# diku-kmc/kleenexlang

Measured on AMD Instinct MI355X. Metric: input GB/s + % HBM-read roofline, apache_log.kex over 10 GiB synthetic log, higher is better.
Workload: dtype u8

## Files before the change

include/kxhip.h:

```cpp
#ifndef KXHIP_H
#define KXHIP_H
#include <stddef.h>
#include <stdint.h>
#ifdef __cplusplus
extern "C" {
#endif

typedef struct kx_program kx_program;
typedef struct kx_shard kx_shard;

#define KX_OK 0
#define KX_MATCH_ERROR 1
#define KX_E_BLOB (-1)
#define KX_E_HIP (-2)
#define KX_E_CAPACITY (-3)
#define KX_E_ARG (-4)
#define KX_E_IO (-5)

enum { KX_K_SYNC = 0, KX_K_FORWARD = 1, KX_K_HEAD = 2, KX_K_BACKLEN = 3, KX_K_RESOLVE = 4, KX_K_EMIT = 5, KX_NKERNELS = 6 };

typedef struct kx_stats {
  uint64_t fail_pos;
  uint32_t fail_stage;
  uint32_t unsynced_segments;
// ... 44 lines not shown
int kx_load_config(const void* blob, size_t blob_len, const kx_config* cfg, kx_program** prog);
int kx_validate(const void* blob, size_t blob_len);
void kx_free(kx_program* prog);
const char* kx_last_error(void);
int kx_set_config(kx_program* prog, const kx_config* cfg);
uint32_t kx_num_stages(const kx_program* prog);
int kx_stage_has_actions(const kx_program* prog, uint32_t stage);

typedef struct kx_df_info {
  uint32_t available;
  uint32_t delay;
  uint32_t nstates;
  uint32_t nclasses;
  uint32_t image_bytes, off_pool, start_handle, dead_handle, escape_handle;
  uint32_t transitions, escapes;
  uint32_t transitions_start, escapes_start;
  uint32_t merge_window;
  char reason[96];
} kx_df_info;
int kx_df_describe(const void* blob, size_t blob_len, uint32_t stage, kx_df_info* info, void* image, size_t image_cap);
int kx_df_pending(const void* blob, size_t blob_len, uint32_t stage, uint32_t state, uint32_t slot, uint32_t* sst_state,
                  uint32_t* kinds, uint32_t* n_out);
int kx_df_describe_cfg(const void* blob, size_t blob_len, uint32_t stage, const kx_config* cfg, kx_df_info* info, void* image, size_t image_cap);
int kx_df_pending_cfg(const void* blob, size_t blob_len, uint32_t stage, const kx_config* cfg, uint32_t state, uint32_t slot,
                      uint32_t* sst_state, uint32_t* kinds, uint32_t* n_out);
int kx_df_deferred(const void* blob, size_t blob_len, uint32_t stage, const kx_config* cfg, uint32_t state, void* bytes, size_t cap, size_t* n_out);
int kx_df_start_of_state(const void* blob, size_t blob_len, uint32_t stage, const kx_config* cfg, uint32_t sst_state, uint32_t* handle);
int kx_stage_delayed_form(const kx_program* prog, uint32_t stage);
void kx_stage_reset_delayed_form(kx_program* prog, uint32_t stage);

#define KX_STAGE_MAIN 0u
#define KX_STAGE_ALT 1u
#define KX_STAGE_DELAYED 2u
#define KX_STAGE_SLOW 3u
typedef struct kx_stage_info {
  uint32_t size;
  uint32_t which;
  uint64_t image_bytes;
  uint32_t general, big, has_alt, has_df, actions, action_regs, max_const_len, reserved0;
  uint64_t lds_bytes, sync_lds_bytes;
  struct {
    uint64_t packed, pair, wlen, cls, nleaves, fin_leaf, sync16, init_off, init_len;
    uint32_t packed_words, off_fwd, off_ent, off_pool, off_cls, off_adesc, naid, nstates, nclasses, q0h, maxleaves, deadh, nullrow, cshift,
        debug, big, hshift, rshift, rbase, stage_words, pair_words, pair_magic, nsync, sync_multi, sync_words, off_tbl, xlat, tblmode,
        aid_mask, inl, jl, direct, short_consts, reserved0;
  } t;
  struct {
    uint64_t img, start_of_state, sl_fmap, sl_back, sl_nleaves, sl_fin_leaf, sl_cls, sl_pcoff, sl_pcpool, sl_pend, sl_defoff, sl_defpc, sl_q;
    uint32_t words, off_pool, deadh, esch, starth, K, C, orig_c4, hshift, short_consts, debug, nstates, J, wide, sl_Lm, sl_npc, sl_on, reserved0;
  } d;
} kx_stage_info;
int kx_stage_describe_cfg(const void* blob, size_t blob_len, uint32_t stage, const kx_config* cfg, uint32_t which, kx_stage_info* info,
                          void* image, size_t image_cap);

int kx_run_device(kx_program* prog, const void* d_in, size_t n, void* d_out, size_t cap, size_t* out_len,
                  kx_stats* stats, void* stream);

int kx_run_host(kx_program* prog, const void* in, size_t n, void** out, size_t* out_len, kx_stats* stats);
void kx_host_free(void* p);

int kx_run_fd(kx_program* prog, int in_fd, int out_fd, kx_stats* stats);

typedef struct kx_batch_doc {
  uint64_t fail_pos;
  uint32_t status;
  uint32_t fail_stage;
} kx_batch_doc;
typedef struct kx_batch_stats {
  uint64_t docs, docs_rejected;
  uint64_t docs_routed;
  uint64_t in_bytes, out_bytes;
  float forward_ms, back_ms, scan_ms, emit_ms, routed_ms, total_ms;
  uint64_t docs_replayed;
  float actions_ms;
  uint32_t reserved[1];
} kx_batch_stats;
int kx_run_batch(kx_program* prog, const void* d_in, const uint64_t* d_in_off, uint64_t n_docs, void* d_out, size_t cap,
                 uint64_t* d_out_off, kx_batch_doc* d_docs, size_t* out_len, kx_batch_stats* stats, void* stream);

typedef struct kx_batch_frame {
  uint32_t trim;
  uint32_t last_whole;
  uint32_t suffix_len;
  uint8_t suffix[8];
  uint32_t reserved[3];
} kx_batch_frame;
int kx_run_batch_framed(kx_program* prog, const void* d_in, const uint64_t* d_in_off, uint64_t n_docs, const kx_batch_frame* frame,
                        void* d_out, size_t cap, uint64_t* d_out_off, kx_batch_doc* d_docs, size_t* out_len, kx_batch_stats* stats,
                        void* stream);

int kx_split_records(const void* d_in, size_t n, uint8_t sep, uint64_t base, uint64_t* d_off, uint64_t cap,
                     uint64_t* n_records, void* stream);

typedef struct kx_records_stats {
  uint64_t records, records_rejected, records_routed, in_bytes, out_bytes, windows, longest_record;
  float split_ms, batch_ms, total_ms;
  uint32_t reserved[4];
} kx_records_stats;
int kx_run_records_fd(kx_program* p, int in_fd, int out_fd, uint8_t sep, int report_fd, kx_records_stats* stats);

int kx_split_records_quoted(const void* d_in, size_t n, uint8_t sep, uint8_t quote, uint32_t parity_in, uint64_t base,
                            uint64_t* d_off, uint64_t cap, uint64_t* n_records, uint32_t* parity_out, void* stream);
int kx_run_records_fd_quoted(kx_program* p, int in_fd, int out_fd, uint8_t sep, uint8_t quote, int report_fd,
                             kx_records_stats* stats);

int kx_split_records_escaped(const void* d_in, size_t n, uint8_t sep, int quote, uint8_t escape, uint32_t state_in, uint64_t base,
// ... 139 lines not shown
```

kleenexlang_amd/csrc/engine/gen_sweeps.py:

```python
#!/usr/bin/env python3
import sys

SD = "dst_sel:DWORD dst_unused:UNUSED_PAD"


def fwd2():
    L = []
    ap = L.append
    def cls_issue(ch, t, slot):
        wi, by = t >> 2, t & 3
        ap("v_lshlrev_b32_sdwa %%[x%s], 0, %%[w%d] %s src0_sel:DWORD src1_sel:BYTE_%d" % (ch, wi, SD, by))
        ap("ds_read_u8 %%[c%s%d], %%[x%s]" % (ch, slot, ch))
    base = {"A": 0, "B": 32}
    for d in (0, 1):
        for ch in "AB":
            cls_issue(ch, base[ch] + d, d)
    ap("s_waitcnt lgkmcnt(2)")
    for ch in "AB":
        ap("v_add_u32 %%[a%s], %%[h%s], %%[c%s0]" % (ch, ch, ch))
        ap("ds_read_b32 %%[e%s0], %%[a%s]" % (ch, ch))
    for j in range(32):
        cur, nxt = j & 1, (j + 1) & 1
        if j + 2 < 32:
            for ch in "AB":
# ... 314 lines not shown
            sweep2j(),
            ['[%s] "=&v"(%s)' % (t, t) for t in tmpj] + ['[leafA] "+v"(leafA)', '[oA] "+v"(oA)', '[leafB] "+v"(leafB)', '[oB] "+v"(oB)',
                                                        '[pA] "+v"(pA)', '[pB] "+v"(pB)'],
            ['[bo%d] "v"(bo[%d])' % (i, i) for i in range(32)] + ['[w%d] "v"(w[%d])' % (i, i) for i in range(16)],
            '"memory"')
    tmp = tmp + ["tiA", "tiB"]
    emit_fn(out, "piece_sweep2i",
            "const uint32_t (&bo)[32], const uint32_t (&w)[16], uint32_t leafA, uint32_t oA, uint32_t leafB, uint32_t oB, "
            "uint32_t& jb, uint32_t jlim",
            "uint32_t " + ", ".join(tmp) + ", st; unsigned long long sv, mA, mU;",
            sweep2(True),
            ['[%s] "=&v"(%s)' % (t, t) for t in tmp] + ['[sv] "=&s"(sv)', '[mA] "=&s"(mA)', '[mU] "=&s"(mU)', '[st] "=&s"(st)', '[leafA] "+v"(leafA)', '[oA] "+v"(oA)',
                                                       '[leafB] "+v"(leafB)', '[oB] "+v"(oB)', '[jb] "+s"(jb)'],
            ['[bo%d] "v"(bo[%d])' % (i, i) for i in range(32)] + ['[w%d] "v"(w[%d])' % (i, i) for i in range(16)] +
            ['[jlim] "s"(jlim)'],
            '"vcc", "scc", "memory"')


def main2(out):
    tmp = ["e0", "e1", "c0", "c1", "c2", "x"]
    emit_fn(out, "piece_forward1",
            "const uint32_t (&w)[16], uint32_t h, uint32_t himask, uint32_t (&bo)[32]",
            "uint32_t " + ", ".join(tmp) + ";",
            fwd1(True),
            ['[bo%d] "=&v"(bo[%d])' % (i, i) for i in range(32)] + ['[%s] "=&v"(%s)' % (t, t) for t in tmp],
            ['[w%d] "v"(w[%d])' % (i, i) for i in range(16)] + ['[h] "v"(h)', '[hm] "s"(himask)'],
            '"memory"')
    emit_fn(out, "piece_run1",
            "const uint32_t (&w)[16], uint32_t& h, uint32_t& mid",
            "uint32_t " + ", ".join(tmp) + ";",
            fwd1(False),
            ['[%s] "=&v"(%s)' % (t, t) for t in tmp] + ['[mid] "=&v"(mid)', '[h] "+v"(h)'],
            ['[w%d] "v"(w[%d])' % (i, i) for i in range(16)],
            '"memory"')
    emit_fn(out, "piece_walk1j",
            "const uint32_t (&bo)[32], uint32_t& leaf, uint32_t& sum, uint32_t& lmid, uint32_t& shi",
            "uint32_t a, e;",
            walk1(True),
            ['[a] "=&v"(a)', '[e] "=&v"(e)', '[lmid] "=&v"(lmid)', '[shi] "=&v"(shi)', '[leaf] "+v"(leaf)', '[sum] "+v"(sum)'],
            ['[bo%d] "v"(bo[%d])' % (i, i) for i in range(32)],
            '"memory"')
    emit_fn(out, "piece_walk1",
            "const uint32_t (&bo)[32], uint32_t& leaf, uint32_t& sum, uint32_t& lmid, uint32_t& shi",
            "uint32_t a, e;",
            walk1(),
            ['[a] "=&v"(a)', '[e] "=&v"(e)', '[lmid] "=&v"(lmid)', '[shi] "=&v"(shi)', '[leaf] "+v"(leaf)', '[sum] "+v"(sum)'],
            ['[bo%d] "v"(bo[%d])' % (i, i) for i in range(32)],
            '"memory"')


DF_WALK_E = {"A": (("v116", "v117"), ("v118", "v119")), "B": (("v120", "v121"), ("v122", "v123"))}


def dfrun1(wide=False):
    L = []
    ap = L.append
    E = (("%[e0]",), ("%[e1]",))
    def cls_issue(tt):
        ap("v_lshlrev_b32_sdwa %%[x], 0, %%[w%d] %s src0_sel:DWORD src1_sel:BYTE_%d" % (tt >> 2, SD, tt & 3))
        ap("ds_read_u8 %%[c%d], %%[x]" % (tt % 3))
    for tt in (0, 1, 2):
        cls_issue(tt)
    ap("s_waitcnt lgkmcnt(2)")
    if wide:
        ap("v_lshlrev_b32 %[c0], 3, %[c0]")
    ap("v_add_u32 %[x], %[h], %[c0]")
    ap("ds_read_b32 %s, %%[x]" % E[0][0])
    for j in range(64):
        cur, nxt = j & 1, (j + 1) & 1
        if j + 3 < 64:
            cls_issue(j + 3)
        ap("s_waitcnt lgkmcnt(%d)" % (1 if j + 3 < 64 else 0))
        if j + 1 < 64:
            if wide:
                ap("v_lshlrev_b32 %%[c%d], 3, %%[c%d]" % ((j + 1) % 3, (j + 1) % 3))
            ap("v_add_u32_sdwa %%[x], %s, %%[c%d] %s src0_sel:WORD_0 src1_sel:DWORD" % (E[cur][0], (j + 1) % 3, SD))
            ap("ds_read_b32 %s, %%[x]" % E[nxt][0])
        ap("v_add_u32_sdwa %%[sum], %%[sum], %s %s src0_sel:DWORD src1_sel:WORD_1" % (E[cur][0], SD))
        if j == 31:
            ap("v_and_b32 %%[mid], 0xffff, %s" % E[cur][0])
            ap("v_mov_b32 %[lenA], %[sum]")
            ap("v_and_b32 %[sum], 0xffffff00, %[sum]")
        if j == 63:
            ap("v_and_b32 %%[h], 0xffff, %s" % E[cur][0])
    return L


def dfwalk2(K, counted=True, wide=False):
    L = []
    ap = L.append
    base = {"A": 0, "B": 32}
    E = DF_WALK_E
    pair = lambda ch, k: "v[%s:%s]" % (E[ch][k][0][1:], E[ch][k][1][1:])
    def cls_issue(ch, t, slot):
        ap("v_lshlrev_b32_sdwa %%[x%s], 0, %%[w%d] %s src0_sel:DWORD src1_sel:BYTE_%d" % (ch, t >> 2, SD, t & 3))
        ap("ds_read_u8 %%[c%s%d], %%[x%s]" % (ch, slot, ch))
    twof = {"A": None, "B": None}
    ap("s_setprio 3")
    for d in (0, 1):
        for ch in "AB":
            cls_issue(ch, base[ch] + d, d)
    ap("s_waitcnt lgkmcnt(2)")
    for ch in "AB":
        if wide:
            ap("v_lshlrev_b32 %%[c%s0], 3, %%[c%s0]" % (ch, ch))
        ap("v_add_u32 %%[a%s0], %%[h%s], %%[c%s0]" % (ch, ch, ch))
        ap("ds_read_b64 %s, %%[a%s0]" % (pair(ch, 0), ch))
    for j in range(32):
        cur, nxt = j & 1, (j + 1) & 1
        if j + 2 < 32:
            for ch in "AB":
                cls_issue(ch, base[ch] + j + 2, (j + 2) % 3)
        ap("s_waitcnt lgkmcnt(%d)" % (2 if j == 0 else (4 if counted else 6) if j + 2 < 32 else (2 if counted else 4)))
        if j + 1 < 32:
            for ch in "AB":
                if wide:
                    ap("v_lshlrev_b32 %%[c%s%d], 3, %%[c%s%d]" % (ch, (j + 1) % 3, ch, (j + 1) % 3))
                ap("v_add_u32_sdwa %%[a%s%d], %s, %%[c%s%d] %s src0_sel:WORD_0 src1_sel:DWORD" % (ch, nxt, E[ch][cur][0], ch, (j + 1) % 3, SD))
                ap("ds_read_b64 %s, %%[a%s%d]" % (pair(ch, nxt), ch, nxt))
        for ch in "AB":
            t = base[ch] + j
            so = t - K
            hi, o, a, x = E[ch][cur][1], "%%[o%s]" % ch, "%%[a%s%d]" % (ch, cur), "%%[x%s]" % ch
            if so >= 0:
                wreg, by = "%%[w%d]" % (so >> 2), so & 3
            else:
                wreg, by = "%[wp]", (4 + so) & 3
            if by in (1, 3) and twof[ch] != wreg:
# ... 36 lines not shown
    E = DF_WALK_E["A"]
    pair = lambda k: "v[%s:%s]" % (E[k][0][1:], E[k][1][1:])
    def cls_issue(t, slot):
        ap("v_lshlrev_b32_sdwa %%[x], 0, %%[w%d] %s src0_sel:DWORD src1_sel:BYTE_%d" % (t >> 2, SD, t & 3))
        ap("ds_read_u8 %%[c%d], %%[x]" % slot)
    twof = None
    ap("s_setprio 3")
    for d in (0, 1, 2):
        cls_issue(d, d)
    ap("s_waitcnt lgkmcnt(2)")
    if wide:
        ap("v_lshlrev_b32 %[c0], 3, %[c0]")
    ap("v_add_u32 %[a0], %[h], %[c0]")
    ap("ds_read_b64 %s, %%[a0]" % pair(0))
    for j in range(32):
        cur, nxt = j & 1, (j + 1) & 1
        if j + 3 < 32:
            cls_issue(j + 3, (j + 3) % 3)
        ap("s_waitcnt lgkmcnt(%d)" % ((1 if j + 3 < 32 else 0) + (0 if j == 0 else 1)))
        if j + 1 < 32:
            if wide:
                ap("v_lshlrev_b32 %%[c%d], 3, %%[c%d]" % ((j + 1) % 3, (j + 1) % 3))
            ap("v_add_u32_sdwa %%[a%d], %s, %%[c%d] %s src0_sel:WORD_0 src1_sel:DWORD" % (nxt, E[cur][0], (j + 1) % 3, SD))
            ap("ds_read_b64 %s, %%[a%d]" % (pair(nxt), nxt))
        so = j - K
        hi, a = E[cur][1], "%%[a%d]" % cur
        if so >= 0:
            wreg, by = "%%[w%d]" % (so >> 2), so & 3
        else:
            wreg, by = "%[wp]", (4 + so) & 3
        if by in (1, 3) and twof != wreg:
            ap("v_lshrrev_b32 %%[tw], 8, %s" % wreg)
            twof = wreg
        src = "%[tw]" if by in (1, 3) else wreg
        wr = "ds_write_b8_d16_hi" if by >= 2 else "ds_write_b8"
        ap("v_cmp_gt_i32_sdwa vcc, 0, sext(%s) src0_sel:DWORD src1_sel:BYTE_2" % hi)
        ap("v_lshl_or_b32 %s, %%[o], 16, %s" % (a, a))
        ap("v_lshl_or_b32 %%[x], %s, 31, %%[o]" % hi)
        ap("v_add_u32_sdwa %%[o], %%[o], %s %s src0_sel:DWORD src1_sel:BYTE_3" % (hi, SD))
        ap("%s %%[x], %s" % (wr, src))
        ap("s_and_saveexec_b64 %[sv], vcc")
        ap("ds_write_b32 %%[p], %s" % a)
        ap("s_mov_b64 exec, %[sv]")
        ap("v_add_u32_sdwa %%[p], %%[p], %s %s src0_sel:DWORD src1_sel:BYTE_2" % (E[cur][0], SD))
    ap("s_setprio 0")
    return L


def main7(out):
    tmp = ["c0", "c1", "c2", "x", "e0", "e1"]
    emit_fn(out, "piece_dfrun1w",
            "const uint32_t (&w)[16], uint32_t& h, uint32_t& mid, uint32_t& lenA, uint32_t& sum",
            "uint32_t " + ", ".join(tmp) + ";",
            dfrun1(True),
            ['[%s] "=&v"(%s)' % (t, t) for t in tmp] + ['[mid] "=&v"(mid)', '[lenA] "=&v"(lenA)', '[h] "+v"(h)', '[sum] "+v"(sum)'],
            ['[w%d] "v"(w[%d])' % (i, i) for i in range(16)],
            '"memory"')
    emit_fn(out, "piece_dfrun1",
            "const uint32_t (&w)[16], uint32_t& h, uint32_t& mid, uint32_t& lenA, uint32_t& sum",
            "uint32_t " + ", ".join(tmp) + ";",
            dfrun1(),
            ['[%s] "=&v"(%s)' % (t, t) for t in tmp] + ['[mid] "=&v"(mid)', '[lenA] "=&v"(lenA)', '[h] "+v"(h)', '[sum] "+v"(sum)'],
            ['[w%d] "v"(w[%d])' % (i, i) for i in range(16)],
            '"memory"')
    tmp1 = ["c0", "c1", "c2", "x", "a0", "a1", "tw"]
    clob1 = ", ".join('"%s"' % r for pr in DF_WALK_E["A"] for r in pr)
    for K, wd in ((1, False), (2, False), (1, True), (2, True)):
        emit_fn(out, "piece_dfwalk1c%s_k%d" % ("w" if wd else "", K),
                "const uint32_t (&w)[8], uint32_t wp, uint32_t h, uint32_t& o, uint32_t& p",
                "uint32_t " + ", ".join(tmp1) + "; unsigned long long sv;",
                dfwalk1(K, wd),
                ['[%s] "=&v"(%s)' % (t, t) for t in tmp1] + ['[sv] "=&s"(sv)', '[o] "+v"(o)', '[p] "+v"(p)'],
                ['[w%d] "v"(w[%d])' % (i, i) for i in range(8)] + ['[wp] "v"(wp)', '[h] "v"(h)'],
                '"vcc", "scc", "memory", ' + clob1)
    tmp = ["cA0", "cA1", "cA2", "cB0", "cB1", "cB2", "xA", "xB", "aA0", "aA1", "aB0", "aB1", "twA", "twB"]
    clob = ", ".join('"%s"' % r for ch in "AB" for pr in DF_WALK_E[ch] for r in pr)
    for K, wd in ((1, False), (2, False), (1, True), (2, True)):
        emit_fn(out, "piece_dfwalk2c%s_k%d" % ("w" if wd else "", K),
                "const uint32_t (&w)[16], uint32_t wp, uint32_t hA, uint32_t& oA, uint32_t hB, uint32_t& oB, uint32_t& pA, uint32_t& pB",
                "uint32_t " + ", ".join(tmp) + "; unsigned long long sv;",
                dfwalk2(K, counted=True, wide=wd),
                ['[%s] "=&v"(%s)' % (t, t) for t in tmp] + ['[sv] "=&s"(sv)', '[oA] "+v"(oA)', '[oB] "+v"(oB)', '[pA] "+v"(pA)', '[pB] "+v"(pB)'],
                ['[w%d] "v"(w[%d])' % (i, i) for i in range(16)] + ['[wp] "v"(wp)', '[hA] "v"(hA)', '[hB] "v"(hB)'],
                '"vcc", "scc", "memory", ' + clob)


if __name__ == "__main__":
    main()
    main2(sys.stdout)
    main6(sys.stdout)
    main7(sys.stdout)
```

kleenexlang_amd/csrc/engine/kx_dfkernels.inc:

```

constexpr uint32_t DF_HOLE_MAX = 4096, DF_HOLE_FIRST = 1024, DF_SL_LEAVES = 32;
struct __attribute__((aligned(8))) DfRec { uint32_t x, y; };
constexpr uint32_t DFREC_OWN = 0x80000000u, DFREC_HOLE = 0x80000000u, DFREC_HOLE_FIRST = 0x40000000u;
constexpr uint32_t DF_MERGE_WINDOW_MAX = 64;
using kxst::DF_STEP_MAX;
constexpr uint32_t DF_HOLE_LEN_MAX = 0xFFFFu, DF_HOLE_CNT_MAX = 0x3FFFu, DF_WBASE_PIECES = 32;
constexpr DfRec dfrec_pack(uint32_t start, uint32_t middle, uint32_t lenA, uint32_t len, uint32_t kA, uint32_t kB) {
  return DfRec{(start >> 3) | ((middle >> 3) << 13) | (kA << 26), len | (lenA << 13) | (kB << 25)};
}
constexpr DfRec dfrec_pack_hole(uint32_t side_first, uint32_t entries, bool first, uint32_t len) {
  return DfRec{side_first, len | (entries << 16) | (first ? DFREC_HOLE_FIRST : 0u) | DFREC_HOLE};
}
constexpr bool dfrec_hole(DfRec r) { return (r.y & DFREC_HOLE) != 0; }
constexpr uint32_t dfrec_start(DfRec r) { return (r.x & 0x1FFFu) << 3; }
constexpr uint32_t dfrec_middle(DfRec r) { return ((r.x >> 13) & 0x1FFFu) << 3; }
constexpr uint32_t dfrec_kA(DfRec r) { return r.x >> 26; }
constexpr uint32_t dfrec_kB(DfRec r) { return (r.y >> 25) & 0x3Fu; }
constexpr uint32_t dfrec_len(DfRec r) { return r.y & 0x1FFFu; }
constexpr uint32_t dfrec_lenA(DfRec r) { return (r.y >> 13) & 0xFFFu; }
constexpr uint32_t dfrec_hole_side(DfRec r) { return r.x; }
constexpr uint32_t dfrec_hole_len(DfRec r) { return r.y & DF_HOLE_LEN_MAX; }
constexpr uint32_t dfrec_hole_entries(DfRec r) { return (r.y >> 16) & DF_HOLE_CNT_MAX; }
constexpr bool dfrec_hole_first(DfRec r) { return (r.y & DFREC_HOLE_FIRST) != 0; }
namespace dfrec_check {
constexpr uint32_t H = 65536 - 8, LA = HALF * DF_STEP_MAX, LN = PIECE * DF_STEP_MAX, KH = HALF;
constexpr DfRec top = dfrec_pack(H, H, LA, LN, KH, KH), one = dfrec_pack(8, 65536 - 16, 1, 2, 0, KH), zero = dfrec_pack(0, 0, 0, 0, 0, 0);
static_assert(sizeof(DfRec) == 8 && LN < (1u << 13) && LA < (1u << 12) && KH < (1u << 6), "piece record: a field outgrew its width");
static_assert(!dfrec_hole(top) && dfrec_start(top) == H && dfrec_middle(top) == H && dfrec_lenA(top) == LA && dfrec_len(top) == LN &&
              dfrec_kA(top) == KH && dfrec_kB(top) == KH, "piece record: every field at its maximum");
static_assert(!dfrec_hole(one) && dfrec_start(one) == 8 && dfrec_middle(one) == 65536 - 16 && dfrec_lenA(one) == 1 && dfrec_len(one) == 2 &&
              dfrec_kA(one) == 0 && dfrec_kB(one) == KH, "piece record: neighbouring fields do not bleed");
static_assert(!dfrec_hole(zero) && zero.x == 0 && zero.y == 0, "piece record: all fields zero");
constexpr DfRec htop = dfrec_pack_hole(0xFFFFFFFFu, DF_HOLE_CNT_MAX, true, DF_HOLE_LEN_MAX), hlow = dfrec_pack_hole(0, 0, false, 0);
static_assert(dfrec_hole(htop) && dfrec_hole_side(htop) == 0xFFFFFFFFu && dfrec_hole_entries(htop) == DF_HOLE_CNT_MAX && dfrec_hole_first(htop) &&
              dfrec_hole_len(htop) == DF_HOLE_LEN_MAX, "hole record: every field at its maximum");
static_assert(dfrec_hole(hlow) && dfrec_hole_side(hlow) == 0 && dfrec_hole_entries(hlow) == 0 && !dfrec_hole_first(hlow) && dfrec_hole_len(hlow) == 0, "hole record: all fields zero");
static_assert(PIECE + kxdf::DF_MAX_K + DF_MERGE_WINDOW_MAX <= DF_HOLE_CNT_MAX, "hole record: the entries of a piece fit");
static_assert((uint64_t)MAX_SEG * DF_STEP_MAX < DFREC_OWN, "wave base: a block part's output stays below the own flag");
static_assert(DF_WBASE_PIECES == HALF && 2 * DF_WBASE_PIECES == PIECE, "wave base: one word per wave-iteration of half pieces, two per iteration of pieces");
}
struct DfLds {
  const uint8_t* base; uint32_t csh;
  __device__ __forceinline__ uint32_t c8(uint32_t byte) const { return (uint32_t)base[byte] << csh; }
  __device__ __forceinline__ uint2 ent(uint32_t a) const { return *reinterpret_cast<const uint2*>(base + a); }
};
__device__ __forceinline__ DfLds df_stage(const DfDev& D, uint32_t* smem) {
  for (uint32_t i = threadIdx.x; i < D.words; i += blockDim.x) smem[i] = D.img[i];
  __syncthreads();
  return DfLds{reinterpret_cast<const uint8_t*>(smem), D.wide ? 3u : 0u};
}

__device__ __forceinline__ void df_run_piece(const uint32_t (&w)[16], uint32_t& h, uint32_t& mid, uint32_t& lenA, uint32_t& len, const DfLds& L) {
  uint32_t c[8], cn[8], sum = 0;
  static_for<0, 8>([&](auto ic) { constexpr int i = decltype(ic)::value; c[i] = L.c8(BYTE_AT_DEP(w, i, h)); });
  static_for<0, PIECE / 8>([&](auto gc) {
    constexpr int g = decltype(gc)::value;
    if constexpr (g + 1 < PIECE / 8)
      static_for<0, 8>([&](auto ic) { constexpr int i = decltype(ic)::value; cn[i] = L.c8(BYTE_AT_DEP(w, 8 * (g + 1) + i, h)); });
    static_for<0, 8>([&](auto ic) {
      constexpr int i = decltype(ic)::value;
      const uint2 e = L.ent(h + c[i]);
      h = e.x & 0xFFFFu; sum += e.y >> 24; tie(h, sum);
    });
    if constexpr (g == HALF / 8 - 1) { mid = h; lenA = sum; }
    if constexpr (g + 1 < PIECE / 8)
      static_for<0, 8>([&](auto ic) { constexpr int i = decltype(ic)::value; c[i] = cn[i]; });
  });
  len = sum;
}

__device__ __forceinline__ uint64_t df_own_start(uint32_t j, uint64_t n, uint64_t seg, int first_known, const uint64_t* __restrict__ seg_pos,
                                                 const uint16_t* __restrict__ seg_state, const DfDev& D) {
  if (j == 0 && first_known) return 0;
  const uint64_t p = seg_pos[j];
  if (p == UNSYNC) return UNSYNC;
  const uint32_t q = (((uint32_t)seg_state[j] << D.hshift) - OFF_FWD) / D.orig_c4;
  if (q >= D.nstates || D.start_of_state[q] == 0xFFFFu) return UNSYNC;
  const uint64_t b = (p + D.K + D.J + 63) & ~63ull;
  const uint64_t lim = ((uint64_t)j + 1) * seg < n ? ((uint64_t)j + 1) * seg : n;
  return b < lim ? b : UNSYNC;
}

struct DfSlowIO {
  const uint8_t* in; uint64_t n, a, end; uint32_t h0, last, is_last;
  uint32_t h_behind; uint32_t* side; uint32_t side_cap; Flags* flags; const uint8_t* lds; uint32_t clsh; uint8_t* lmap; uint32_t max_steps;
  uint32_t base, nd, h_next; uint64_t e_out;
};
__device__ __noinline__ int df_slow_resolve(DfSlowIO& io, const DfDev& D) {
  const uint8_t* __restrict__ in = io.in;
  const uint64_t n = io.n, a = io.a, end = io.end;
  const uint32_t h0 = io.h0;
  const bool last = io.last != 0, is_last = io.is_last != 0;
  uint32_t* side = io.side; const uint32_t side_cap = io.side_cap; Flags* flags = io.flags;
  if (!D.sl_on || !side) return 1;
  const uint32_t C = D.C, Lm = D.sl_Lm, K = D.K, NONE = D.sl_npc << 1;
  const uint32_t i0 = (h0 - 256u) / (C * 8u);
  uint32_t q = D.sl_q[i0];
  const uint32_t nd = D.sl_defoff[i0 + 1] - D.sl_defoff[i0];
  const uint64_t hard = a + io.max_steps < n ? a + io.max_steps : n;
  const uint32_t need = nd + K + (uint32_t)(hard - a) + 64u;
  const uint32_t base = atomicAdd(&flags->side_used, need);
  if ((uint64_t)base + need > side_cap) return 1;
// ... 83 lines not shown
    uint32_t v = 0xFFu; bool same = true;
    const uint32_t par[8] = {f1.x, f1.y, f1.z, f1.w, f2v.x, f2v.y, f2v.z, f2v.w};
#pragma unroll
    for (uint32_t l = 0; l < DF_SL_LEAVES; ++l) {
      const uint32_t pl = (par[l >> 2] >> (8 * (l & 3u))) & 0xFFu;
      const uint32_t x = l >= nnl || pl == 0xFFu ? 0xFFu : M[pl];
      if (l < nnl) M2[l] = (uint8_t)x;
      if (x != 0xFFu) { if (v == 0xFFu) v = x; else same = same && x == v; }
    }
    { uint8_t* tmp = M; M = M2; M2 = tmp; }
    q = nq; nl = nnl; ++t;
    if ((!same || v == 0xFFu) && ((t - a) & 63u) == 0 && t + PIECE <= end && D.start_of_state[q] != 0xFFFFu && agree_at(t, nl)) {
      qb[(t - a) >> 6] = (uint16_t)q;
      mode = 1; e_out = t;
      break;
    }
    if (!same || v == 0xFFu) continue;
    anchor_known(v);
    const uint64_t decided = anchor;
    prev = anchor; anchor = t;
    for (uint32_t l = 0; l < DF_SL_LEAVES; ++l) M[l] = (uint8_t)l;
    const uint64_t e = decided & ~63ull;
    if (e > a && e + PIECE <= end && D.start_of_state[qb[(e - a) >> 6]] != 0xFFFFu) { mode = 1; e_out = e; break; }
    if (!last && decided + K >= end) { mode = 2; e_out = end; break; }
  }
  (void)nl;
  uint32_t h_next = h0;
  if (mode == 1) h_next = D.start_of_state[qb[(e_out - a) >> 6]];
  if (mode == 3) {
    if (D.start_of_state[q] == 0xFFFFu) return 1;
    h_next = D.start_of_state[q];
  }
  if (mode == 2) {
    for (uint64_t u = end - K; u < end; ++u) if (u >= a) R[u - a] = NONE; else E[nd + K - (a - u)] = NONE;
    const uint32_t ix = (io.h_behind - 256u) / (C * 8u);
    uint32_t due = D.sl_defoff[ix + 1] - D.sl_defoff[ix];
    for (uint32_t idx = nd + K + (uint32_t)(end - K - a); due && idx-- > 0;) {
      const uint32_t pc = (E[idx] >> 1) & 0x3FFFFFFFu;
      if (pc < D.sl_npc && D.sl_pcoff[pc + 1] > D.sl_pcoff[pc]) { E[idx] = (E[idx] & 0x80000001u) | NONE; --due; }
    }
    if (due) return 1;
  }
  io.base = base; io.nd = nd; io.h_next = h_next; io.e_out = e_out;
  return 0;
}

template <int BT, uint32_t DF_STAGE, int MINW, bool SLOW>
__global__ __launch_bounds__(BT, MINW) void k_dforward(const uint8_t* __restrict__ in, uint64_t n, uint64_t seg, uint32_t nseg, int first_known,
                           const uint64_t* __restrict__ seg_pos, const uint16_t* __restrict__ seg_state,
                           DfRec* __restrict__ rec, uint32_t* __restrict__ wbase, uint32_t* __restrict__ own, uint32_t* __restrict__ spill, Flags* flags,
                           uint32_t* __restrict__ side, uint32_t side_cap, int is_last, DfDev D) {
  static_assert(DF_STAGE == 8 || DF_STAGE == 16, "a group of staged records is one or half a 128-byte line, and at least the slow path's 64-byte map");
  extern __shared__ __attribute__((aligned(16))) uint32_t smem[];
  DfLds L = df_stage(D, smem);
  uint2* lrec = reinterpret_cast<uint2*>(smem + ((D.words + 3) & ~3u)) + (size_t)threadIdx.x * DF_STAGE;
  const uint32_t k = blockIdx.x * blockDim.x + threadIdx.x;
  const uint32_t lane = threadIdx.x & 63;
  const uint64_t B = k < nseg ? df_own_start(k, n, seg, first_known, seg_pos, seg_state, D) : UNSYNC;
  bool alive = B != UNSYNC;
  const uint32_t dead = D.deadh, esc = D.esch;
  auto warm = [&](uint32_t jj, uint64_t Bj) -> uint32_t {
    if (jj == 0 && first_known) return D.starth;
    uint32_t hw = D.start_of_state[(((uint32_t)seg_state[jj] << D.hshift) - OFF_FWD) / D.orig_c4];
    for (uint64_t pw = seg_pos[jj]; pw < Bj;) {
      const uint2 v = *reinterpret_cast<const uint2*>(in + (pw & ~7ull));
      const uint64_t x = (uint64_t)v.x | ((uint64_t)v.y << 32);
      for (uint32_t b = (uint32_t)pw & 7u; b < 8u && pw < Bj; ++b, ++pw) hw = L.ent(hw + L.c8((uint32_t)(x >> (8 * b)) & 0xFFu)).x & 0xFFFFu;
    }
    if (hw == esc && jj == k) atomicAdd(&flags->warm_esc, 1u);
    return hw == esc || hw == dead ? 0xFFFFFFFFu : hw;
  };
  uint32_t h = dead, h_behind = 0;
  if (alive) { h = warm(k, B); if (h == 0xFFFFFFFFu) { alive = false; h = dead; } }
  uint32_t j = k + 1;
  uint64_t end = n;
  if (alive) for (; j < nseg; ++j) {
    const uint64_t b = df_own_start(j, n, seg, first_known, seg_pos, seg_state, D);
    if (b == UNSYNC) continue;
    h_behind = warm(j, b);
    if (h_behind != 0xFFFFFFFFu) { end = b; break; }
  }
  const bool last = alive && j >= nseg;
  uint64_t pos = alive ? B : 0;
  if (alive) atomicMin(&flags->df_first_own, (unsigned long long)B);
  bool failed = !alive;
  if (!alive) { end = 0; pos = 0; }
  uint32_t m = (uint32_t)(pos / seg), cum = 0, flag = DFREC_OWN;
  uint64_t block_end = ((uint64_t)m + 1) * seg;
  auto fail_in = [&](uint32_t h0, uint64_t p0, uint32_t plen) -> int {
    uint32_t hh = h0;
    for (uint32_t t = 0; t < plen; ++t) {
      const uint32_t nh = L.ent(hh + L.c8(in[p0 + t])).x & 0xFFFFu;
      if (nh == dead) { atomicMin(&flags->fail_pos, (unsigned long long)(p0 + t)); failed = true; return 1; }
      if (nh == esc) return 2;
      hh = nh;
    }
    failed = true;
    return 1;
  };
  uint32_t nst = 0; uint64_t gfirst = 0;
  auto flush_group = [&]() {
    uint2* dst = reinterpret_cast<uint2*>(rec + gfirst);
    for (uint32_t i = 0; i < nst; ++i) dst[i] = lrec[(gfirst + i) & (DF_STAGE - 1)];
    nst = 0;
  };
  const bool coop = !(D.debug & 256u);
  bool in_trip = false;
  auto stage_rec = [&](uint64_t pc, DfRec r) {
    if (nst == 0) gfirst = pc;
    if ((pc & (DF_WBASE_PIECES - 1)) == 0) wbase[pc / DF_WBASE_PIECES] = cum | flag;
    lrec[pc & (DF_STAGE - 1)] = make_uint2(r.x, r.y); ++nst;
    if (!in_trip && (pc & (DF_STAGE - 1)) == DF_STAGE - 1) flush_group();
  };
  auto group_aligned = [&]() { return ((uint32_t)(pos >> 6) & (DF_STAGE - 1)) == nst; };
  uint2* const lrec_wave = reinterpret_cast<uint2*>(smem + ((D.words + 3) & ~3u)) + (size_t)(threadIdx.x & ~63u) * DF_STAGE;
  auto coop_flush = [&]() {
    const bool full = nst == DF_STAGE && (gfirst & (DF_STAGE - 1)) == 0;
    if (!__any(full)) return;
    const uint32_t glo = (uint32_t)gfirst, ghi = (uint32_t)(gfirst >> 32) | (full ? 0u : 0x80000000u);
    constexpr uint32_t RPL = DF_STAGE / 8;
    const uint32_t team = lane & ~7u, r = (lane & 7u) * RPL;
    static_for<0, 8>([&](auto ic) {
      constexpr uint32_t i = decltype(ic)::value;
      const uint32_t slo = (uint32_t)__shfl((int)glo, (int)(team + i)), shi = (uint32_t)__shfl((int)ghi, (int)(team + i));
      if (!(shi & 0x80000000u)) {
        const uint64_t g = ((uint64_t)shi << 32) | slo;
        const uint2* src = lrec_wave + (size_t)(team + i) * DF_STAGE + r;
        if constexpr (RPL == 2) *reinterpret_cast<uint4*>(rec + g + r) = *reinterpret_cast<const uint4*>(src);
        else *reinterpret_cast<uint2*>(rec + g + r) = *src;
      }
    });
    if (full) nst = 0;
  };
  auto cross = [&]() { if (pos == block_end) { (flag ? own : spill)[m] = cum; cum = 0; flag = 0; ++m; block_end += seg; } };
  uint32_t kc_sum = 0, kc_max = 0, kc_n = 0;
  auto slow = [&](const uint64_t a, const uint32_t h0) -> int {
    flush_group();
    DfSlowIO io{in, n, a, end, h0, last ? 1u : 0u, (uint32_t)is_last, h_behind, side, side_cap, flags, L.base, D.wide ? 0u : 3u, reinterpret_cast<uint8_t*>(lrec), DF_HOLE_FIRST, 0, 0, 0, 0};
    {
      int rc = df_slow_resolve(io, D);
      if (rc == 3) { io.max_steps = DF_HOLE_MAX; rc = df_slow_resolve(io, D); }
      if (rc) return rc == 3 ? 1 : rc;
    }
    const uint32_t base = io.base, nd = io.nd, K = D.K;
    const uint64_t e_out = io.e_out;
    const uint32_t* const E = side + base;
    const uint64_t pend = (e_out + 63) & ~63ull;
    uint32_t idx = 0;
    for (uint64_t pp = a; pp < pend; pp += PIECE) {
      cross();
      const bool first = pp == a;
      const uint32_t steps = (uint32_t)((e_out - pp) < PIECE ? e_out - pp : PIECE);
      const uint32_t cnt = first ? nd + K + steps : steps;
      uint32_t len = 0;
      for (uint32_t x = 0; x < cnt; ++x) {
        const uint32_t ee = E[idx + x], pc = (ee >> 1) & 0x3FFFFFFFu;
        len += (ee & 1u) + (pc < D.sl_npc ? D.sl_pcoff[pc + 1] - D.sl_pcoff[pc] : 0u);
      }
      if (len > DF_HOLE_LEN_MAX || cnt > DF_HOLE_CNT_MAX) return 1;
      if (((pp >> 6) & (DF_WBASE_PIECES - 1)) == 0) wbase[(pp >> 6) / DF_WBASE_PIECES] = cum | flag;
      rec[pp >> 6] = dfrec_pack_hole(base + idx, cnt, first, len);
      idx += cnt; cum += len; pos = pp + steps;
    }
    h = io.h_next;
    atomicAdd(&flags->slow_steps, (uint32_t)(e_out - a));
    return 0;
  };
  bool need_slow = false;
  auto run_slow = [&]() {
    need_slow = false;
    int r = 1;
    if constexpr (SLOW) r = slow(pos, h);
    if (r) { if (r == 1) atomicAdd(&flags->df_esc, 1u); failed = true; }
  };
  auto do_piece = [&](const uint32_t (&w)[16]) -> bool {
    cross();
    const uint32_t h0 = h;
    uint32_t mid, sumA, sum = 0;
    if (D.wide) piece_dfrun1w(w, h, mid, sumA, sum); else piece_dfrun1(w, h, mid, sumA, sum);
    if (h == dead || h == esc) {
      if (fail_in(h0, pos, PIECE) == 2) { need_slow = true; h = h0; }
      return false;
    }
    const uint32_t kA = (sumA & 0xFFu) >> 2, kB = (sum & 0xFFu) >> 2;
    kc_sum += kA + kB; kc_max = kA + kB > kc_max ? kA + kB : kc_max; ++kc_n;
    stage_rec(pos >> 6, dfrec_pack(h0, mid, sumA >> 8, sum >> 8, kA, kB));
    cum += sum >> 8; pos += PIECE;
    return true;
  };
  auto single_piece = [&]() {
    uint32_t w[16];
    load_piece(in, n, pos, w);
    do_piece(w);
  };
  for (;;) {
  if (need_slow) run_slow();
  while (!failed && !need_slow && pos + PIECE <= end && ((pos & (8 * PIECE - 1)) || !group_aligned())) single_piece();
  for (;;) {
    const bool can = !failed && !need_slow && pos + 8 * PIECE <= end && !(pos & (8 * PIECE - 1)) && group_aligned();
    if (!__any(can) || __any(need_slow)) break;
    uint32_t line[8];
    {
      const uint32_t mine = can ? (uint32_t)(pos >> 7) : 0xFFFFFFFFu;
      static_for<0, 8>([&](auto ic) { constexpr int i = decltype(ic)::value; line[i] = __shfl(mine, (int)((lane & ~7u) + i)); });
    }
    auto issue = [&](uint32_t k2, uint4 (&dst)[8]) {
      static_for<0, 8>([&](auto ic) {
        constexpr int i = decltype(ic)::value;
        const uint64_t ln = line[i] != 0xFFFFFFFFu ? line[i] : 0u;
        dst[i] = *reinterpret_cast<const uint4*>(in + ((ln + k2) << 7) + (lane & 7u) * 16);
      });
    };
    uint4 v[8];
    issue(0, v);
    bool died = false;
    in_trip = coop;
#pragma nounroll
    for (uint32_t k2 = 0; k2 < 4; ++k2) {
      transpose8(v, lane);
      uint32_t wa[16], wb[16];
      static_for<0, 8>([&](auto ic) {
        constexpr int w = decltype(ic)::value;
        uint32_t (&dst)[16] = w < 4 ? wa : wb;
        dst[4 * (w & 3)] = v[w].x; dst[4 * (w & 3) + 1] = v[w].y; dst[4 * (w & 3) + 2] = v[w].z; dst[4 * (w & 3) + 3] = v[w].w;
      });
      bool go = can && !died;
      if (go && !do_piece(wa)) { died = true; go = false; }
      if (k2 < 3) issue(k2 + 1, v);
      if (go && !do_piece(wb)) died = true;
    }
    if (coop) coop_flush();
    in_trip = false;
  }
  if (!__any(!failed && (need_slow || pos + 8 * PIECE <= end))) break;
  }
  if (!alive) return;
  for (;;) {
  if (need_slow) run_slow();
  while (!failed && !need_slow && pos + PIECE <= end) single_piece();
  if (need_slow) continue;
  if (!failed && pos < end) {
    cross();
    const uint32_t plen = (uint32_t)(end - pos), h0 = h;
    uint32_t mid = h, lenA = 0, len = 0, kA = 0, kc = 0;
    for (uint32_t t = 0; t < plen; ++t) {
      if (t == HALF) { mid = h; lenA = len; kA = kc; }
      const uint2 e = L.ent(h + L.c8(in[pos + t]));
      h = e.x & 0xFFFFu; len += e.y >> 24; kc += (e.y >> 23) & 1u;
    }
    if (plen <= HALF) { mid = h; lenA = len; kA = kc; }
    if (h == dead || h == esc) {
      if (fail_in(h0, pos, plen) == 2) { h = h0; need_slow = true; continue; }
    }
    else { stage_rec(pos >> 6, dfrec_pack(h0, mid, lenA, len, kA, kc - kA)); cum += len; pos = end; }
  }
  break;
  }
  flush_group();
  if (failed) return;
  (flag ? own : spill)[m] = cum;
  if (last) flags->end_state = h;
  if (kc_n) { if ((k & 15u) == 0) { atomicAdd(&flags->emit_ksum, kc_sum); atomicAdd(&flags->emit_kn, kc_n); } atomicMax(&flags->emit_kmax, kc_max); }
}

__global__ void k_dhead(const uint8_t* __restrict__ in, uint64_t n, uint64_t seg, uint64_t head_len, uint32_t h,
                        DfRec* __restrict__ rec, uint32_t* __restrict__ wbase, uint32_t* __restrict__ own, uint32_t* __restrict__ spill, Flags* flags, DfDev D) {
  extern __shared__ __attribute__((aligned(16))) uint32_t smem[];
  DfLds L = df_stage(D, smem);
  if (blockIdx.x || threadIdx.x) return;
  const uint32_t dead = D.deadh, esc = D.esch;
  uint32_t m = 0, cum = 0;
  uint64_t block_end = seg;
  for (uint64_t pos = 0; pos < head_len;) {
    if (pos == block_end) { spill[m] = cum; cum = 0; ++m; block_end += seg; }
    const uint32_t plen = (uint32_t)(head_len - pos < PIECE ? head_len - pos : PIECE);
    const uint32_t h0 = h;
    uint32_t mid = h, lenA = 0, len = 0, kA = 0, kc = 0;
    for (uint32_t t = 0; t < plen; ++t) {
      if (t == HALF) { mid = h; lenA = len; kA = kc; }
      const uint2 e = L.ent(h + L.c8(in[pos + t]));
      const uint32_t nh = e.x & 0xFFFFu;
      if (nh == dead) { atomicMin(&flags->fail_pos, (unsigned long long)(pos + t)); return; }
      if (nh == esc) { flags->df_esc = 1; return; }
      h = nh; len += e.y >> 24; kc += (e.y >> 23) & 1u;
    }
    if (plen <= HALF) { mid = h; lenA = len; kA = kc; }
    if (kc > 0) atomicMax(&flags->emit_kmax, kc);
    if (((pos >> 6) & (DF_WBASE_PIECES - 1)) == 0) wbase[(pos >> 6) / DF_WBASE_PIECES] = cum;
    rec[pos >> 6] = dfrec_pack(h0, mid, lenA, len, kA, kc - kA);
    cum += len; pos += plen;
  }
  spill[m] = cum;
  if (head_len == n) flags->end_state = h;
}

__global__ void k_dlen(uint32_t nblk, const uint32_t* __restrict__ own, const uint32_t* __restrict__ spill, uint32_t* __restrict__ len,
                       unsigned long long* __restrict__ wsum) {
  __shared__ unsigned long long red[1024];
  const uint32_t m = blockIdx.x * blockDim.x + threadIdx.x;
  uint32_t mylen = 0;
  if (m < nblk) { mylen = own[m] + spill[m]; len[m] = mylen; }
  red[threadIdx.x] = mylen;
  __syncthreads();
  for (uint32_t s = blockDim.x >> 1; s > 0; s >>= 1) {
    if (threadIdx.x < s) red[threadIdx.x] += red[threadIdx.x + s];
    __syncthreads();
  }
  if (threadIdx.x == 0) wsum[blockIdx.x] = red[0];
}

template <bool GENERAL>
__global__ void k_dmap(const uint8_t* __restrict__ in, uint64_t n, uint32_t q_in, uint64_t cap, uint8_t* __restrict__ map_out,
                       uint32_t* __restrict__ status, DevTables T) {
  extern __shared__ __attribute__((aligned(16))) uint32_t smem[];
// ... 309 lines not shown
```

kleenexlang_amd/csrc/engine/kx_engine.hip:

```cpp
#include <hip/hip_runtime.h>
#include <fcntl.h>
#include <sys/stat.h>
#include <unistd.h>

#include <cerrno>
#include <condition_variable>
#include <cstdint>
#include <algorithm>
#include <deque>
#include <mutex>
#include <chrono>
#include <thread>
#include <cstdio>
#include <cstdlib>
#include <cstring>
#include <string>
#include <type_traits>
#include <vector>

#include "../../../include/kxhip.h"
#include "../../../include/kxp_format.h"
#include "kx_stage.h"

namespace {
// ... 1833 lines not shown

}

extern "C" {

const char* kx_last_error(void) { return g_err.c_str(); }
void kx_internal_set_error(const char* m) { g_err = m ? m : ""; }

static int buildStage(const uint8_t*& c, const uint8_t* end, const kx_config& cfg, unsigned what, Stage& S) {
  std::string err;
  const int rc = kxst::buildStage(c, end, cfg, what, S, err);
  return rc ? setErr(rc, err) : 0;
}
static int blobHeader(const void* blob, size_t blob_len, const uint8_t** first, uint32_t* nstages) {
  std::string err;
  const int rc = kxst::readBlobHeader(blob, blob_len, first, nstages, err);
  return rc ? setErr(rc, err) : 0;
}

int kx_validate(const void* blob, size_t blob_len) {
  const uint8_t* c = nullptr; uint32_t ns = 0;
  int rc = blobHeader(blob, blob_len, &c, &ns);
  for (uint32_t s = 0; s < ns && !rc; ++s) {
    Stage S;
    rc = buildStage(c, (const uint8_t*)blob + blob_len, kx_config{}, 0, S);
  }
  return rc;
}

static int parseOneStage(const void* blob, size_t blob_len, uint32_t stage, const kx_config* cfgp, Stage& S, unsigned what = kxst::WITH_DELAYED) {
  const uint8_t* c; uint32_t ns;
  int rc = blobHeader(blob, blob_len, &c, &ns);
  if (rc) return rc;
  if (stage >= ns) return setErr(KX_E_ARG, "no such stage");
  for (uint32_t st = 0; st <= stage && !rc; ++st) {
    Stage T;
    rc = buildStage(c, (const uint8_t*)blob + blob_len, cfgp ? *cfgp : kx_config{}, st == stage ? what : 0, st == stage ? S : T);
  }
  return rc;
}

int kx_stage_describe_cfg(const void* blob, size_t blob_len, uint32_t stage, const kx_config* cfg, uint32_t which, kx_stage_info* info,
                          void* image, size_t image_cap) {
  if (!info || info->size != sizeof(kx_stage_info) || which > KX_STAGE_SLOW) return setErr(KX_E_ARG, "kx_stage_info::size is not this library's, or no such image");
  Stage S;
  int rc = parseOneStage(blob, blob_len, stage, cfg, S, kxst::WITH_ALT | kxst::WITH_DELAYED);
  if (rc) return rc;
  kxst::describeStage(S, which, *info);
  const std::vector<uint8_t>& bytes = which == KX_STAGE_MAIN ? S.img : which == KX_STAGE_ALT ? S.img_alt : which == KX_STAGE_DELAYED ? S.img_df : S.img_slow;
  if (image && !bytes.empty()) memcpy(image, bytes.data(), image_cap < bytes.size() ? image_cap : bytes.size());
  return 0;
}

int kx_df_describe(const void* blob, size_t blob_len, uint32_t stage, kx_df_info* info, void* image, size_t image_cap) {
  return kx_df_describe_cfg(blob, blob_len, stage, nullptr, info, image, image_cap);
}

int kx_df_describe_cfg(const void* blob, size_t blob_len, uint32_t stage, const kx_config* cfg, kx_df_info* info, void* image, size_t image_cap) {
  if (!info) return setErr(KX_E_ARG, "null argument");
  Stage S;
  int rc = parseOneStage(blob, blob_len, stage, cfg, S);
  if (rc) return rc;
  memset(info, 0, sizeof *info);
  info->available = S.has_df ? 1u : 0u;
  snprintf(info->reason, sizeof info->reason, "%s", S.df_why.c_str());
  if (S.df.nP) {
    info->delay = S.df.K; info->nstates = S.df.nP; info->nclasses = S.df.C; info->image_bytes = (uint32_t)S.df.img.size() * 4;
    info->off_pool = S.df.off_pool; info->start_handle = S.df.starth; info->dead_handle = S.df.deadh; info->escape_handle = S.df.esch;
    info->transitions = S.df.ntrans; info->escapes = S.df.nesc; info->transitions_start = S.df.ntrans_start; info->escapes_start = S.df.nesc_start;
    info->merge_window = S.df.J;
    if (image) memcpy(image, S.df.img.data(), image_cap < S.df.img.size() * 4 ? image_cap : S.df.img.size() * 4);
  }
  return 0;
}

int kx_df_pending(const void* blob, size_t blob_len, uint32_t stage, uint32_t state, uint32_t slot, uint32_t* sst_state,
                  uint32_t* kinds, uint32_t* n_out) {
  return kx_df_pending_cfg(blob, blob_len, stage, nullptr, state, slot, sst_state, kinds, n_out);
}

int kx_df_pending_cfg(const void* blob, size_t blob_len, uint32_t stage, const kx_config* cfg, uint32_t state, uint32_t slot,
                      uint32_t* sst_state, uint32_t* kinds, uint32_t* n_out) {
  if (!kinds || !n_out || !sst_state) return setErr(KX_E_ARG, "null argument");
  Stage S;
  int rc = parseOneStage(blob, blob_len, stage, cfg, S);
  if (rc) return rc;
  if (state >= S.df.states.size() || slot >= S.df.K) return setErr(KX_E_ARG, "no such product state / slot");
  const kxdf::Slot& g = S.df.states[state].pend[slot];
  *sst_state = S.df.states[state].q;
  *n_out = (uint32_t)g.size();
  for (size_t i = 0; i < g.size() && i < KX_MAX_LEAVES; ++i) kinds[i] = g[i];
  return 0;
}

int kx_df_deferred(const void* blob, size_t blob_len, uint32_t stage, const kx_config* cfg, uint32_t state, void* bytes, size_t cap, size_t* n_out) {
  if (!n_out || (cap && !bytes)) return setErr(KX_E_ARG, "null argument");
  Stage S;
  int rc = parseOneStage(blob, blob_len, stage, cfg, S);
  if (rc) return rc;
  if (state >= S.df.states.size()) return setErr(KX_E_ARG, "no such product state");
  std::string t;
  for (const auto& d : S.df.states[state].def)
    if (d.first < S.df_pc_len.size()) t.append((const char*)S.h_pool.data() + S.df_pc_off[d.first], S.df_pc_len[d.first]);
  *n_out = t.size();
  if (cap) memcpy(bytes, t.data(), t.size() < cap ? t.size() : cap);
  return 0;
// ... 1159 lines not shown
```

kleenexlang_amd/csrc/engine/kx_stage.h:

```cpp
#ifndef KX_STAGE_H
#define KX_STAGE_H
#include <cstdint>
#include <cstring>
#include <string>
#include <vector>

#include "../../../include/kxhip.h"
#include "../../../include/kxp_format.h"
#include "kx_delayed.h"

namespace kxst {

#ifdef __HIP__
using Quad = uint4;
#else
struct Quad { uint32_t x, y, z, w; };
#endif

constexpr uint32_t OFF_FWD = 256;
constexpr uint32_t PAIR_CLS2_AT = 16128;
constexpr uint32_t DF_STEP_MAX = 126;

struct DevTables {
  const uint32_t* packed;
  uint32_t packed_words;
  uint32_t off_fwd, off_ent, off_pool, off_cls, off_adesc, naid;
  uint32_t nstates, nclasses, q0h, maxleaves, deadh, nullrow, cshift, debug;
  uint32_t big, hshift, rshift, rbase, stage_words;
  const uint32_t* pair; uint32_t pair_words, pair_magic;
  const uint32_t* wlen;
  const uint8_t* cls;
  const uint8_t* nleaves;
  const uint8_t* fin_leaf;
  const uint16_t* sync16;
  uint32_t nsync, sync_multi, sync_words;
  const uint32_t* init_off;
  const uint32_t* init_len;
  uint32_t off_tbl, xlat, tblmode, aid_mask;
  uint32_t inl;
  uint32_t jl;
  uint32_t direct;
  uint32_t short_consts;
};

struct DfDev {
  const uint32_t* img; uint32_t words;
  uint32_t off_pool, deadh, esch, starth, K, C;
  const uint16_t* start_of_state;
  uint32_t orig_c4, hshift;
  uint32_t short_consts, debug;
  uint32_t nstates;
  uint32_t J;
  uint32_t wide;
  const Quad* sl_fmap;
  const uint32_t* sl_back; const uint8_t* sl_nleaves; const uint8_t* sl_fin_leaf; const uint8_t* sl_cls;
  const uint32_t* sl_pcoff; const uint8_t* sl_pcpool; const uint32_t* sl_pend; const uint32_t* sl_defoff; const uint32_t* sl_defpc; const uint16_t* sl_q;
  uint32_t sl_Lm, sl_npc, sl_on;
};

template <class P> void setOff(const P*& p, size_t off) { p = reinterpret_cast<const P*>(off); }
template <class P> size_t offOf(const P* p) { return reinterpret_cast<size_t>(p); }
template <class P> void rebase(const P*& p, const void* base) { p = reinterpret_cast<const P*>(reinterpret_cast<uintptr_t>(base) + offOf(p)); }
// ... 546 lines not shown
```

kleenexlang_amd/csrc/engine/kx_sweeps.inc:

```

__device__ __forceinline__ void piece_forward2(const uint32_t (&w)[16], uint32_t hA, uint32_t hB, uint32_t himask, uint32_t (&bo)[32]) {
  uint32_t eA0, eA1, eB0, eB1, cA0, cA1, cA2, cB0, cB1, cB2, xA, xB, aA, aB;
  asm volatile(
      "v_lshlrev_b32_sdwa %[xA], 0, %[w0] dst_sel:DWORD dst_unused:UNUSED_PAD src0_sel:DWORD src1_sel:BYTE_0\n"
      "ds_read_u8 %[cA0], %[xA]\n"
      "v_lshlrev_b32_sdwa %[xB], 0, %[w8] dst_sel:DWORD dst_unused:UNUSED_PAD src0_sel:DWORD src1_sel:BYTE_0\n"
      "ds_read_u8 %[cB0], %[xB]\n"
      "v_lshlrev_b32_sdwa %[xA], 0, %[w0] dst_sel:DWORD dst_unused:UNUSED_PAD src0_sel:DWORD src1_sel:BYTE_1\n"
      "ds_read_u8 %[cA1], %[xA]\n"
      "v_lshlrev_b32_sdwa %[xB], 0, %[w8] dst_sel:DWORD dst_unused:UNUSED_PAD src0_sel:DWORD src1_sel:BYTE_1\n"
      "ds_read_u8 %[cB1], %[xB]\n"
      "s_waitcnt lgkmcnt(2)\n"
      "v_add_u32 %[aA], %[hA], %[cA0]\n"
      "ds_read_b32 %[eA0], %[aA]\n"
      "v_add_u32 %[aB], %[hB], %[cB0]\n"
      "ds_read_b32 %[eB0], %[aB]\n"
      "v_lshlrev_b32_sdwa %[xA], 0, %[w0] dst_sel:DWORD dst_unused:UNUSED_PAD src0_sel:DWORD src1_sel:BYTE_2\n"
      "ds_read_u8 %[cA2], %[xA]\n"
      "v_lshlrev_b32_sdwa %[xB], 0, %[w8] dst_sel:DWORD dst_unused:UNUSED_PAD src0_sel:DWORD src1_sel:BYTE_2\n"
      "ds_read_u8 %[cB2], %[xB]\n"
      "s_waitcnt lgkmcnt(2)\n"
      "v_add_u32_sdwa %[aA], %[eA0], %[cA1] dst_sel:DWORD dst_unused:UNUSED_PAD src0_sel:WORD_0 src1_sel:DWORD\n"
      "ds_read_b32 %[eA1], %[aA]\n"
      "v_add_u32_sdwa %[aB], %[eB0], %[cB1] dst_sel:DWORD dst_unused:UNUSED_PAD src0_sel:WORD_0 src1_sel:DWORD\n"
// ... 6631 lines not shown
      "v_mad_u32_u24 %[p1], %[c0a], %[C], %[c0b]\n"
      "s_waitcnt lgkmcnt(2)\n"
      "v_lshl_add_u32 %[x], %[e0], 1, %[p1]\n"
      "ds_read_u16 %[e1], %[x] offset:16384\n"
      "v_lshlrev_b32_sdwa %[x], 0, %[w14] dst_sel:DWORD dst_unused:UNUSED_PAD src0_sel:DWORD src1_sel:BYTE_2\n"
      "ds_read_u8 %[c2a], %[x] offset:16128\n"
      "v_lshlrev_b32_sdwa %[x], 0, %[w14] dst_sel:DWORD dst_unused:UNUSED_PAD src0_sel:DWORD src1_sel:BYTE_3\n"
      "ds_read_u8 %[c2b], %[x] offset:16128\n"
      "s_waitcnt lgkmcnt(3)\n"
      "v_mad_u32_u24 %[p0], %[c1a], %[C], %[c1b]\n"
      "s_waitcnt lgkmcnt(2)\n"
      "v_lshl_add_u32 %[x], %[e1], 1, %[p0]\n"
      "ds_read_u16 %[e0], %[x] offset:16384\n"
      "v_lshlrev_b32_sdwa %[x], 0, %[w15] dst_sel:DWORD dst_unused:UNUSED_PAD src0_sel:DWORD src1_sel:BYTE_0\n"
      "ds_read_u8 %[c0a], %[x] offset:16128\n"
      "v_lshlrev_b32_sdwa %[x], 0, %[w15] dst_sel:DWORD dst_unused:UNUSED_PAD src0_sel:DWORD src1_sel:BYTE_1\n"
      "ds_read_u8 %[c0b], %[x] offset:16128\n"
      "s_waitcnt lgkmcnt(3)\n"
      "v_mad_u32_u24 %[p1], %[c2a], %[C], %[c2b]\n"
      "s_waitcnt lgkmcnt(2)\n"
      "v_lshl_add_u32 %[x], %[e0], 1, %[p1]\n"
      "ds_read_u16 %[e1], %[x] offset:16384\n"
      "v_lshlrev_b32_sdwa %[x], 0, %[w15] dst_sel:DWORD dst_unused:UNUSED_PAD src0_sel:DWORD src1_sel:BYTE_2\n"
      "ds_read_u8 %[c1a], %[x] offset:16128\n"
      "v_lshlrev_b32_sdwa %[x], 0, %[w15] dst_sel:DWORD dst_unused:UNUSED_PAD src0_sel:DWORD src1_sel:BYTE_3\n"
      "ds_read_u8 %[c1b], %[x] offset:16128\n"
      "s_waitcnt lgkmcnt(3)\n"
      "v_mad_u32_u24 %[p0], %[c0a], %[C], %[c0b]\n"
      "s_waitcnt lgkmcnt(2)\n"
      "v_lshl_add_u32 %[x], %[e1], 1, %[p0]\n"
      "ds_read_u16 %[e0], %[x] offset:16384\n"
      "s_waitcnt lgkmcnt(1)\n"
      "v_mad_u32_u24 %[p1], %[c1a], %[C], %[c1b]\n"
      "s_waitcnt lgkmcnt(0)\n"
      "v_lshl_add_u32 %[x], %[e0], 1, %[p1]\n"
      "ds_read_u16 %[e1], %[x] offset:16384\n"
      "s_waitcnt lgkmcnt(0)\n"
      "v_mov_b32 %[e], %[e1]\n"
      : [e0] "=&v"(e0), [e1] "=&v"(e1), [c0a] "=&v"(c0a), [c0b] "=&v"(c0b), [c1a] "=&v"(c1a), [c1b] "=&v"(c1b), [c2a] "=&v"(c2a), [c2b] "=&v"(c2b), [p0] "=&v"(p0), [p1] "=&v"(p1), [x] "=&v"(x), [mid] "=&v"(mid), [e] "+v"(e)
      : [w0] "v"(w[0]), [w1] "v"(w[1]), [w2] "v"(w[2]), [w3] "v"(w[3]), [w4] "v"(w[4]), [w5] "v"(w[5]), [w6] "v"(w[6]), [w7] "v"(w[7]), [w8] "v"(w[8]), [w9] "v"(w[9]), [w10] "v"(w[10]), [w11] "v"(w[11]), [w12] "v"(w[12]), [w13] "v"(w[13]), [w14] "v"(w[14]), [w15] "v"(w[15]), [C] "s"(C)
      : "memory");
}

__device__ __forceinline__ void piece_dfrun1w(const uint32_t (&w)[16], uint32_t& h, uint32_t& mid, uint32_t& lenA, uint32_t& sum) {
  uint32_t c0, c1, c2, x, e0, e1;
  asm volatile(
      "v_lshlrev_b32_sdwa %[x], 0, %[w0] dst_sel:DWORD dst_unused:UNUSED_PAD src0_sel:DWORD src1_sel:BYTE_0\n"
      "ds_read_u8 %[c0], %[x]\n"
      "v_lshlrev_b32_sdwa %[x], 0, %[w0] dst_sel:DWORD dst_unused:UNUSED_PAD src0_sel:DWORD src1_sel:BYTE_1\n"
      "ds_read_u8 %[c1], %[x]\n"
      "v_lshlrev_b32_sdwa %[x], 0, %[w0] dst_sel:DWORD dst_unused:UNUSED_PAD src0_sel:DWORD src1_sel:BYTE_2\n"
      "ds_read_u8 %[c2], %[x]\n"
      "s_waitcnt lgkmcnt(2)\n"
      "v_lshlrev_b32 %[c0], 3, %[c0]\n"
      "v_add_u32 %[x], %[h], %[c0]\n"
      "ds_read_b32 %[e0], %[x]\n"
      "v_lshlrev_b32_sdwa %[x], 0, %[w0] dst_sel:DWORD dst_unused:UNUSED_PAD src0_sel:DWORD src1_sel:BYTE_3\n"
      "ds_read_u8 %[c0], %[x]\n"
      "s_waitcnt lgkmcnt(1)\n"
      "v_lshlrev_b32 %[c1], 3, %[c1]\n"
      "v_add_u32_sdwa %[x], %[e0], %[c1] dst_sel:DWORD dst_unused:UNUSED_PAD src0_sel:WORD_0 src1_sel:DWORD\n"
      "ds_read_b32 %[e1], %[x]\n"
      "v_add_u32_sdwa %[sum], %[sum], %[e0] dst_sel:DWORD dst_unused:UNUSED_PAD src0_sel:DWORD src1_sel:WORD_1\n"
      "v_lshlrev_b32_sdwa %[x], 0, %[w1] dst_sel:DWORD dst_unused:UNUSED_PAD src0_sel:DWORD src1_sel:BYTE_0\n"
      "ds_read_u8 %[c1], %[x]\n"
      "s_waitcnt lgkmcnt(1)\n"
      "v_lshlrev_b32 %[c2], 3, %[c2]\n"
      "v_add_u32_sdwa %[x], %[e1], %[c2] dst_sel:DWORD dst_unused:UNUSED_PAD src0_sel:WORD_0 src1_sel:DWORD\n"
      "ds_read_b32 %[e0], %[x]\n"
      "v_add_u32_sdwa %[sum], %[sum], %[e1] dst_sel:DWORD dst_unused:UNUSED_PAD src0_sel:DWORD src1_sel:WORD_1\n"
      "v_lshlrev_b32_sdwa %[x], 0, %[w1] dst_sel:DWORD dst_unused:UNUSED_PAD src0_sel:DWORD src1_sel:BYTE_1\n"
      "ds_read_u8 %[c2], %[x]\n"
      "s_waitcnt lgkmcnt(1)\n"
      "v_lshlrev_b32 %[c0], 3, %[c0]\n"
      "v_add_u32_sdwa %[x], %[e0], %[c0] dst_sel:DWORD dst_unused:UNUSED_PAD src0_sel:WORD_0 src1_sel:DWORD\n"
      "ds_read_b32 %[e1], %[x]\n"
      "v_add_u32_sdwa %[sum], %[sum], %[e0] dst_sel:DWORD dst_unused:UNUSED_PAD src0_sel:DWORD src1_sel:WORD_1\n"
      "v_lshlrev_b32_sdwa %[x], 0, %[w1] dst_sel:DWORD dst_unused:UNUSED_PAD src0_sel:DWORD src1_sel:BYTE_2\n"
      "ds_read_u8 %[c0], %[x]\n"
      "s_waitcnt lgkmcnt(1)\n"
      "v_lshlrev_b32 %[c1], 3, %[c1]\n"
      "v_add_u32_sdwa %[x], %[e1], %[c1] dst_sel:DWORD dst_unused:UNUSED_PAD src0_sel:WORD_0 src1_sel:DWORD\n"
      "ds_read_b32 %[e0], %[x]\n"
      "v_add_u32_sdwa %[sum], %[sum], %[e1] dst_sel:DWORD dst_unused:UNUSED_PAD src0_sel:DWORD src1_sel:WORD_1\n"
      "v_lshlrev_b32_sdwa %[x], 0, %[w1] dst_sel:DWORD dst_unused:UNUSED_PAD src0_sel:DWORD src1_sel:BYTE_3\n"
      "ds_read_u8 %[c1], %[x]\n"
      "s_waitcnt lgkmcnt(1)\n"
      "v_lshlrev_b32 %[c2], 3, %[c2]\n"
      "v_add_u32_sdwa %[x], %[e0], %[c2] dst_sel:DWORD dst_unused:UNUSED_PAD src0_sel:WORD_0 src1_sel:DWORD\n"
      "ds_read_b32 %[e1], %[x]\n"
      "v_add_u32_sdwa %[sum], %[sum], %[e0] dst_sel:DWORD dst_unused:UNUSED_PAD src0_sel:DWORD src1_sel:WORD_1\n"
      "v_lshlrev_b32_sdwa %[x], 0, %[w2] dst_sel:DWORD dst_unused:UNUSED_PAD src0_sel:DWORD src1_sel:BYTE_0\n"
      "ds_read_u8 %[c2], %[x]\n"
      "s_waitcnt lgkmcnt(1)\n"
      "v_lshlrev_b32 %[c0], 3, %[c0]\n"
      "v_add_u32_sdwa %[x], %[e1], %[c0] dst_sel:DWORD dst_unused:UNUSED_PAD src0_sel:WORD_0 src1_sel:DWORD\n"
      "ds_read_b32 %[e0], %[x]\n"
      "v_add_u32_sdwa %[sum], %[sum], %[e1] dst_sel:DWORD dst_unused:UNUSED_PAD src0_sel:DWORD src1_sel:WORD_1\n"
      "v_lshlrev_b32_sdwa %[x], 0, %[w2] dst_sel:DWORD dst_unused:UNUSED_PAD src0_sel:DWORD src1_sel:BYTE_1\n"
      "ds_read_u8 %[c0], %[x]\n"
      "s_waitcnt lgkmcnt(1)\n"
      "v_lshlrev_b32 %[c1], 3, %[c1]\n"
      "v_add_u32_sdwa %[x], %[e0], %[c1] dst_sel:DWORD dst_unused:UNUSED_PAD src0_sel:WORD_0 src1_sel:DWORD\n"
      "ds_read_b32 %[e1], %[x]\n"
      "v_add_u32_sdwa %[sum], %[sum], %[e0] dst_sel:DWORD dst_unused:UNUSED_PAD src0_sel:DWORD src1_sel:WORD_1\n"
      "v_lshlrev_b32_sdwa %[x], 0, %[w2] dst_sel:DWORD dst_unused:UNUSED_PAD src0_sel:DWORD src1_sel:BYTE_2\n"
      "ds_read_u8 %[c1], %[x]\n"
      "s_waitcnt lgkmcnt(1)\n"
      "v_lshlrev_b32 %[c2], 3, %[c2]\n"
      "v_add_u32_sdwa %[x], %[e1], %[c2] dst_sel:DWORD dst_unused:UNUSED_PAD src0_sel:WORD_0 src1_sel:DWORD\n"
      "ds_read_b32 %[e0], %[x]\n"
      "v_add_u32_sdwa %[sum], %[sum], %[e1] dst_sel:DWORD dst_unused:UNUSED_PAD src0_sel:DWORD src1_sel:WORD_1\n"
      "v_lshlrev_b32_sdwa %[x], 0, %[w2] dst_sel:DWORD dst_unused:UNUSED_PAD src0_sel:DWORD src1_sel:BYTE_3\n"
      "ds_read_u8 %[c2], %[x]\n"
      "s_waitcnt lgkmcnt(1)\n"
      "v_lshlrev_b32 %[c0], 3, %[c0]\n"
      "v_add_u32_sdwa %[x], %[e0], %[c0] dst_sel:DWORD dst_unused:UNUSED_PAD src0_sel:WORD_0 src1_sel:DWORD\n"
      "ds_read_b32 %[e1], %[x]\n"
      "v_add_u32_sdwa %[sum], %[sum], %[e0] dst_sel:DWORD dst_unused:UNUSED_PAD src0_sel:DWORD src1_sel:WORD_1\n"
      "v_lshlrev_b32_sdwa %[x], 0, %[w3] dst_sel:DWORD dst_unused:UNUSED_PAD src0_sel:DWORD src1_sel:BYTE_0\n"
      "ds_read_u8 %[c0], %[x]\n"
      "s_waitcnt lgkmcnt(1)\n"
      "v_lshlrev_b32 %[c1], 3, %[c1]\n"
      "v_add_u32_sdwa %[x], %[e1], %[c1] dst_sel:DWORD dst_unused:UNUSED_PAD src0_sel:WORD_0 src1_sel:DWORD\n"
      "ds_read_b32 %[e0], %[x]\n"
      "v_add_u32_sdwa %[sum], %[sum], %[e1] dst_sel:DWORD dst_unused:UNUSED_PAD src0_sel:DWORD src1_sel:WORD_1\n"
      "v_lshlrev_b32_sdwa %[x], 0, %[w3] dst_sel:DWORD dst_unused:UNUSED_PAD src0_sel:DWORD src1_sel:BYTE_1\n"
      "ds_read_u8 %[c1], %[x]\n"
      "s_waitcnt lgkmcnt(1)\n"
      "v_lshlrev_b32 %[c2], 3, %[c2]\n"
      "v_add_u32_sdwa %[x], %[e0], %[c2] dst_sel:DWORD dst_unused:UNUSED_PAD src0_sel:WORD_0 src1_sel:DWORD\n"
      "ds_read_b32 %[e1], %[x]\n"
      "v_add_u32_sdwa %[sum], %[sum], %[e0] dst_sel:DWORD dst_unused:UNUSED_PAD src0_sel:DWORD src1_sel:WORD_1\n"
      "v_lshlrev_b32_sdwa %[x], 0, %[w3] dst_sel:DWORD dst_unused:UNUSED_PAD src0_sel:DWORD src1_sel:BYTE_2\n"
      "ds_read_u8 %[c2], %[x]\n"
      "s_waitcnt lgkmcnt(1)\n"
      "v_lshlrev_b32 %[c0], 3, %[c0]\n"
      "v_add_u32_sdwa %[x], %[e1], %[c0] dst_sel:DWORD dst_unused:UNUSED_PAD src0_sel:WORD_0 src1_sel:DWORD\n"
      "ds_read_b32 %[e0], %[x]\n"
      "v_add_u32_sdwa %[sum], %[sum], %[e1] dst_sel:DWORD dst_unused:UNUSED_PAD src0_sel:DWORD src1_sel:WORD_1\n"
      "v_lshlrev_b32_sdwa %[x], 0, %[w3] dst_sel:DWORD dst_unused:UNUSED_PAD src0_sel:DWORD src1_sel:BYTE_3\n"
      "ds_read_u8 %[c0], %[x]\n"
      "s_waitcnt lgkmcnt(1)\n"
      "v_lshlrev_b32 %[c1], 3, %[c1]\n"
      "v_add_u32_sdwa %[x], %[e0], %[c1] dst_sel:DWORD dst_unused:UNUSED_PAD src0_sel:WORD_0 src1_sel:DWORD\n"
      "ds_read_b32 %[e1], %[x]\n"
      "v_add_u32_sdwa %[sum], %[sum], %[e0] dst_sel:DWORD dst_unused:UNUSED_PAD src0_sel:DWORD src1_sel:WORD_1\n"
      "v_lshlrev_b32_sdwa %[x], 0, %[w4] dst_sel:DWORD dst_unused:UNUSED_PAD src0_sel:DWORD src1_sel:BYTE_0\n"
      "ds_read_u8 %[c1], %[x]\n"
      "s_waitcnt lgkmcnt(1)\n"
      "v_lshlrev_b32 %[c2], 3, %[c2]\n"
      "v_add_u32_sdwa %[x], %[e1], %[c2] dst_sel:DWORD dst_unused:UNUSED_PAD src0_sel:WORD_0 src1_sel:DWORD\n"
      "ds_read_b32 %[e0], %[x]\n"
      "v_add_u32_sdwa %[sum], %[sum], %[e1] dst_sel:DWORD dst_unused:UNUSED_PAD src0_sel:DWORD src1_sel:WORD_1\n"
      "v_lshlrev_b32_sdwa %[x], 0, %[w4] dst_sel:DWORD dst_unused:UNUSED_PAD src0_sel:DWORD src1_sel:BYTE_1\n"
      "ds_read_u8 %[c2], %[x]\n"
      "s_waitcnt lgkmcnt(1)\n"
      "v_lshlrev_b32 %[c0], 3, %[c0]\n"
      "v_add_u32_sdwa %[x], %[e0], %[c0] dst_sel:DWORD dst_unused:UNUSED_PAD src0_sel:WORD_0 src1_sel:DWORD\n"
      "ds_read_b32 %[e1], %[x]\n"
      "v_add_u32_sdwa %[sum], %[sum], %[e0] dst_sel:DWORD dst_unused:UNUSED_PAD src0_sel:DWORD src1_sel:WORD_1\n"
      "v_lshlrev_b32_sdwa %[x], 0, %[w4] dst_sel:DWORD dst_unused:UNUSED_PAD src0_sel:DWORD src1_sel:BYTE_2\n"
      "ds_read_u8 %[c0], %[x]\n"
      "s_waitcnt lgkmcnt(1)\n"
      "v_lshlrev_b32 %[c1], 3, %[c1]\n"
      "v_add_u32_sdwa %[x], %[e1], %[c1] dst_sel:DWORD dst_unused:UNUSED_PAD src0_sel:WORD_0 src1_sel:DWORD\n"
      "ds_read_b32 %[e0], %[x]\n"
      "v_add_u32_sdwa %[sum], %[sum], %[e1] dst_sel:DWORD dst_unused:UNUSED_PAD src0_sel:DWORD src1_sel:WORD_1\n"
      "v_lshlrev_b32_sdwa %[x], 0, %[w4] dst_sel:DWORD dst_unused:UNUSED_PAD src0_sel:DWORD src1_sel:BYTE_3\n"
      "ds_read_u8 %[c1], %[x]\n"
      "s_waitcnt lgkmcnt(1)\n"
      "v_lshlrev_b32 %[c2], 3, %[c2]\n"
      "v_add_u32_sdwa %[x], %[e0], %[c2] dst_sel:DWORD dst_unused:UNUSED_PAD src0_sel:WORD_0 src1_sel:DWORD\n"
      "ds_read_b32 %[e1], %[x]\n"
      "v_add_u32_sdwa %[sum], %[sum], %[e0] dst_sel:DWORD dst_unused:UNUSED_PAD src0_sel:DWORD src1_sel:WORD_1\n"
      "v_lshlrev_b32_sdwa %[x], 0, %[w5] dst_sel:DWORD dst_unused:UNUSED_PAD src0_sel:DWORD src1_sel:BYTE_0\n"
      "ds_read_u8 %[c2], %[x]\n"
      "s_waitcnt lgkmcnt(1)\n"
      "v_lshlrev_b32 %[c0], 3, %[c0]\n"
      "v_add_u32_sdwa %[x], %[e1], %[c0] dst_sel:DWORD dst_unused:UNUSED_PAD src0_sel:WORD_0 src1_sel:DWORD\n"
      "ds_read_b32 %[e0], %[x]\n"
      "v_add_u32_sdwa %[sum], %[sum], %[e1] dst_sel:DWORD dst_unused:UNUSED_PAD src0_sel:DWORD src1_sel:WORD_1\n"
      "v_lshlrev_b32_sdwa %[x], 0, %[w5] dst_sel:DWORD dst_unused:UNUSED_PAD src0_sel:DWORD src1_sel:BYTE_1\n"
      "ds_read_u8 %[c0], %[x]\n"
      "s_waitcnt lgkmcnt(1)\n"
      "v_lshlrev_b32 %[c1], 3, %[c1]\n"
      "v_add_u32_sdwa %[x], %[e0], %[c1] dst_sel:DWORD dst_unused:UNUSED_PAD src0_sel:WORD_0 src1_sel:DWORD\n"
      "ds_read_b32 %[e1], %[x]\n"
      "v_add_u32_sdwa %[sum], %[sum], %[e0] dst_sel:DWORD dst_unused:UNUSED_PAD src0_sel:DWORD src1_sel:WORD_1\n"
      "v_lshlrev_b32_sdwa %[x], 0, %[w5] dst_sel:DWORD dst_unused:UNUSED_PAD src0_sel:DWORD src1_sel:BYTE_2\n"
      "ds_read_u8 %[c1], %[x]\n"
      "s_waitcnt lgkmcnt(1)\n"
      "v_lshlrev_b32 %[c2], 3, %[c2]\n"
      "v_add_u32_sdwa %[x], %[e1], %[c2] dst_sel:DWORD dst_unused:UNUSED_PAD src0_sel:WORD_0 src1_sel:DWORD\n"
      "ds_read_b32 %[e0], %[x]\n"
      "v_add_u32_sdwa %[sum], %[sum], %[e1] dst_sel:DWORD dst_unused:UNUSED_PAD src0_sel:DWORD src1_sel:WORD_1\n"
      "v_lshlrev_b32_sdwa %[x], 0, %[w5] dst_sel:DWORD dst_unused:UNUSED_PAD src0_sel:DWORD src1_sel:BYTE_3\n"
      "ds_read_u8 %[c2], %[x]\n"
      "s_waitcnt lgkmcnt(1)\n"
      "v_lshlrev_b32 %[c0], 3, %[c0]\n"
      "v_add_u32_sdwa %[x], %[e0], %[c0] dst_sel:DWORD dst_unused:UNUSED_PAD src0_sel:WORD_0 src1_sel:DWORD\n"
      "ds_read_b32 %[e1], %[x]\n"
      "v_add_u32_sdwa %[sum], %[sum], %[e0] dst_sel:DWORD dst_unused:UNUSED_PAD src0_sel:DWORD src1_sel:WORD_1\n"
      "v_lshlrev_b32_sdwa %[x], 0, %[w6] dst_sel:DWORD dst_unused:UNUSED_PAD src0_sel:DWORD src1_sel:BYTE_0\n"
      "ds_read_u8 %[c0], %[x]\n"
      "s_waitcnt lgkmcnt(1)\n"
      "v_lshlrev_b32 %[c1], 3, %[c1]\n"
      "v_add_u32_sdwa %[x], %[e1], %[c1] dst_sel:DWORD dst_unused:UNUSED_PAD src0_sel:WORD_0 src1_sel:DWORD\n"
      "ds_read_b32 %[e0], %[x]\n"
      "v_add_u32_sdwa %[sum], %[sum], %[e1] dst_sel:DWORD dst_unused:UNUSED_PAD src0_sel:DWORD src1_sel:WORD_1\n"
      "v_lshlrev_b32_sdwa %[x], 0, %[w6] dst_sel:DWORD dst_unused:UNUSED_PAD src0_sel:DWORD src1_sel:BYTE_1\n"
      "ds_read_u8 %[c1], %[x]\n"
      "s_waitcnt lgkmcnt(1)\n"
      "v_lshlrev_b32 %[c2], 3, %[c2]\n"
      "v_add_u32_sdwa %[x], %[e0], %[c2] dst_sel:DWORD dst_unused:UNUSED_PAD src0_sel:WORD_0 src1_sel:DWORD\n"
      "ds_read_b32 %[e1], %[x]\n"
      "v_add_u32_sdwa %[sum], %[sum], %[e0] dst_sel:DWORD dst_unused:UNUSED_PAD src0_sel:DWORD src1_sel:WORD_1\n"
      "v_lshlrev_b32_sdwa %[x], 0, %[w6] dst_sel:DWORD dst_unused:UNUSED_PAD src0_sel:DWORD src1_sel:BYTE_2\n"
      "ds_read_u8 %[c2], %[x]\n"
      "s_waitcnt lgkmcnt(1)\n"
      "v_lshlrev_b32 %[c0], 3, %[c0]\n"
      "v_add_u32_sdwa %[x], %[e1], %[c0] dst_sel:DWORD dst_unused:UNUSED_PAD src0_sel:WORD_0 src1_sel:DWORD\n"
      "ds_read_b32 %[e0], %[x]\n"
      "v_add_u32_sdwa %[sum], %[sum], %[e1] dst_sel:DWORD dst_unused:UNUSED_PAD src0_sel:DWORD src1_sel:WORD_1\n"
      "v_lshlrev_b32_sdwa %[x], 0, %[w6] dst_sel:DWORD dst_unused:UNUSED_PAD src0_sel:DWORD src1_sel:BYTE_3\n"
      "ds_read_u8 %[c0], %[x]\n"
      "s_waitcnt lgkmcnt(1)\n"
      "v_lshlrev_b32 %[c1], 3, %[c1]\n"
      "v_add_u32_sdwa %[x], %[e0], %[c1] dst_sel:DWORD dst_unused:UNUSED_PAD src0_sel:WORD_0 src1_sel:DWORD\n"
      "ds_read_b32 %[e1], %[x]\n"
      "v_add_u32_sdwa %[sum], %[sum], %[e0] dst_sel:DWORD dst_unused:UNUSED_PAD src0_sel:DWORD src1_sel:WORD_1\n"
      "v_lshlrev_b32_sdwa %[x], 0, %[w7] dst_sel:DWORD dst_unused:UNUSED_PAD src0_sel:DWORD src1_sel:BYTE_0\n"
      "ds_read_u8 %[c1], %[x]\n"
      "s_waitcnt lgkmcnt(1)\n"
      "v_lshlrev_b32 %[c2], 3, %[c2]\n"
      "v_add_u32_sdwa %[x], %[e1], %[c2] dst_sel:DWORD dst_unused:UNUSED_PAD src0_sel:WORD_0 src1_sel:DWORD\n"
      "ds_read_b32 %[e0], %[x]\n"
      "v_add_u32_sdwa %[sum], %[sum], %[e1] dst_sel:DWORD dst_unused:UNUSED_PAD src0_sel:DWORD src1_sel:WORD_1\n"
      "v_lshlrev_b32_sdwa %[x], 0, %[w7] dst_sel:DWORD dst_unused:UNUSED_PAD src0_sel:DWORD src1_sel:BYTE_1\n"
      "ds_read_u8 %[c2], %[x]\n"
      "s_waitcnt lgkmcnt(1)\n"
      "v_lshlrev_b32 %[c0], 3, %[c0]\n"
      "v_add_u32_sdwa %[x], %[e0], %[c0] dst_sel:DWORD dst_unused:UNUSED_PAD src0_sel:WORD_0 src1_sel:DWORD\n"
      "ds_read_b32 %[e1], %[x]\n"
      "v_add_u32_sdwa %[sum], %[sum], %[e0] dst_sel:DWORD dst_unused:UNUSED_PAD src0_sel:DWORD src1_sel:WORD_1\n"
      "v_lshlrev_b32_sdwa %[x], 0, %[w7] dst_sel:DWORD dst_unused:UNUSED_PAD src0_sel:DWORD src1_sel:BYTE_2\n"
      "ds_read_u8 %[c0], %[x]\n"
      "s_waitcnt lgkmcnt(1)\n"
      "v_lshlrev_b32 %[c1], 3, %[c1]\n"
      "v_add_u32_sdwa %[x], %[e1], %[c1] dst_sel:DWORD dst_unused:UNUSED_PAD src0_sel:WORD_0 src1_sel:DWORD\n"
      "ds_read_b32 %[e0], %[x]\n"
      "v_add_u32_sdwa %[sum], %[sum], %[e1] dst_sel:DWORD dst_unused:UNUSED_PAD src0_sel:DWORD src1_sel:WORD_1\n"
      "v_lshlrev_b32_sdwa %[x], 0, %[w7] dst_sel:DWORD dst_unused:UNUSED_PAD src0_sel:DWORD src1_sel:BYTE_3\n"
      "ds_read_u8 %[c1], %[x]\n"
      "s_waitcnt lgkmcnt(1)\n"
      "v_lshlrev_b32 %[c2], 3, %[c2]\n"
      "v_add_u32_sdwa %[x], %[e0], %[c2] dst_sel:DWORD dst_unused:UNUSED_PAD src0_sel:WORD_0 src1_sel:DWORD\n"
      "ds_read_b32 %[e1], %[x]\n"
      "v_add_u32_sdwa %[sum], %[sum], %[e0] dst_sel:DWORD dst_unused:UNUSED_PAD src0_sel:DWORD src1_sel:WORD_1\n"
      "v_lshlrev_b32_sdwa %[x], 0, %[w8] dst_sel:DWORD dst_unused:UNUSED_PAD src0_sel:DWORD src1_sel:BYTE_0\n"
      "ds_read_u8 %[c2], %[x]\n"
      "s_waitcnt lgkmcnt(1)\n"
      "v_lshlrev_b32 %[c0], 3, %[c0]\n"
      "v_add_u32_sdwa %[x], %[e1], %[c0] dst_sel:DWORD dst_unused:UNUSED_PAD src0_sel:WORD_0 src1_sel:DWORD\n"
      "ds_read_b32 %[e0], %[x]\n"
      "v_add_u32_sdwa %[sum], %[sum], %[e1] dst_sel:DWORD dst_unused:UNUSED_PAD src0_sel:DWORD src1_sel:WORD_1\n"
      "v_lshlrev_b32_sdwa %[x], 0, %[w8] dst_sel:DWORD dst_unused:UNUSED_PAD src0_sel:DWORD src1_sel:BYTE_1\n"
      "ds_read_u8 %[c0], %[x]\n"
      "s_waitcnt lgkmcnt(1)\n"
      "v_lshlrev_b32 %[c1], 3, %[c1]\n"
      "v_add_u32_sdwa %[x], %[e0], %[c1] dst_sel:DWORD dst_unused:UNUSED_PAD src0_sel:WORD_0 src1_sel:DWORD\n"
      "ds_read_b32 %[e1], %[x]\n"
      "v_add_u32_sdwa %[sum], %[sum], %[e0] dst_sel:DWORD dst_unused:UNUSED_PAD src0_sel:DWORD src1_sel:WORD_1\n"
      "v_lshlrev_b32_sdwa %[x], 0, %[w8] dst_sel:DWORD dst_unused:UNUSED_PAD src0_sel:DWORD src1_sel:BYTE_2\n"
      "ds_read_u8 %[c1], %[x]\n"
      "s_waitcnt lgkmcnt(1)\n"
      "v_lshlrev_b32 %[c2], 3, %[c2]\n"
      "v_add_u32_sdwa %[x], %[e1], %[c2] dst_sel:DWORD dst_unused:UNUSED_PAD src0_sel:WORD_0 src1_sel:DWORD\n"
      "ds_read_b32 %[e0], %[x]\n"
      "v_add_u32_sdwa %[sum], %[sum], %[e1] dst_sel:DWORD dst_unused:UNUSED_PAD src0_sel:DWORD src1_sel:WORD_1\n"
      "v_and_b32 %[mid], 0xffff, %[e1]\n"
      "v_mov_b32 %[lenA], %[sum]\n"
      "v_and_b32 %[sum], 0xffffff00, %[sum]\n"
      "v_lshlrev_b32_sdwa %[x], 0, %[w8] dst_sel:DWORD dst_unused:UNUSED_PAD src0_sel:DWORD src1_sel:BYTE_3\n"
      "ds_read_u8 %[c2], %[x]\n"
      "s_waitcnt lgkmcnt(1)\n"
      "v_lshlrev_b32 %[c0], 3, %[c0]\n"
      "v_add_u32_sdwa %[x], %[e0], %[c0] dst_sel:DWORD dst_unused:UNUSED_PAD src0_sel:WORD_0 src1_sel:DWORD\n"
      "ds_read_b32 %[e1], %[x]\n"
      "v_add_u32_sdwa %[sum], %[sum], %[e0] dst_sel:DWORD dst_unused:UNUSED_PAD src0_sel:DWORD src1_sel:WORD_1\n"
      "v_lshlrev_b32_sdwa %[x], 0, %[w9] dst_sel:DWORD dst_unused:UNUSED_PAD src0_sel:DWORD src1_sel:BYTE_0\n"
      "ds_read_u8 %[c0], %[x]\n"
      "s_waitcnt lgkmcnt(1)\n"
      "v_lshlrev_b32 %[c1], 3, %[c1]\n"
      "v_add_u32_sdwa %[x], %[e1], %[c1] dst_sel:DWORD dst_unused:UNUSED_PAD src0_sel:WORD_0 src1_sel:DWORD\n"
      "ds_read_b32 %[e0], %[x]\n"
      "v_add_u32_sdwa %[sum], %[sum], %[e1] dst_sel:DWORD dst_unused:UNUSED_PAD src0_sel:DWORD src1_sel:WORD_1\n"
      "v_lshlrev_b32_sdwa %[x], 0, %[w9] dst_sel:DWORD dst_unused:UNUSED_PAD src0_sel:DWORD src1_sel:BYTE_1\n"
      "ds_read_u8 %[c1], %[x]\n"
      "s_waitcnt lgkmcnt(1)\n"
      "v_lshlrev_b32 %[c2], 3, %[c2]\n"
      "v_add_u32_sdwa %[x], %[e0], %[c2] dst_sel:DWORD dst_unused:UNUSED_PAD src0_sel:WORD_0 src1_sel:DWORD\n"
      "ds_read_b32 %[e1], %[x]\n"
      "v_add_u32_sdwa %[sum], %[sum], %[e0] dst_sel:DWORD dst_unused:UNUSED_PAD src0_sel:DWORD src1_sel:WORD_1\n"
      "v_lshlrev_b32_sdwa %[x], 0, %[w9] dst_sel:DWORD dst_unused:UNUSED_PAD src0_sel:DWORD src1_sel:BYTE_2\n"
      "ds_read_u8 %[c2], %[x]\n"
      "s_waitcnt lgkmcnt(1)\n"
      "v_lshlrev_b32 %[c0], 3, %[c0]\n"
      "v_add_u32_sdwa %[x], %[e1], %[c0] dst_sel:DWORD dst_unused:UNUSED_PAD src0_sel:WORD_0 src1_sel:DWORD\n"
      "ds_read_b32 %[e0], %[x]\n"
      "v_add_u32_sdwa %[sum], %[sum], %[e1] dst_sel:DWORD dst_unused:UNUSED_PAD src0_sel:DWORD src1_sel:WORD_1\n"
      "v_lshlrev_b32_sdwa %[x], 0, %[w9] dst_sel:DWORD dst_unused:UNUSED_PAD src0_sel:DWORD src1_sel:BYTE_3\n"
      "ds_read_u8 %[c0], %[x]\n"
      "s_waitcnt lgkmcnt(1)\n"
      "v_lshlrev_b32 %[c1], 3, %[c1]\n"
      "v_add_u32_sdwa %[x], %[e0], %[c1] dst_sel:DWORD dst_unused:UNUSED_PAD src0_sel:WORD_0 src1_sel:DWORD\n"
      "ds_read_b32 %[e1], %[x]\n"
      "v_add_u32_sdwa %[sum], %[sum], %[e0] dst_sel:DWORD dst_unused:UNUSED_PAD src0_sel:DWORD src1_sel:WORD_1\n"
      "v_lshlrev_b32_sdwa %[x], 0, %[w10] dst_sel:DWORD dst_unused:UNUSED_PAD src0_sel:DWORD src1_sel:BYTE_0\n"
      "ds_read_u8 %[c1], %[x]\n"
      "s_waitcnt lgkmcnt(1)\n"
      "v_lshlrev_b32 %[c2], 3, %[c2]\n"
      "v_add_u32_sdwa %[x], %[e1], %[c2] dst_sel:DWORD dst_unused:UNUSED_PAD src0_sel:WORD_0 src1_sel:DWORD\n"
      "ds_read_b32 %[e0], %[x]\n"
      "v_add_u32_sdwa %[sum], %[sum], %[e1] dst_sel:DWORD dst_unused:UNUSED_PAD src0_sel:DWORD src1_sel:WORD_1\n"
      "v_lshlrev_b32_sdwa %[x], 0, %[w10] dst_sel:DWORD dst_unused:UNUSED_PAD src0_sel:DWORD src1_sel:BYTE_1\n"
      "ds_read_u8 %[c2], %[x]\n"
      "s_waitcnt lgkmcnt(1)\n"
      "v_lshlrev_b32 %[c0], 3, %[c0]\n"
      "v_add_u32_sdwa %[x], %[e0], %[c0] dst_sel:DWORD dst_unused:UNUSED_PAD src0_sel:WORD_0 src1_sel:DWORD\n"
      "ds_read_b32 %[e1], %[x]\n"
      "v_add_u32_sdwa %[sum], %[sum], %[e0] dst_sel:DWORD dst_unused:UNUSED_PAD src0_sel:DWORD src1_sel:WORD_1\n"
      "v_lshlrev_b32_sdwa %[x], 0, %[w10] dst_sel:DWORD dst_unused:UNUSED_PAD src0_sel:DWORD src1_sel:BYTE_2\n"
      "ds_read_u8 %[c0], %[x]\n"
      "s_waitcnt lgkmcnt(1)\n"
      "v_lshlrev_b32 %[c1], 3, %[c1]\n"
      "v_add_u32_sdwa %[x], %[e1], %[c1] dst_sel:DWORD dst_unused:UNUSED_PAD src0_sel:WORD_0 src1_sel:DWORD\n"
      "ds_read_b32 %[e0], %[x]\n"
      "v_add_u32_sdwa %[sum], %[sum], %[e1] dst_sel:DWORD dst_unused:UNUSED_PAD src0_sel:DWORD src1_sel:WORD_1\n"
      "v_lshlrev_b32_sdwa %[x], 0, %[w10] dst_sel:DWORD dst_unused:UNUSED_PAD src0_sel:DWORD src1_sel:BYTE_3\n"
      "ds_read_u8 %[c1], %[x]\n"
      "s_waitcnt lgkmcnt(1)\n"
      "v_lshlrev_b32 %[c2], 3, %[c2]\n"
      "v_add_u32_sdwa %[x], %[e0], %[c2] dst_sel:DWORD dst_unused:UNUSED_PAD src0_sel:WORD_0 src1_sel:DWORD\n"
      "ds_read_b32 %[e1], %[x]\n"
      "v_add_u32_sdwa %[sum], %[sum], %[e0] dst_sel:DWORD dst_unused:UNUSED_PAD src0_sel:DWORD src1_sel:WORD_1\n"
      "v_lshlrev_b32_sdwa %[x], 0, %[w11] dst_sel:DWORD dst_unused:UNUSED_PAD src0_sel:DWORD src1_sel:BYTE_0\n"
      "ds_read_u8 %[c2], %[x]\n"
      "s_waitcnt lgkmcnt(1)\n"
      "v_lshlrev_b32 %[c0], 3, %[c0]\n"
      "v_add_u32_sdwa %[x], %[e1], %[c0] dst_sel:DWORD dst_unused:UNUSED_PAD src0_sel:WORD_0 src1_sel:DWORD\n"
      "ds_read_b32 %[e0], %[x]\n"
      "v_add_u32_sdwa %[sum], %[sum], %[e1] dst_sel:DWORD dst_unused:UNUSED_PAD src0_sel:DWORD src1_sel:WORD_1\n"
      "v_lshlrev_b32_sdwa %[x], 0, %[w11] dst_sel:DWORD dst_unused:UNUSED_PAD src0_sel:DWORD src1_sel:BYTE_1\n"
      "ds_read_u8 %[c0], %[x]\n"
      "s_waitcnt lgkmcnt(1)\n"
      "v_lshlrev_b32 %[c1], 3, %[c1]\n"
      "v_add_u32_sdwa %[x], %[e0], %[c1] dst_sel:DWORD dst_unused:UNUSED_PAD src0_sel:WORD_0 src1_sel:DWORD\n"
      "ds_read_b32 %[e1], %[x]\n"
      "v_add_u32_sdwa %[sum], %[sum], %[e0] dst_sel:DWORD dst_unused:UNUSED_PAD src0_sel:DWORD src1_sel:WORD_1\n"
      "v_lshlrev_b32_sdwa %[x], 0, %[w11] dst_sel:DWORD dst_unused:UNUSED_PAD src0_sel:DWORD src1_sel:BYTE_2\n"
      "ds_read_u8 %[c1], %[x]\n"
      "s_waitcnt lgkmcnt(1)\n"
      "v_lshlrev_b32 %[c2], 3, %[c2]\n"
      "v_add_u32_sdwa %[x], %[e1], %[c2] dst_sel:DWORD dst_unused:UNUSED_PAD src0_sel:WORD_0 src1_sel:DWORD\n"
      "ds_read_b32 %[e0], %[x]\n"
      "v_add_u32_sdwa %[sum], %[sum], %[e1] dst_sel:DWORD dst_unused:UNUSED_PAD src0_sel:DWORD src1_sel:WORD_1\n"
      "v_lshlrev_b32_sdwa %[x], 0, %[w11] dst_sel:DWORD dst_unused:UNUSED_PAD src0_sel:DWORD src1_sel:BYTE_3\n"
      "ds_read_u8 %[c2], %[x]\n"
      "s_waitcnt lgkmcnt(1)\n"
      "v_lshlrev_b32 %[c0], 3, %[c0]\n"
      "v_add_u32_sdwa %[x], %[e0], %[c0] dst_sel:DWORD dst_unused:UNUSED_PAD src0_sel:WORD_0 src1_sel:DWORD\n"
      "ds_read_b32 %[e1], %[x]\n"
      "v_add_u32_sdwa %[sum], %[sum], %[e0] dst_sel:DWORD dst_unused:UNUSED_PAD src0_sel:DWORD src1_sel:WORD_1\n"
      "v_lshlrev_b32_sdwa %[x], 0, %[w12] dst_sel:DWORD dst_unused:UNUSED_PAD src0_sel:DWORD src1_sel:BYTE_0\n"
      "ds_read_u8 %[c0], %[x]\n"
      "s_waitcnt lgkmcnt(1)\n"
      "v_lshlrev_b32 %[c1], 3, %[c1]\n"
      "v_add_u32_sdwa %[x], %[e1], %[c1] dst_sel:DWORD dst_unused:UNUSED_PAD src0_sel:WORD_0 src1_sel:DWORD\n"
      "ds_read_b32 %[e0], %[x]\n"
      "v_add_u32_sdwa %[sum], %[sum], %[e1] dst_sel:DWORD dst_unused:UNUSED_PAD src0_sel:DWORD src1_sel:WORD_1\n"
      "v_lshlrev_b32_sdwa %[x], 0, %[w12] dst_sel:DWORD dst_unused:UNUSED_PAD src0_sel:DWORD src1_sel:BYTE_1\n"
      "ds_read_u8 %[c1], %[x]\n"
      "s_waitcnt lgkmcnt(1)\n"
      "v_lshlrev_b32 %[c2], 3, %[c2]\n"
      "v_add_u32_sdwa %[x], %[e0], %[c2] dst_sel:DWORD dst_unused:UNUSED_PAD src0_sel:WORD_0 src1_sel:DWORD\n"
      "ds_read_b32 %[e1], %[x]\n"
      "v_add_u32_sdwa %[sum], %[sum], %[e0] dst_sel:DWORD dst_unused:UNUSED_PAD src0_sel:DWORD src1_sel:WORD_1\n"
      "v_lshlrev_b32_sdwa %[x], 0, %[w12] dst_sel:DWORD dst_unused:UNUSED_PAD src0_sel:DWORD src1_sel:BYTE_2\n"
      "ds_read_u8 %[c2], %[x]\n"
      "s_waitcnt lgkmcnt(1)\n"
      "v_lshlrev_b32 %[c0], 3, %[c0]\n"
      "v_add_u32_sdwa %[x], %[e1], %[c0] dst_sel:DWORD dst_unused:UNUSED_PAD src0_sel:WORD_0 src1_sel:DWORD\n"
      "ds_read_b32 %[e0], %[x]\n"
      "v_add_u32_sdwa %[sum], %[sum], %[e1] dst_sel:DWORD dst_unused:UNUSED_PAD src0_sel:DWORD src1_sel:WORD_1\n"
      "v_lshlrev_b32_sdwa %[x], 0, %[w12] dst_sel:DWORD dst_unused:UNUSED_PAD src0_sel:DWORD src1_sel:BYTE_3\n"
      "ds_read_u8 %[c0], %[x]\n"
      "s_waitcnt lgkmcnt(1)\n"
      "v_lshlrev_b32 %[c1], 3, %[c1]\n"
      "v_add_u32_sdwa %[x], %[e0], %[c1] dst_sel:DWORD dst_unused:UNUSED_PAD src0_sel:WORD_0 src1_sel:DWORD\n"
      "ds_read_b32 %[e1], %[x]\n"
      "v_add_u32_sdwa %[sum], %[sum], %[e0] dst_sel:DWORD dst_unused:UNUSED_PAD src0_sel:DWORD src1_sel:WORD_1\n"
      "v_lshlrev_b32_sdwa %[x], 0, %[w13] dst_sel:DWORD dst_unused:UNUSED_PAD src0_sel:DWORD src1_sel:BYTE_0\n"
      "ds_read_u8 %[c1], %[x]\n"
      "s_waitcnt lgkmcnt(1)\n"
      "v_lshlrev_b32 %[c2], 3, %[c2]\n"
      "v_add_u32_sdwa %[x], %[e1], %[c2] dst_sel:DWORD dst_unused:UNUSED_PAD src0_sel:WORD_0 src1_sel:DWORD\n"
      "ds_read_b32 %[e0], %[x]\n"
      "v_add_u32_sdwa %[sum], %[sum], %[e1] dst_sel:DWORD dst_unused:UNUSED_PAD src0_sel:DWORD src1_sel:WORD_1\n"
      "v_lshlrev_b32_sdwa %[x], 0, %[w13] dst_sel:DWORD dst_unused:UNUSED_PAD src0_sel:DWORD src1_sel:BYTE_1\n"
      "ds_read_u8 %[c2], %[x]\n"
      "s_waitcnt lgkmcnt(1)\n"
      "v_lshlrev_b32 %[c0], 3, %[c0]\n"
      "v_add_u32_sdwa %[x], %[e0], %[c0] dst_sel:DWORD dst_unused:UNUSED_PAD src0_sel:WORD_0 src1_sel:DWORD\n"
      "ds_read_b32 %[e1], %[x]\n"
      "v_add_u32_sdwa %[sum], %[sum], %[e0] dst_sel:DWORD dst_unused:UNUSED_PAD src0_sel:DWORD src1_sel:WORD_1\n"
      "v_lshlrev_b32_sdwa %[x], 0, %[w13] dst_sel:DWORD dst_unused:UNUSED_PAD src0_sel:DWORD src1_sel:BYTE_2\n"
      "ds_read_u8 %[c0], %[x]\n"
      "s_waitcnt lgkmcnt(1)\n"
      "v_lshlrev_b32 %[c1], 3, %[c1]\n"
      "v_add_u32_sdwa %[x], %[e1], %[c1] dst_sel:DWORD dst_unused:UNUSED_PAD src0_sel:WORD_0 src1_sel:DWORD\n"
      "ds_read_b32 %[e0], %[x]\n"
      "v_add_u32_sdwa %[sum], %[sum], %[e1] dst_sel:DWORD dst_unused:UNUSED_PAD src0_sel:DWORD src1_sel:WORD_1\n"
      "v_lshlrev_b32_sdwa %[x], 0, %[w13] dst_sel:DWORD dst_unused:UNUSED_PAD src0_sel:DWORD src1_sel:BYTE_3\n"
      "ds_read_u8 %[c1], %[x]\n"
      "s_waitcnt lgkmcnt(1)\n"
      "v_lshlrev_b32 %[c2], 3, %[c2]\n"
      "v_add_u32_sdwa %[x], %[e0], %[c2] dst_sel:DWORD dst_unused:UNUSED_PAD src0_sel:WORD_0 src1_sel:DWORD\n"
      "ds_read_b32 %[e1], %[x]\n"
      "v_add_u32_sdwa %[sum], %[sum], %[e0] dst_sel:DWORD dst_unused:UNUSED_PAD src0_sel:DWORD src1_sel:WORD_1\n"
      "v_lshlrev_b32_sdwa %[x], 0, %[w14] dst_sel:DWORD dst_unused:UNUSED_PAD src0_sel:DWORD src1_sel:BYTE_0\n"
      "ds_read_u8 %[c2], %[x]\n"
      "s_waitcnt lgkmcnt(1)\n"
      "v_lshlrev_b32 %[c0], 3, %[c0]\n"
      "v_add_u32_sdwa %[x], %[e1], %[c0] dst_sel:DWORD dst_unused:UNUSED_PAD src0_sel:WORD_0 src1_sel:DWORD\n"
      "ds_read_b32 %[e0], %[x]\n"
      "v_add_u32_sdwa %[sum], %[sum], %[e1] dst_sel:DWORD dst_unused:UNUSED_PAD src0_sel:DWORD src1_sel:WORD_1\n"
      "v_lshlrev_b32_sdwa %[x], 0, %[w14] dst_sel:DWORD dst_unused:UNUSED_PAD src0_sel:DWORD src1_sel:BYTE_1\n"
      "ds_read_u8 %[c0], %[x]\n"
      "s_waitcnt lgkmcnt(1)\n"
      "v_lshlrev_b32 %[c1], 3, %[c1]\n"
      "v_add_u32_sdwa %[x], %[e0], %[c1] dst_sel:DWORD dst_unused:UNUSED_PAD src0_sel:WORD_0 src1_sel:DWORD\n"
      "ds_read_b32 %[e1], %[x]\n"
      "v_add_u32_sdwa %[sum], %[sum], %[e0] dst_sel:DWORD dst_unused:UNUSED_PAD src0_sel:DWORD src1_sel:WORD_1\n"
      "v_lshlrev_b32_sdwa %[x], 0, %[w14] dst_sel:DWORD dst_unused:UNUSED_PAD src0_sel:DWORD src1_sel:BYTE_2\n"
      "ds_read_u8 %[c1], %[x]\n"
      "s_waitcnt lgkmcnt(1)\n"
      "v_lshlrev_b32 %[c2], 3, %[c2]\n"
      "v_add_u32_sdwa %[x], %[e1], %[c2] dst_sel:DWORD dst_unused:UNUSED_PAD src0_sel:WORD_0 src1_sel:DWORD\n"
      "ds_read_b32 %[e0], %[x]\n"
      "v_add_u32_sdwa %[sum], %[sum], %[e1] dst_sel:DWORD dst_unused:UNUSED_PAD src0_sel:DWORD src1_sel:WORD_1\n"
      "v_lshlrev_b32_sdwa %[x], 0, %[w14] dst_sel:DWORD dst_unused:UNUSED_PAD src0_sel:DWORD src1_sel:BYTE_3\n"
      "ds_read_u8 %[c2], %[x]\n"
      "s_waitcnt lgkmcnt(1)\n"
      "v_lshlrev_b32 %[c0], 3, %[c0]\n"
      "v_add_u32_sdwa %[x], %[e0], %[c0] dst_sel:DWORD dst_unused:UNUSED_PAD src0_sel:WORD_0 src1_sel:DWORD\n"
      "ds_read_b32 %[e1], %[x]\n"
      "v_add_u32_sdwa %[sum], %[sum], %[e0] dst_sel:DWORD dst_unused:UNUSED_PAD src0_sel:DWORD src1_sel:WORD_1\n"
      "v_lshlrev_b32_sdwa %[x], 0, %[w15] dst_sel:DWORD dst_unused:UNUSED_PAD src0_sel:DWORD src1_sel:BYTE_0\n"
      "ds_read_u8 %[c0], %[x]\n"
      "s_waitcnt lgkmcnt(1)\n"
      "v_lshlrev_b32 %[c1], 3, %[c1]\n"
      "v_add_u32_sdwa %[x], %[e1], %[c1] dst_sel:DWORD dst_unused:UNUSED_PAD src0_sel:WORD_0 src1_sel:DWORD\n"
      "ds_read_b32 %[e0], %[x]\n"
      "v_add_u32_sdwa %[sum], %[sum], %[e1] dst_sel:DWORD dst_unused:UNUSED_PAD src0_sel:DWORD src1_sel:WORD_1\n"
      "v_lshlrev_b32_sdwa %[x], 0, %[w15] dst_sel:DWORD dst_unused:UNUSED_PAD src0_sel:DWORD src1_sel:BYTE_1\n"
      "ds_read_u8 %[c1], %[x]\n"
      "s_waitcnt lgkmcnt(1)\n"
      "v_lshlrev_b32 %[c2], 3, %[c2]\n"
      "v_add_u32_sdwa %[x], %[e0], %[c2] dst_sel:DWORD dst_unused:UNUSED_PAD src0_sel:WORD_0 src1_sel:DWORD\n"
      "ds_read_b32 %[e1], %[x]\n"
      "v_add_u32_sdwa %[sum], %[sum], %[e0] dst_sel:DWORD dst_unused:UNUSED_PAD src0_sel:DWORD src1_sel:WORD_1\n"
      "v_lshlrev_b32_sdwa %[x], 0, %[w15] dst_sel:DWORD dst_unused:UNUSED_PAD src0_sel:DWORD src1_sel:BYTE_2\n"
      "ds_read_u8 %[c2], %[x]\n"
      "s_waitcnt lgkmcnt(1)\n"
      "v_lshlrev_b32 %[c0], 3, %[c0]\n"
      "v_add_u32_sdwa %[x], %[e1], %[c0] dst_sel:DWORD dst_unused:UNUSED_PAD src0_sel:WORD_0 src1_sel:DWORD\n"
      "ds_read_b32 %[e0], %[x]\n"
      "v_add_u32_sdwa %[sum], %[sum], %[e1] dst_sel:DWORD dst_unused:UNUSED_PAD src0_sel:DWORD src1_sel:WORD_1\n"
      "v_lshlrev_b32_sdwa %[x], 0, %[w15] dst_sel:DWORD dst_unused:UNUSED_PAD src0_sel:DWORD src1_sel:BYTE_3\n"
      "ds_read_u8 %[c0], %[x]\n"
      "s_waitcnt lgkmcnt(1)\n"
      "v_lshlrev_b32 %[c1], 3, %[c1]\n"
      "v_add_u32_sdwa %[x], %[e0], %[c1] dst_sel:DWORD dst_unused:UNUSED_PAD src0_sel:WORD_0 src1_sel:DWORD\n"
      "ds_read_b32 %[e1], %[x]\n"
      "v_add_u32_sdwa %[sum], %[sum], %[e0] dst_sel:DWORD dst_unused:UNUSED_PAD src0_sel:DWORD src1_sel:WORD_1\n"
      "s_waitcnt lgkmcnt(0)\n"
      "v_lshlrev_b32 %[c2], 3, %[c2]\n"
      "v_add_u32_sdwa %[x], %[e1], %[c2] dst_sel:DWORD dst_unused:UNUSED_PAD src0_sel:WORD_0 src1_sel:DWORD\n"
      "ds_read_b32 %[e0], %[x]\n"
      "v_add_u32_sdwa %[sum], %[sum], %[e1] dst_sel:DWORD dst_unused:UNUSED_PAD src0_sel:DWORD src1_sel:WORD_1\n"
      "s_waitcnt lgkmcnt(0)\n"
      "v_lshlrev_b32 %[c0], 3, %[c0]\n"
      "v_add_u32_sdwa %[x], %[e0], %[c0] dst_sel:DWORD dst_unused:UNUSED_PAD src0_sel:WORD_0 src1_sel:DWORD\n"
      "ds_read_b32 %[e1], %[x]\n"
      "v_add_u32_sdwa %[sum], %[sum], %[e0] dst_sel:DWORD dst_unused:UNUSED_PAD src0_sel:DWORD src1_sel:WORD_1\n"
      "s_waitcnt lgkmcnt(0)\n"
      "v_add_u32_sdwa %[sum], %[sum], %[e1] dst_sel:DWORD dst_unused:UNUSED_PAD src0_sel:DWORD src1_sel:WORD_1\n"
      "v_and_b32 %[h], 0xffff, %[e1]\n"
      : [c0] "=&v"(c0), [c1] "=&v"(c1), [c2] "=&v"(c2), [x] "=&v"(x), [e0] "=&v"(e0), [e1] "=&v"(e1), [mid] "=&v"(mid), [lenA] "=&v"(lenA), [h] "+v"(h), [sum] "+v"(sum)
      : [w0] "v"(w[0]), [w1] "v"(w[1]), [w2] "v"(w[2]), [w3] "v"(w[3]), [w4] "v"(w[4]), [w5] "v"(w[5]), [w6] "v"(w[6]), [w7] "v"(w[7]), [w8] "v"(w[8]), [w9] "v"(w[9]), [w10] "v"(w[10]), [w11] "v"(w[11]), [w12] "v"(w[12]), [w13] "v"(w[13]), [w14] "v"(w[14]), [w15] "v"(w[15])
      : "memory");
}

__device__ __forceinline__ void piece_dfrun1(const uint32_t (&w)[16], uint32_t& h, uint32_t& mid, uint32_t& lenA, uint32_t& sum) {
  uint32_t c0, c1, c2, x, e0, e1;
  asm volatile(
      "v_lshlrev_b32_sdwa %[x], 0, %[w0] dst_sel:DWORD dst_unused:UNUSED_PAD src0_sel:DWORD src1_sel:BYTE_0\n"
      "ds_read_u8 %[c0], %[x]\n"
      "v_lshlrev_b32_sdwa %[x], 0, %[w0] dst_sel:DWORD dst_unused:UNUSED_PAD src0_sel:DWORD src1_sel:BYTE_1\n"
      "ds_read_u8 %[c1], %[x]\n"
      "v_lshlrev_b32_sdwa %[x], 0, %[w0] dst_sel:DWORD dst_unused:UNUSED_PAD src0_sel:DWORD src1_sel:BYTE_2\n"
      "ds_read_u8 %[c2], %[x]\n"
      "s_waitcnt lgkmcnt(2)\n"
      "v_add_u32 %[x], %[h], %[c0]\n"
      "ds_read_b32 %[e0], %[x]\n"
      "v_lshlrev_b32_sdwa %[x], 0, %[w0] dst_sel:DWORD dst_unused:UNUSED_PAD src0_sel:DWORD src1_sel:BYTE_3\n"
      "ds_read_u8 %[c0], %[x]\n"
      "s_waitcnt lgkmcnt(1)\n"
      "v_add_u32_sdwa %[x], %[e0], %[c1] dst_sel:DWORD dst_unused:UNUSED_PAD src0_sel:WORD_0 src1_sel:DWORD\n"
      "ds_read_b32 %[e1], %[x]\n"
      "v_add_u32_sdwa %[sum], %[sum], %[e0] dst_sel:DWORD dst_unused:UNUSED_PAD src0_sel:DWORD src1_sel:WORD_1\n"
      "v_lshlrev_b32_sdwa %[x], 0, %[w1] dst_sel:DWORD dst_unused:UNUSED_PAD src0_sel:DWORD src1_sel:BYTE_0\n"
      "ds_read_u8 %[c1], %[x]\n"
      "s_waitcnt lgkmcnt(1)\n"
      "v_add_u32_sdwa %[x], %[e1], %[c2] dst_sel:DWORD dst_unused:UNUSED_PAD src0_sel:WORD_0 src1_sel:DWORD\n"
      "ds_read_b32 %[e0], %[x]\n"
      "v_add_u32_sdwa %[sum], %[sum], %[e1] dst_sel:DWORD dst_unused:UNUSED_PAD src0_sel:DWORD src1_sel:WORD_1\n"
      "v_lshlrev_b32_sdwa %[x], 0, %[w1] dst_sel:DWORD dst_unused:UNUSED_PAD src0_sel:DWORD src1_sel:BYTE_1\n"
      "ds_read_u8 %[c2], %[x]\n"
      "s_waitcnt lgkmcnt(1)\n"
      "v_add_u32_sdwa %[x], %[e0], %[c0] dst_sel:DWORD dst_unused:UNUSED_PAD src0_sel:WORD_0 src1_sel:DWORD\n"
      "ds_read_b32 %[e1], %[x]\n"
      "v_add_u32_sdwa %[sum], %[sum], %[e0] dst_sel:DWORD dst_unused:UNUSED_PAD src0_sel:DWORD src1_sel:WORD_1\n"
      "v_lshlrev_b32_sdwa %[x], 0, %[w1] dst_sel:DWORD dst_unused:UNUSED_PAD src0_sel:DWORD src1_sel:BYTE_2\n"
      "ds_read_u8 %[c0], %[x]\n"
      "s_waitcnt lgkmcnt(1)\n"
      "v_add_u32_sdwa %[x], %[e1], %[c1] dst_sel:DWORD dst_unused:UNUSED_PAD src0_sel:WORD_0 src1_sel:DWORD\n"
      "ds_read_b32 %[e0], %[x]\n"
      "v_add_u32_sdwa %[sum], %[sum], %[e1] dst_sel:DWORD dst_unused:UNUSED_PAD src0_sel:DWORD src1_sel:WORD_1\n"
      "v_lshlrev_b32_sdwa %[x], 0, %[w1] dst_sel:DWORD dst_unused:UNUSED_PAD src0_sel:DWORD src1_sel:BYTE_3\n"
      "ds_read_u8 %[c1], %[x]\n"
      "s_waitcnt lgkmcnt(1)\n"
      "v_add_u32_sdwa %[x], %[e0], %[c2] dst_sel:DWORD dst_unused:UNUSED_PAD src0_sel:WORD_0 src1_sel:DWORD\n"
      "ds_read_b32 %[e1], %[x]\n"
      "v_add_u32_sdwa %[sum], %[sum], %[e0] dst_sel:DWORD dst_unused:UNUSED_PAD src0_sel:DWORD src1_sel:WORD_1\n"
// ... 5992 lines not shown
```

kleenexlang_amd/host.py:

```python
import contextlib
import ctypes
import os

_HERE = os.path.dirname(os.path.abspath(__file__))
BUILD_DIR = os.path.join(_HERE, "_build")
PROGRAM_DIR = os.path.join(_HERE, "programs")

KX_NKERNELS = 6
KERNEL_NAMES = ("sync", "forward", "head", "backlen", "resolve", "emit")
KX_MAX_LEAVES = 256
NOFAIL = 0xFFFFFFFFFFFFFFFF


class KleenexError(RuntimeError):
    pass


class CompileError(KleenexError):
    pass


class EngineError(KleenexError):
    pass

# ... 750 lines not shown
_kxhip = None


def _lib_path(name):
    return os.path.join(BUILD_DIR, name)


def load_compiler():
    global _kexc
    if _kexc is None:
        path = _lib_path("libkexc.so")
        if not os.path.exists(path):
            raise CompileError("%s not built: run `python -c 'import __graft_entry__ as g; g.build()'`" % path)
        lib = ctypes.CDLL(path)
        lib.kexc_compile.argtypes = [ctypes.c_char_p, ctypes.c_size_t, ctypes.c_char_p, ctypes.c_int,
                                     ctypes.POINTER(ctypes.c_void_p), ctypes.POINTER(ctypes.c_size_t)]
        lib.kexc_emit_c.argtypes = lib.kexc_compile.argtypes
        lib.kexc_last_error.restype = ctypes.c_char_p
        lib.kexc_free.argtypes = [ctypes.c_void_p]
        _kexc = lib
    return _kexc


def load_engine():
    global _kxhip
    if _kxhip is None:
        path = _lib_path("libkxhip.so")
        if not os.path.exists(path):
            raise EngineError("HIP engine %s is missing: build it with __graft_entry__.build(); "
                              "there is no CPU fallback" % path)
        try:
            import torch
        except ImportError:
            pass
        lib = ctypes.CDLL(path)
        vp, sz, u32, u64 = ctypes.c_void_p, ctypes.c_size_t, ctypes.c_uint32, ctypes.c_uint64
        lib.kx_load.argtypes = [ctypes.c_char_p, sz, ctypes.POINTER(vp)]
        lib.kx_load_config.argtypes = [ctypes.c_char_p, sz, ctypes.POINTER(KxConfig), ctypes.POINTER(vp)]
        lib.kx_stage_reset_delayed_form.argtypes = [vp, u32]
        lib.kx_stage_reset_delayed_form.restype = None
        lib.kx_validate.argtypes = [ctypes.c_char_p, sz]
        lib.kx_free.argtypes = [vp]
        lib.kx_last_error.restype = ctypes.c_char_p
        lib.kx_set_config.argtypes = [vp, ctypes.POINTER(KxConfig)]
        lib.kx_num_stages.argtypes = [vp]
        lib.kx_num_stages.restype = u32
        lib.kx_stage_has_actions.argtypes = [vp, u32]
        lib.kx_stage_delayed_form.argtypes = [vp, u32]
        lib.kx_df_describe.argtypes = [ctypes.c_char_p, sz, u32, ctypes.POINTER(KxDfInfo), vp, sz]
        lib.kx_df_pending.argtypes = [ctypes.c_char_p, sz, u32, u32, u32, ctypes.POINTER(u32), ctypes.POINTER(u32), ctypes.POINTER(u32)]
        cfgp = ctypes.POINTER(KxConfig)
        lib.kx_df_describe_cfg.argtypes = [ctypes.c_char_p, sz, u32, cfgp, ctypes.POINTER(KxDfInfo), vp, sz]
        lib.kx_stage_describe_cfg.argtypes = [ctypes.c_char_p, sz, u32, cfgp, u32, ctypes.POINTER(KxStageInfo), vp, sz]
        lib.kx_df_pending_cfg.argtypes = [ctypes.c_char_p, sz, u32, cfgp, u32, u32, ctypes.POINTER(u32), ctypes.POINTER(u32), ctypes.POINTER(u32)]
        lib.kx_df_deferred.argtypes = [ctypes.c_char_p, sz, u32, cfgp, u32, ctypes.c_void_p, sz, ctypes.POINTER(sz)]
        lib.kx_df_start_of_state.argtypes = [ctypes.c_char_p, sz, u32, cfgp, u32, ctypes.POINTER(u32)]
        lib.kx_run_device.argtypes = [vp, vp, sz, vp, sz, ctypes.POINTER(sz), ctypes.POINTER(KxStats), vp]
        lib.kx_run_host.argtypes = [vp, ctypes.c_char_p, sz, ctypes.POINTER(vp), ctypes.POINTER(sz),
                                    ctypes.POINTER(KxStats)]
        lib.kx_host_free.argtypes = [vp]
        lib.kx_run_fd.argtypes = [vp, ctypes.c_int, ctypes.c_int, ctypes.POINTER(KxStats)]
        lib.kx_run_batch.argtypes = [vp, vp, vp, u64, vp, sz, vp, vp, ctypes.POINTER(sz), ctypes.POINTER(KxBatchStats), vp]
        lib.kx_run_batch_framed.argtypes = [vp, vp, vp, u64, ctypes.POINTER(KxBatchFrame), vp, sz, vp, vp, ctypes.POINTER(sz),
                                            ctypes.POINTER(KxBatchStats), vp]
        lib.kx_run_batch_fields.argtypes = [vp, vp, vp, u64, ctypes.POINTER(KxBatchFields), vp, sz, vp, vp, ctypes.POINTER(sz),
                                            ctypes.POINTER(KxBatchStats), vp]
        lib.kx_fields_stats.argtypes = [vp, ctypes.POINTER(KxFieldsKernelStats)]
        lib.kx_run_batch_field_list.argtypes = [vp, vp, vp, u64, ctypes.POINTER(KxBatchFieldList), vp, sz, vp, vp, vp, ctypes.POINTER(sz),
                                                ctypes.POINTER(KxBatchStats), vp]
        lib.kx_run_records_fd_field_list.argtypes = [vp, ctypes.c_int, ctypes.c_int, ctypes.POINTER(KxRecordsOpts), ctypes.POINTER(KxFieldRange),
                                                     u32, ctypes.c_uint8, ctypes.c_int, ctypes.POINTER(KxRecordsStats)]
        lib.kx_run_batch_field_values.argtypes = [vp, vp, vp, u64, ctypes.POINTER(KxBatchFieldList), ctypes.POINTER(KxFieldCodec), vp, sz, vp, vp, vp,
                                                  ctypes.POINTER(sz), ctypes.POINTER(KxBatchStats), vp]
        lib.kx_run_records_fd_field_values.argtypes = lib.kx_run_records_fd_field_list.argtypes
        lib.kx_run_records_fd_fields.argtypes = [vp, ctypes.c_int, ctypes.c_int, ctypes.POINTER(KxRecordsOpts), u32, ctypes.c_uint8,
                                                 ctypes.c_int, ctypes.POINTER(KxRecordsStats)]
        lib.kx_run_records_fd_opts.argtypes = [vp, ctypes.c_int, ctypes.c_int, ctypes.POINTER(KxRecordsOpts), ctypes.c_int,
                                               ctypes.POINTER(KxRecordsStats)]
        lib.kx_split_records.argtypes = [vp, sz, ctypes.c_uint8, u64, vp, u64, ctypes.POINTER(u64), vp]
        lib.kx_run_records_fd.argtypes = [vp, ctypes.c_int, ctypes.c_int, ctypes.c_uint8, ctypes.c_int, ctypes.POINTER(KxRecordsStats)]
        lib.kx_split_records_quoted.argtypes = [vp, sz, ctypes.c_uint8, ctypes.c_uint8, u32, u64, vp, u64, ctypes.POINTER(u64),
                                                ctypes.POINTER(u32), vp]
        lib.kx_run_records_fd_quoted.argtypes = [vp, ctypes.c_int, ctypes.c_int, ctypes.c_uint8, ctypes.c_uint8, ctypes.c_int,
                                                 ctypes.POINTER(KxRecordsStats)]
        lib.kx_split_records_escaped.argtypes = [vp, sz, ctypes.c_uint8, ctypes.c_int, ctypes.c_uint8, u32, u64, vp, u64,
                                                 ctypes.POINTER(u64), ctypes.POINTER(u32), vp]
        lib.kx_run_records_fd_escaped.argtypes = [vp, ctypes.c_int, ctypes.c_int, ctypes.c_uint8, ctypes.c_int, ctypes.c_uint8,
                                                  ctypes.c_int, ctypes.POINTER(KxRecordsStats)]
        lib.kx_split_records_rs.argtypes = [vp, sz, ctypes.c_char_p, u32, ctypes.c_char_p, u32, u64, vp, u64, ctypes.POINTER(u64),
                                            ctypes.POINTER(ctypes.c_uint8), ctypes.POINTER(u32), ctypes.POINTER(u64), vp]
        lib.kx_run_records_fd_rs.argtypes = [vp, ctypes.c_int, ctypes.c_int, ctypes.c_char_p, u32, ctypes.c_int,
                                             ctypes.POINTER(KxRecordsStats)]
        lib.kx_shard_begin.argtypes = [vp, u32, vp, sz, ctypes.c_int, ctypes.c_int, vp, ctypes.POINTER(vp)]
        lib.kx_shard_forward.argtypes = [vp, ctypes.POINTER(KxFwdSummary)]
        lib.kx_shard_fix_head.argtypes = [vp, u32, ctypes.POINTER(KxFwdSummary)]
        lib.kx_shard_backward.argtypes = [vp, ctypes.POINTER(KxBwdSummary)]
        lib.kx_shard_resolve.argtypes = [vp, u32, ctypes.POINTER(u64)]
        lib.kx_shard_emit.argtypes = [vp, vp, sz]
        lib.kx_shard_stats.argtypes = [vp, ctypes.POINTER(KxStats)]
        lib.kx_shard_end.argtypes = [vp]
        lib.kx_run_sharded.argtypes = [vp, ctypes.c_int, ctypes.c_int, vp, vp, vp, sz, vp, sz, ctypes.POINTER(KxShardedResult), vp]
        lib.kx_comm_unique_id.argtypes = [ctypes.c_char_p]
        lib.kx_comm_init.argtypes = [ctypes.POINTER(vp), ctypes.c_int, ctypes.c_int, ctypes.c_char_p]
        lib.kx_comm_free.argtypes = [vp]
        lib.kx_group_create.argtypes = [ctypes.c_int]
        lib.kx_group_create.restype = vp
# ... 121 lines not shown
    import json
    lib = load_compiler()
    if isinstance(regex, str):
        regex = regex.encode("utf-8")
    txt = ctypes.c_void_p()
    n = ctypes.c_size_t()
    lib.kexc_dump_regex_fst.argtypes = [ctypes.c_char_p, ctypes.c_size_t, ctypes.c_int, ctypes.POINTER(ctypes.c_void_p),
                                        ctypes.POINTER(ctypes.c_size_t)]
    rc = lib.kexc_dump_regex_fst(regex, len(regex), 1 if oracle else 0, ctypes.byref(txt), ctypes.byref(n))
    if rc:
        raise CompileError(lib.kexc_last_error().decode("utf-8", "replace"))
    try:
        return json.loads(ctypes.string_at(txt, n.value).decode("utf-8"))
    finally:
        lib.kexc_free(txt)


def validate_blob(blob):
    lib = load_engine()
    blob = bytes(blob)
    if lib.kx_validate(blob, len(blob)):
        raise EngineError(lib.kx_last_error().decode("utf-8", "replace"))


def df_describe(blob, stage=0, with_image=True, cfg=None):
    lib = load_engine()
    blob = bytes(blob)
    info = KxDfInfo()
    cfg = config_from_env() if cfg is None else cfg
    if lib.kx_df_describe_cfg(blob, len(blob), stage, ctypes.byref(cfg), ctypes.byref(info), None, 0):
        raise EngineError(lib.kx_last_error().decode("utf-8", "replace"))
    img = None
    if with_image and info.image_bytes:
        buf = ctypes.create_string_buffer(info.image_bytes)
        lib.kx_df_describe_cfg(blob, len(blob), stage, ctypes.byref(cfg), ctypes.byref(info), buf, info.image_bytes)
        img = buf.raw
    return info, img


def stage_describe(blob, stage=0, which=KX_STAGE_MAIN, cfg=None, with_image=True):
    lib = load_engine()
    blob = bytes(blob)
    info = KxStageInfo(size=ctypes.sizeof(KxStageInfo))
    cfg = config_from_env() if cfg is None else cfg
    probe = ctypes.create_string_buffer(1 << 20) if with_image else None
    if lib.kx_stage_describe_cfg(blob, len(blob), stage, ctypes.byref(cfg), which, ctypes.byref(info), probe, (1 << 20) if with_image else 0):
        raise EngineError(lib.kx_last_error().decode("utf-8", "replace"))
    if not with_image or not info.image_bytes:
        return info, None
    if info.image_bytes > (1 << 20):
        probe = ctypes.create_string_buffer(info.image_bytes)
        lib.kx_stage_describe_cfg(blob, len(blob), stage, ctypes.byref(cfg), which, ctypes.byref(info), probe, info.image_bytes)
    return info, probe.raw[:info.image_bytes]


def df_pending(blob, stage, state, slot, cfg=None):
    lib = load_engine()
    blob = bytes(blob)
    kinds = (ctypes.c_uint32 * KX_MAX_LEAVES)()
    n = ctypes.c_uint32()
    q = ctypes.c_uint32()
    cfg = config_from_env() if cfg is None else cfg
    if lib.kx_df_pending_cfg(blob, len(blob), stage, ctypes.byref(cfg), state, slot, ctypes.byref(q), kinds, ctypes.byref(n)):
        raise EngineError(lib.kx_last_error().decode("utf-8", "replace"))
    return q.value, list(kinds[:n.value])


def df_deferred(blob, stage, state, cfg=None):
    lib = load_engine()
    blob = bytes(blob)
    buf = ctypes.create_string_buffer(1024)
    n = ctypes.c_size_t()
    cfg = config_from_env() if cfg is None else cfg
    if lib.kx_df_deferred(blob, len(blob), stage, ctypes.byref(cfg), state, buf, 1024, ctypes.byref(n)):
        raise EngineError(lib.kx_last_error().decode("utf-8", "replace"))
    return buf.raw[:n.value]


def df_start_of_state(blob, stage, sst_state, cfg=None):
    lib = load_engine()
    blob = bytes(blob)
    h = ctypes.c_uint32()
    cfg = config_from_env() if cfg is None else cfg
    if lib.kx_df_start_of_state(blob, len(blob), stage, ctypes.byref(cfg), sst_state, ctypes.byref(h)):
        raise EngineError(lib.kx_last_error().decode("utf-8", "replace"))
    return h.value


class KexcIlProgram(ctypes.Structure):
    _u8p, _u16p, _u32p = ctypes.POINTER(ctypes.c_uint8), ctypes.POINTER(ctypes.c_uint16), ctypes.POINTER(ctypes.c_uint32)
    _fields_ = [("nstates", ctypes.c_uint32), ("nclasses", ctypes.c_uint32), ("init_state", ctypes.c_uint32), ("nregs", ctypes.c_uint32),
                ("class_of", _u8p), ("delta", _u16p), ("action", _u32p), ("final_action", _u32p),
                ("nactions", ctypes.c_uint32), ("action_off", _u32p), ("ops", _u32p),
                ("nconsts", ctypes.c_uint32), ("const_off", _u32p), ("const_pool", _u8p),
                ("maxleaves", ctypes.c_uint32), ("nback", ctypes.c_uint32), ("back_row", _u32p),
                ("nleaves", _u8p), ("final_leaf", _u8p), ("back", _u32p),
                ("npconsts", ctypes.c_uint32), ("pconst_off", _u32p), ("pconst_pool", _u8p), ("init_const", _u32p),
                ("has_actions", ctypes.c_uint32), ("action_regs", ctypes.c_uint32),
                ("ntables", ctypes.c_uint32), ("tbl_width", _u32p), ("tbl_data", _u8p), ("back_table", _u32p),
                ("ntests", ctypes.c_uint32), ("test_block", _u32p), ("test_target", _u32p), ("test_len", _u32p),
                ("test_preds", _u8p), ("test_back", _u32p)]


class KexcPipeline(ctypes.Structure):
    _fields_ = [("is_oracle_action", ctypes.c_int), ("nprograms", ctypes.c_uint32), ("programs", ctypes.POINTER(KexcIlProgram)),
                ("program_size", ctypes.c_uint32)]
# ... 618 lines not shown
```

Baseline: 1119.

## Stage delayed-forward table densely in LDS with odd row pitch to cut bank conflicts

The delayed-forward kernel now stages a compacted copy of the transition table in LDS. It keeps only the 4-byte lo words at an odd row pitch, replacing the 8-byte-stride entries, and translates state handles between the dense and image encodings wherever they leave or enter the kernel. The inline-asm walker's class shift drops from 3 to 2 to match the new stride. Per-lane record staging slots are also rotated by lane to spread LDS banks. The aim is fewer LDS bank conflicts and a smaller LDS footprint on the hot per-byte lookup chain, at the cost of extra handle conversions (mulhi-based) at the boundaries and a more complex staging loop.

```diff
diff --git a/include/kxhip.h b/include/kxhip.h
--- a/include/kxhip.h
+++ b/include/kxhip.h
@@ -120,6 +120,8 @@
 } kx_stage_info;
 int kx_stage_describe_cfg(const void* blob, size_t blob_len, uint32_t stage, const kx_config* cfg, uint32_t which, kx_stage_info* info,
                           void* image, size_t image_cap);
+int kx_df_dense_image(const void* blob, size_t blob_len, uint32_t stage, const kx_config* cfg, void* image, size_t image_cap, size_t* image_bytes);
+uint32_t kx_df_dense_handle(uint32_t nclasses, uint32_t off_pool, uint32_t handle, int to_dense);
 
 int kx_run_device(kx_program* prog, const void* d_in, size_t n, void* d_out, size_t cap, size_t* out_len,
                   kx_stats* stats, void* stream);
diff --git a/kleenexlang_amd/csrc/engine/gen_sweeps.py b/kleenexlang_amd/csrc/engine/gen_sweeps.py
--- a/kleenexlang_amd/csrc/engine/gen_sweeps.py
+++ b/kleenexlang_amd/csrc/engine/gen_sweeps.py
@@ -390,7 +390,7 @@
 DF_WALK_E = {"A": (("v116", "v117"), ("v118", "v119")), "B": (("v120", "v121"), ("v122", "v123"))}
 
 
-def dfrun1(wide=False):
+def dfrun1(shift=0):
     L = []
     ap = L.append
     E = (("%[e0]",), ("%[e1]",))
@@ -400,8 +400,8 @@
     for tt in (0, 1, 2):
         cls_issue(tt)
     ap("s_waitcnt lgkmcnt(2)")
-    if wide:
-        ap("v_lshlrev_b32 %[c0], 3, %[c0]")
+    if shift:
+        ap("v_lshlrev_b32 %%[c0], %d, %%[c0]" % shift)
     ap("v_add_u32 %[x], %[h], %[c0]")
     ap("ds_read_b32 %s, %%[x]" % E[0][0])
     for j in range(64):
@@ -410,8 +410,8 @@
             cls_issue(j + 3)
         ap("s_waitcnt lgkmcnt(%d)" % (1 if j + 3 < 64 else 0))
         if j + 1 < 64:
-            if wide:
-                ap("v_lshlrev_b32 %%[c%d], 3, %%[c%d]" % ((j + 1) % 3, (j + 1) % 3))
+            if shift:
+                ap("v_lshlrev_b32 %%[c%d], %d, %%[c%d]" % ((j + 1) % 3, shift, (j + 1) % 3))
             ap("v_add_u32_sdwa %%[x], %s, %%[c%d] %s src0_sel:WORD_0 src1_sel:DWORD" % (E[cur][0], (j + 1) % 3, SD))
             ap("ds_read_b32 %s, %%[x]" % E[nxt][0])
         ap("v_add_u32_sdwa %%[sum], %%[sum], %s %s src0_sel:DWORD src1_sel:WORD_1" % (E[cur][0], SD))
@@ -554,7 +554,7 @@
     emit_fn(out, "piece_dfrun1w",
             "const uint32_t (&w)[16], uint32_t& h, uint32_t& mid, uint32_t& lenA, uint32_t& sum",
             "uint32_t " + ", ".join(tmp) + ";",
-            dfrun1(True),
+            dfrun1(2),
             ['[%s] "=&v"(%s)' % (t, t) for t in tmp] + ['[mid] "=&v"(mid)', '[lenA] "=&v"(lenA)', '[h] "+v"(h)', '[sum] "+v"(sum)'],
             ['[w%d] "v"(w[%d])' % (i, i) for i in range(16)],
             '"memory"')
diff --git a/kleenexlang_amd/csrc/engine/kx_dfdense.h b/kleenexlang_amd/csrc/engine/kx_dfdense.h
--- /dev/null
+++ b/kleenexlang_amd/csrc/engine/kx_dfdense.h
@@ -0,0 +1,52 @@
+#ifndef KX_DFDENSE_H
+#define KX_DFDENSE_H
+#include <cstdint>
+#if defined(__HIPCC__)
+#define KX_DD_FN __host__ __device__ __forceinline__
+#else
+#define KX_DD_FN inline
+#endif
+
+namespace kxdd {
+
+constexpr uint32_t OFF_ROWS = 256;
+constexpr uint32_t CLS4_MAX = 63;
+
+struct Geo {
+  uint32_t C;
+  uint32_t C8, P4;
+  uint32_t m8, mP;
+  uint32_t rows;
+  uint32_t csh;
+};
+
+KX_DD_FN uint32_t pitch(uint32_t C) { return C | 1u; }
+KX_DD_FN uint32_t recip(uint32_t d) { return 0xFFFFFFFFu / d + 1u; }
+KX_DD_FN uint32_t mulhi(uint32_t a, uint32_t b) { return (uint32_t)(((uint64_t)a * b) >> 32); }
+KX_DD_FN Geo geo(uint32_t C, uint32_t off_pool) {
+  Geo g;
+  g.C = C; g.C8 = 8u * C; g.P4 = 4u * pitch(C); g.m8 = recip(g.C8); g.mP = recip(g.P4);
+  g.rows = (off_pool - OFF_ROWS) / g.C8; g.csh = C <= CLS4_MAX ? 0u : 2u;
+  return g;
+}
+KX_DD_FN uint32_t words(const Geo& g) { return OFF_ROWS / 4 + g.rows * (g.P4 / 4); }
+KX_DD_FN uint32_t row_of_image(const Geo& g, uint32_t h8) { return mulhi(h8 - OFF_ROWS, g.m8); }
+KX_DD_FN uint32_t row_of_dense(const Geo& g, uint32_t hd) { return mulhi(hd - OFF_ROWS, g.mP); }
+KX_DD_FN uint32_t to_dense(const Geo& g, uint32_t h8) { return OFF_ROWS + row_of_image(g, h8) * g.P4; }
+KX_DD_FN uint32_t to_image(const Geo& g, uint32_t hd) { return OFF_ROWS + row_of_dense(g, hd) * g.C8; }
+KX_DD_FN uint32_t cls_word(const Geo& g, uint32_t wide, uint32_t w) {
+  if (!wide) return (w >> 1) & 0x7F7F7F7Fu;
+  return g.csh ? w : w << 2;
+}
+KX_DD_FN uint32_t lo_word(const Geo& g, uint32_t lo) { return (lo & 0xFFFF0000u) | to_dense(g, lo & 0xFFFFu); }
+KX_DD_FN uint32_t dense_word(const Geo& g, uint32_t wide, const uint32_t* img, uint32_t i) {
+  if (i < OFF_ROWS / 4) return cls_word(g, wide, img[i]);
+  const uint32_t b = (i - OFF_ROWS / 4) * 4u, r = mulhi(b, g.mP), c = (b - r * g.P4) >> 2;
+  return c < g.C ? lo_word(g, img[OFF_ROWS / 4 + (r * g.C + c) * 2u]) : 0u;
+}
+KX_DD_FN uint32_t lo_next(uint32_t lo) { return lo & 0xFFFFu; }
+KX_DD_FN uint32_t lo_len(uint32_t lo) { return lo >> 24; }
+KX_DD_FN uint32_t lo_const(uint32_t lo) { return (lo >> 18) & 1u; }
+
+}
+#endif
diff --git a/kleenexlang_amd/csrc/engine/kx_dfkernels.inc b/kleenexlang_amd/csrc/engine/kx_dfkernels.inc
--- a/kleenexlang_amd/csrc/engine/kx_dfkernels.inc
+++ b/kleenexlang_amd/csrc/engine/kx_dfkernels.inc
@@ -48,6 +48,23 @@
   for (uint32_t i = threadIdx.x; i < D.words; i += blockDim.x) smem[i] = D.img[i];
   __syncthreads();
   return DfLds{reinterpret_cast<const uint8_t*>(smem), D.wide ? 3u : 0u};
+}
+struct DfDense {
+  const uint8_t* base; kxdd::Geo G;
+  __device__ __forceinline__ uint32_t c4(uint32_t byte) const { return (uint32_t)base[byte] << G.csh; }
+  __device__ __forceinline__ uint32_t lo(uint32_t a) const { return *reinterpret_cast<const uint32_t*>(base + a); }
+  __device__ __forceinline__ uint32_t step(uint32_t h, uint32_t byte) const { return lo(h + c4(byte)); }
+};
+__device__ __forceinline__ DfDense df_stage_dense(const DfDev& D, uint32_t* smem) {
+  const kxdd::Geo G = kxdd::geo(D.C, D.off_pool);
+  const uint32_t nw = kxdd::words(G);
+  for (uint32_t i = threadIdx.x; i < nw; i += blockDim.x) smem[i] = kxdd::dense_word(G, D.wide, D.img, i);
+  __syncthreads();
+  return DfDense{reinterpret_cast<const uint8_t*>(smem), G};
+}
+template <uint32_t DF_STAGE>
+__device__ __forceinline__ uint32_t df_slot(uint32_t pc, uint32_t lane) {
+  return (((((pc & (DF_STAGE - 1)) >> 1) + lane) & (DF_STAGE / 2 - 1)) << 1) | (pc & 1u);
 }
 
 __device__ __forceinline__ void df_run_piece(const uint32_t (&w)[16], uint32_t& h, uint32_t& mid, uint32_t& lenA, uint32_t& len, const DfLds& L) {
@@ -237,20 +254,21 @@
                            uint32_t* __restrict__ side, uint32_t side_cap, int is_last, DfDev D) {
   static_assert(DF_STAGE == 8 || DF_STAGE == 16, "a group of staged records is one or half a 128-byte line, and at least the slow path's 64-byte map");
   extern __shared__ __attribute__((aligned(16))) uint32_t smem[];
-  DfLds L = df_stage(D, smem);
+  const DfDense L = df_stage_dense(D, smem);
+  const kxdd::Geo& G = L.G;
   uint2* lrec = reinterpret_cast<uint2*>(smem + ((D.words + 3) & ~3u)) + (size_t)threadIdx.x * DF_STAGE;
   const uint32_t k = blockIdx.x * blockDim.x + threadIdx.x;
   const uint32_t lane = threadIdx.x & 63;
   const uint64_t B = k < nseg ? df_own_start(k, n, seg, first_known, seg_pos, seg_state, D) : UNSYNC;
   bool alive = B != UNSYNC;
-  const uint32_t dead = D.deadh, esc = D.esch;
+  const uint32_t dead = kxdd::to_dense(G, D.deadh), esc = kxdd::to_dense(G, D.esch);
   auto warm = [&](uint32_t jj, uint64_t Bj) -> uint32_t {
-    if (jj == 0 && first_known) return D.starth;
-    uint32_t hw = D.start_of_state[(((uint32_t)seg_state[jj] << D.hshift) - OFF_FWD) / D.orig_c4];
+    if (jj == 0 && first_known) return kxdd::to_dense(G, D.starth);
+    uint32_t hw = kxdd::to_dense(G, D.start_of_state[(((uint32_t)seg_state[jj] << D.hshift) - OFF_FWD) / D.orig_c4]);
     for (uint64_t pw = seg_pos[jj]; pw < Bj;) {
       const uint2 v = *reinterpret_cast<const uint2*>(in + (pw & ~7ull));
       const uint64_t x = (uint64_t)v.x | ((uint64_t)v.y << 32);
-      for (uint32_t b = (uint32_t)pw & 7u; b < 8u && pw < Bj; ++b, ++pw) hw = L.ent(hw + L.c8((uint32_t)(x >> (8 * b)) & 0xFFu)).x & 0xFFFFu;
+      for (uint32_t b = (uint32_t)pw & 7u; b < 8u && pw < Bj; ++b, ++pw) hw = kxdd::lo_next(L.step(hw, (uint32_t)(x >> (8 * b)) & 0xFFu));
     }
     if (hw == esc && jj == k) atomicAdd(&flags->warm_esc, 1u);
     return hw == esc || hw == dead ? 0xFFFFFFFFu : hw;
@@ -263,7 +281,7 @@
     const uint64_t b = df_own_start(j, n, seg, first_known, seg_pos, seg_state, D);
     if (b == UNSYNC) continue;
     h_behind = warm(j, b);
-    if (h_behind != 0xFFFFFFFFu) { end = b; break; }
+    if (h_behind != 0xFFFFFFFFu) { h_behind = kxdd::to_image(G, h_behind); end = b; break; }
   }
   const bool last = alive && j >= nseg;
   uint64_t pos = alive ? B : 0;
@@ -275,7 +293,7 @@
   auto fail_in = [&](uint32_t h0, uint64_t p0, uint32_t plen) -> int {
     uint32_t hh = h0;
     for (uint32_t t = 0; t < plen; ++t) {
-      const uint32_t nh = L.ent(hh + L.c8(in[p0 + t])).x & 0xFFFFu;
+      const uint32_t nh = kxdd::lo_next(L.step(hh, in[p0 + t]));
       if (nh == dead) { atomicMin(&flags->fail_pos, (unsigned long long)(p0 + t)); failed = true; return 1; }
       if (nh == esc) return 2;
       hh = nh;
@@ -286,7 +304,7 @@
   uint32_t nst = 0; uint64_t gfirst = 0;
   auto flush_group = [&]() {
     uint2* dst = reinterpret_cast<uint2*>(rec + gfirst);
-    for (uint32_t i = 0; i < nst; ++i) dst[i] = lrec[(gfirst + i) & (DF_STAGE - 1)];
+    for (uint32_t i = 0; i < nst; ++i) dst[i] = lrec[df_slot<DF_STAGE>((uint32_t)gfirst + i, lane)];
     nst = 0;
   };
   const bool coop = !(D.debug & 256u);
@@ -294,7 +312,7 @@
   auto stage_rec = [&](uint64_t pc, DfRec r) {
     if (nst == 0) gfirst = pc;
     if ((pc & (DF_WBASE_PIECES - 1)) == 0) wbase[pc / DF_WBASE_PIECES] = cum | flag;
-    lrec[pc & (DF_STAGE - 1)] = make_uint2(r.x, r.y); ++nst;
+    lrec[df_slot<DF_STAGE>((uint32_t)pc, lane)] = make_uint2(r.x, r.y); ++nst;
     if (!in_trip && (pc & (DF_STAGE - 1)) == DF_STAGE - 1) flush_group();
   };
   auto group_aligned = [&]() { return ((uint32_t)(pos >> 6) & (DF_STAGE - 1)) == nst; };
@@ -310,7 +328,7 @@
       const uint32_t slo = (uint32_t)__shfl((int)glo, (int)(team + i)), shi = (uint32_t)__shfl((int)ghi, (int)(team + i));
       if (!(shi & 0x80000000u)) {
         const uint64_t g = ((uint64_t)shi << 32) | slo;
-        const uint2* src = lrec_wave + (size_t)(team + i) * DF_STAGE + r;
+        const uint2* src = lrec_wave + (size_t)(team + i) * DF_STAGE + df_slot<DF_STAGE>(r, team + i);
         if constexpr (RPL == 2) *reinterpret_cast<uint4*>(rec + g + r) = *reinterpret_cast<const uint4*>(src);
         else *reinterpret_cast<uint2*>(rec + g + r) = *src;
       }
@@ -321,7 +339,7 @@
   uint32_t kc_sum = 0, kc_max = 0, kc_n = 0;
   auto slow = [&](const uint64_t a, const uint32_t h0) -> int {
     flush_group();
-    DfSlowIO io{in, n, a, end, h0, last ? 1u : 0u, (uint32_t)is_last, h_behind, side, side_cap, flags, L.base, D.wide ? 0u : 3u, reinterpret_cast<uint8_t*>(lrec), DF_HOLE_FIRST, 0, 0, 0, 0};
+    DfSlowIO io{in, n, a, end, h0, last ? 1u : 0u, (uint32_t)is_last, h_behind, side, side_cap, flags, L.base, G.csh ? 0u : 2u, reinterpret_cast<uint8_t*>(lrec), DF_HOLE_FIRST, 0, 0, 0, 0};
     {
       int rc = df_slow_resolve(io, D);
       if (rc == 3) { io.max_steps = DF_HOLE_MAX; rc = df_slow_resolve(io, D); }
@@ -347,7 +365,7 @@
       rec[pp >> 6] = dfrec_pack_hole(base + idx, cnt, first, len);
       idx += cnt; cum += len; pos = pp + steps;
     }
-    h = io.h_next;
+    h = kxdd::to_dense(G, io.h_next);
     atomicAdd(&flags->slow_steps, (uint32_t)(e_out - a));
     return 0;
   };
@@ -355,21 +373,21 @@
   auto run_slow = [&]() {
     need_slow = false;
     int r = 1;
-    if constexpr (SLOW) r = slow(pos, h);
+    if constexpr (SLOW) r = slow(pos, kxdd::to_image(G, h));
     if (r) { if (r == 1) atomicAdd(&flags->df_esc, 1u); failed = true; }
   };
   auto do_piece = [&](const uint32_t (&w)[16]) -> bool {
     cross();
     const uint32_t h0 = h;
     uint32_t mid, sumA, sum = 0;
-    if (D.wide) piece_dfrun1w(w, h, mid, sumA, sum); else piece_dfrun1(w, h, mid, sumA, sum);
+    if (G.csh) piece_dfrun1w(w, h, mid, sumA, sum); else piece_dfrun1(w, h, mid, sumA, sum);
     if (h == dead || h == esc) {
       if (fail_in(h0, pos, PIECE) == 2) { need_slow = true; h = h0; }
       return false;
     }
     const uint32_t kA = (sumA & 0xFFu) >> 2, kB = (sum & 0xFFu) >> 2;
     kc_sum += kA + kB; kc_max = kA + kB > kc_max ? kA + kB : kc_max; ++kc_n;
-    stage_rec(pos >> 6, dfrec_pack(h0, mid, sumA >> 8, sum >> 8, kA, kB));
+    stage_rec(pos >> 6, dfrec_pack(kxdd::to_image(G, h0), kxdd::to_image(G, mid), sumA >> 8, sum >> 8, kA, kB));
     cum += sum >> 8; pos += PIECE;
     return true;
   };
@@ -430,21 +448,21 @@
     uint32_t mid = h, lenA = 0, len = 0, kA = 0, kc = 0;
     for (uint32_t t = 0; t < plen; ++t) {
       if (t == HALF) { mid = h; lenA = len; kA = kc; }
-      const uint2 e = L.ent(h + L.c8(in[pos + t]));
-      h = e.x & 0xFFFFu; len += e.y >> 24; kc += (e.y >> 23) & 1u;
+      const uint32_t e = L.step(h, in[pos + t]);
+      h = kxdd::lo_next(e); len += kxdd::lo_len(e); kc += kxdd::lo_const(e);
     }
     if (plen <= HALF) { mid = h; lenA = len; kA = kc; }
     if (h == dead || h == esc) {
       if (fail_in(h0, pos, plen) == 2) { h = h0; need_slow = true; continue; }
     }
-    else { stage_rec(pos >> 6, dfrec_pack(h0, mid, lenA, len, kA, kc - kA)); cum += len; pos = end; }
+    else { stage_rec(pos >> 6, dfrec_pack(kxdd::to_image(G, h0), kxdd::to_image(G, mid), lenA, len, kA, kc - kA)); cum += len; pos = end; }
   }
   break;
   }
   flush_group();
   if (failed) return;
   (flag ? own : spill)[m] = cum;
-  if (last) flags->end_state = h;
+  if (last) flags->end_state = kxdd::to_image(G, h);
   if (kc_n) { if ((k & 15u) == 0) { atomicAdd(&flags->emit_ksum, kc_sum); atomicAdd(&flags->emit_kn, kc_n); } atomicMax(&flags->emit_kmax, kc_max); }
 }
 
diff --git a/kleenexlang_amd/csrc/engine/kx_engine.hip b/kleenexlang_amd/csrc/engine/kx_engine.hip
--- a/kleenexlang_amd/csrc/engine/kx_engine.hip
+++ b/kleenexlang_amd/csrc/engine/kx_engine.hip
@@ -1909,6 +1909,29 @@
   return 0;
 }
 
+int kx_df_dense_image(const void* blob, size_t blob_len, uint32_t stage, const kx_config* cfg, void* image, size_t image_cap, size_t* image_bytes) {
+  if (!image_bytes) return setErr(KX_E_ARG, "null argument");
+  Stage S;
+  int rc = parseOneStage(blob, blob_len, stage, cfg, S);
+  if (rc) return rc;
+  *image_bytes = 0;
+  if (!S.has_df) return 0;
+  const DfDev& D = S.D;
+  const uint32_t* img = reinterpret_cast<const uint32_t*>(S.img_df.data() + kxst::offOf(D.img));
+  const kxdd::Geo G = kxdd::geo(D.C, D.off_pool);
+  const uint32_t nw = kxdd::words(G);
+  *image_bytes = (size_t)nw * 4;
+  uint32_t* out = static_cast<uint32_t*>(image);
+  for (uint32_t i = 0; out && i < nw && ((size_t)i + 1) * 4 <= image_cap; ++i) out[i] = kxdd::dense_word(G, D.wide, img, i);
+  return 0;
+}
+
+uint32_t kx_df_dense_handle(uint32_t nclasses, uint32_t off_pool, uint32_t handle, int to_dense) {
+  if (!nclasses || off_pool < kxdd::OFF_ROWS) return 0;
+  const kxdd::Geo G = kxdd::geo(nclasses, off_pool);
+  return to_dense ? kxdd::to_dense(G, handle) : kxdd::to_image(G, handle);
+}
+
 int kx_df_describe(const void* blob, size_t blob_len, uint32_t stage, kx_df_info* info, void* image, size_t image_cap) {
   return kx_df_describe_cfg(blob, blob_len, stage, nullptr, info, image, image_cap);
 }
diff --git a/kleenexlang_amd/csrc/engine/kx_stage.h b/kleenexlang_amd/csrc/engine/kx_stage.h
--- a/kleenexlang_amd/csrc/engine/kx_stage.h
+++ b/kleenexlang_amd/csrc/engine/kx_stage.h
@@ -8,6 +8,7 @@
 #include "../../../include/kxhip.h"
 #include "../../../include/kxp_format.h"
 #include "kx_delayed.h"
+#include "kx_dfdense.h"
 
 namespace kxst {
 
diff --git a/kleenexlang_amd/csrc/engine/kx_sweeps.inc b/kleenexlang_amd/csrc/engine/kx_sweeps.inc
--- a/kleenexlang_amd/csrc/engine/kx_sweeps.inc
+++ b/kleenexlang_amd/csrc/engine/kx_sweeps.inc
@@ -6707,230 +6707,230 @@
       "v_lshlrev_b32_sdwa %[x], 0, %[w0] dst_sel:DWORD dst_unused:UNUSED_PAD src0_sel:DWORD src1_sel:BYTE_2\n"
       "ds_read_u8 %[c2], %[x]\n"
       "s_waitcnt lgkmcnt(2)\n"
-      "v_lshlrev_b32 %[c0], 3, %[c0]\n"
+      "v_lshlrev_b32 %[c0], 2, %[c0]\n"
       "v_add_u32 %[x], %[h], %[c0]\n"
       "ds_read_b32 %[e0], %[x]\n"
       "v_lshlrev_b32_sdwa %[x], 0, %[w0] dst_sel:DWORD dst_unused:UNUSED_PAD src0_sel:DWORD src1_sel:BYTE_3\n"
       "ds_read_u8 %[c0], %[x]\n"
       "s_waitcnt lgkmcnt(1)\n"
-      "v_lshlrev_b32 %[c1], 3, %[c1]\n"
+      "v_lshlrev_b32 %[c1], 2, %[c1]\n"
       "v_add_u32_sdwa %[x], %[e0], %[c1] dst_sel:DWORD dst_unused:UNUSED_PAD src0_sel:WORD_0 src1_sel:DWORD\n"
       "ds_read_b32 %[e1], %[x]\n"
       "v_add_u32_sdwa %[sum], %[sum], %[e0] dst_sel:DWORD dst_unused:UNUSED_PAD src0_sel:DWORD src1_sel:WORD_1\n"
       "v_lshlrev_b32_sdwa %[x], 0, %[w1] dst_sel:DWORD dst_unused:UNUSED_PAD src0_sel:DWORD src1_sel:BYTE_0\n"
       "ds_read_u8 %[c1], %[x]\n"
       "s_waitcnt lgkmcnt(1)\n"
-      "v_lshlrev_b32 %[c2], 3, %[c2]\n"
+      "v_lshlrev_b32 %[c2], 2, %[c2]\n"
       "v_add_u32_sdwa %[x], %[e1], %[c2] dst_sel:DWORD dst_unused:UNUSED_PAD src0_sel:WORD_0 src1_sel:DWORD\n"
       "ds_read_b32 %[e0], %[x]\n"
       "v_add_u32_sdwa %[sum], %[sum], %[e1] dst_sel:DWORD dst_unused:UNUSED_PAD src0_sel:DWORD src1_sel:WORD_1\n"
       "v_lshlrev_b32_sdwa %[x], 0, %[w1] dst_sel:DWORD dst_unused:UNUSED_PAD src0_sel:DWORD src1_sel:BYTE_1\n"
       "ds_read_u8 %[c2], %[x]\n"
       "s_waitcnt lgkmcnt(1)\n"
-      "v_lshlrev_b32 %[c0], 3, %[c0]\n"
+      "v_lshlrev_b32 %[c0], 2, %[c0]\n"
       "v_add_u32_sdwa %[x], %[e0], %[c0] dst_sel:DWORD dst_unused:UNUSED_PAD src0_sel:WORD_0 src1_sel:DWORD\n"
       "ds_read_b32 %[e1], %[x]\n"
       "v_add_u32_sdwa %[sum], %[sum], %[e0] dst_sel:DWORD dst_unused:UNUSED_PAD src0_sel:DWORD src1_sel:WORD_1\n"
       "v_lshlrev_b32_sdwa %[x], 0, %[w1] dst_sel:DWORD dst_unused:UNUSED_PAD src0_sel:DWORD src1_sel:BYTE_2\n"
       "ds_read_u8 %[c0], %[x]\n"
       "s_waitcnt lgkmcnt(1)\n"
-      "v_lshlrev_b32 %[c1], 3, %[c1]\n"
+      "v_lshlrev_b32 %[c1], 2, %[c1]\n"
       "v_add_u32_sdwa %[x], %[e1], %[c1] dst_sel:DWORD dst_unused:UNUSED_PAD src0_sel:WORD_0 src1_sel:DWORD\n"
       "ds_read_b32 %[e0], %[x]\n"
       "v_add_u32_sdwa %[sum], %[sum], %[e1] dst_sel:DWORD dst_unused:UNUSED_PAD src0_sel:DWORD src1_sel:WORD_1\n"
       "v_lshlrev_b32_sdwa %[x], 0, %[w1] dst_sel:DWORD dst_unused:UNUSED_PAD src0_sel:DWORD src1_sel:BYTE_3\n"
       "ds_read_u8 %[c1], %[x]\n"
       "s_waitcnt lgkmcnt(1)\n"
-      "v_lshlrev_b32 %[c2], 3, %[c2]\n"
+      "v_lshlrev_b32 %[c2], 2, %[c2]\n"
       "v_add_u32_sdwa %[x], %[e0], %[c2] dst_sel:DWORD dst_unused:UNUSED_PAD src0_sel:WORD_0 src1_sel:DWORD\n"
       "ds_read_b32 %[e1], %[x]\n"
       "v_add_u32_sdwa %[sum], %[sum], %[e0] dst_sel:DWORD dst_unused:UNUSED_PAD src0_sel:DWORD src1_sel:WORD_1\n"
       "v_lshlrev_b32_sdwa %[x], 0, %[w2] dst_sel:DWORD dst_unused:UNUSED_PAD src0_sel:DWORD src1_sel:BYTE_0\n"
       "ds_read_u8 %[c2], %[x]\n"
       "s_waitcnt lgkmcnt(1)\n"
-      "v_lshlrev_b32 %[c0], 3, %[c0]\n"
+      "v_lshlrev_b32 %[c0], 2, %[c0]\n"
       "v_add_u32_sdwa %[x], %[e1], %[c0] dst_sel:DWORD dst_unused:UNUSED_PAD src0_sel:WORD_0 src1_sel:DWORD\n"
       "ds_read_b32 %[e0], %[x]\n"
       "v_add_u32_sdwa %[sum], %[sum], %[e1] dst_sel:DWORD dst_unused:UNUSED_PAD src0_sel:DWORD src1_sel:WORD_1\n"
       "v_lshlrev_b32_sdwa %[x], 0, %[w2] dst_sel:DWORD dst_unused:UNUSED_PAD src0_sel:DWORD src1_sel:BYTE_1\n"
       "ds_read_u8 %[c0], %[x]\n"
       "s_waitcnt lgkmcnt(1)\n"
-      "v_lshlrev_b32 %[c1], 3, %[c1]\n"
+      "v_lshlrev_b32 %[c1], 2, %[c1]\n"
       "v_add_u32_sdwa %[x], %[e0], %[c1] dst_sel:DWORD dst_unused:UNUSED_PAD src0_sel:WORD_0 src1_sel:DWORD\n"
       "ds_read_b32 %[e1], %[x]\n"
       "v_add_u32_sdwa %[sum], %[sum], %[e0] dst_sel:DWORD dst_unused:UNUSED_PAD src0_sel:DWORD src1_sel:WORD_1\n"
       "v_lshlrev_b32_sdwa %[x], 0, %[w2] dst_sel:DWORD dst_unused:UNUSED_PAD src0_sel:DWORD src1_sel:BYTE_2\n"
       "ds_read_u8 %[c1], %[x]\n"
       "s_waitcnt lgkmcnt(1)\n"
-      "v_lshlrev_b32 %[c2], 3, %[c2]\n"
+      "v_lshlrev_b32 %[c2], 2, %[c2]\n"
       "v_add_u32_sdwa %[x], %[e1], %[c2] dst_sel:DWORD dst_unused:UNUSED_PAD src0_sel:WORD_0 src1_sel:DWORD\n"
       "ds_read_b32 %[e0], %[x]\n"
       "v_add_u32_sdwa %[sum], %[sum], %[e1] dst_sel:DWORD dst_unused:UNUSED_PAD src0_sel:DWORD src1_sel:WORD_1\n"
       "v_lshlrev_b32_sdwa %[x], 0, %[w2] dst_sel:DWORD dst_unused:UNUSED_PAD src0_sel:DWORD src1_sel:BYTE_3\n"
       "ds_read_u8 %[c2], %[x]\n"
       "s_waitcnt lgkmcnt(1)\n"
-      "v_lshlrev_b32 %[c0], 3, %[c0]\n"
+      "v_lshlrev_b32 %[c0], 2, %[c0]\n"
       "v_add_u32_sdwa %[x], %[e0], %[c0] dst_sel:DWORD dst_unused:UNUSED_PAD src0_sel:WORD_0 src1_sel:DWORD\n"
       "ds_read_b32 %[e1], %[x]\n"
       "v_add_u32_sdwa %[sum], %[sum], %[e0] dst_sel:DWORD dst_unused:UNUSED_PAD src0_sel:DWORD src1_sel:WORD_1\n"
       "v_lshlrev_b32_sdwa %[x], 0, %[w3] dst_sel:DWORD dst_unused:UNUSED_PAD src0_sel:DWORD src1_sel:BYTE_0\n"
       "ds_read_u8 %[c0], %[x]\n"
       "s_waitcnt lgkmcnt(1)\n"
-      "v_lshlrev_b32 %[c1], 3, %[c1]\n"
+      "v_lshlrev_b32 %[c1], 2, %[c1]\n"
       "v_add_u32_sdwa %[x], %[e1], %[c1] dst_sel:DWORD dst_unused:UNUSED_PAD src0_sel:WORD_0 src1_sel:DWORD\n"
       "ds_read_b32 %[e0], %[x]\n"
       "v_add_u32_sdwa %[sum], %[sum], %[e1] dst_sel:DWORD dst_unused:UNUSED_PAD src0_sel:DWORD src1_sel:WORD_1\n"
       "v_lshlrev_b32_sdwa %[x], 0, %[w3] dst_sel:DWORD dst_unused:UNUSED_PAD src0_sel:DWORD src1_sel:BYTE_1\n"
       "ds_read_u8 %[c1], %[x]\n"
       "s_waitcnt lgkmcnt(1)\n"
-      "v_lshlrev_b32 %[c2], 3, %[c2]\n"
+      "v_lshlrev_b32 %[c2], 2, %[c2]\n"
       "v_add_u32_sdwa %[x], %[e0], %[c2] dst_sel:DWORD dst_unused:UNUSED_PAD src0_sel:WORD_0 src1_sel:DWORD\n"
       "ds_read_b32 %[e1], %[x]\n"
       "v_add_u32_sdwa %[sum], %[sum], %[e0] dst_sel:DWORD dst_unused:UNUSED_PAD src0_sel:DWORD src1_sel:WORD_1\n"
       "v_lshlrev_b32_sdwa %[x], 0, %[w3] dst_sel:DWORD dst_unused:UNUSED_PAD src0_sel:DWORD src1_sel:BYTE_2\n"
       "ds_read_u8 %[c2], %[x]\n"
       "s_waitcnt lgkmcnt(1)\n"
-      "v_lshlrev_b32 %[c0], 3, %[c0]\n"
+      "v_lshlrev_b32 %[c0], 2, %[c0]\n"
       "v_add_u32_sdwa %[x], %[e1], %[c0] dst_sel:DWORD dst_unused:UNUSED_PAD src0_sel:WORD_0 src1_sel:DWORD\n"
       "ds_read_b32 %[e0], %[x]\n"
       "v_add_u32_sdwa %[sum], %[sum], %[e1] dst_sel:DWORD dst_unused:UNUSED_PAD src0_sel:DWORD src1_sel:WORD_1\n"
       "v_lshlrev_b32_sdwa %[x], 0, %[w3] dst_sel:DWORD dst_unused:UNUSED_PAD src0_sel:DWORD src1_sel:BYTE_3\n"
       "ds_read_u8 %[c0], %[x]\n"
       "s_waitcnt lgkmcnt(1)\n"
-      "v_lshlrev_b32 %[c1], 3, %[c1]\n"
+      "v_lshlrev_b32 %[c1], 2, %[c1]\n"
       "v_add_u32_sdwa %[x], %[e0], %[c1] dst_sel:DWORD dst_unused:UNUSED_PAD src0_sel:WORD_0 src1_sel:DWORD\n"
       "ds_read_b32 %[e1], %[x]\n"
       "v_add_u32_sdwa %[sum], %[sum], %[e0] dst_sel:DWORD dst_unused:UNUSED_PAD src0_sel:DWORD src1_sel:WORD_1\n"
       "v_lshlrev_b32_sdwa %[x], 0, %[w4] dst_sel:DWORD dst_unused:UNUSED_PAD src0_sel:DWORD src1_sel:BYTE_0\n"
       "ds_read_u8 %[c1], %[x]\n"
       "s_waitcnt lgkmcnt(1)\n"
-      "v_lshlrev_b32 %[c2], 3, %[c2]\n"
+      "v_lshlrev_b32 %[c2], 2, %[c2]\n"
       "v_add_u32_sdwa %[x], %[e1], %[c2] dst_sel:DWORD dst_unused:UNUSED_PAD src0_sel:WORD_0 src1_sel:DWORD\n"
       "ds_read_b32 %[e0], %[x]\n"
       "v_add_u32_sdwa %[sum], %[sum], %[e1] dst_sel:DWORD dst_unused:UNUSED_PAD src0_sel:DWORD src1_sel:WORD_1\n"
       "v_lshlrev_b32_sdwa %[x], 0, %[w4] dst_sel:DWORD dst_unused:UNUSED_PAD src0_sel:DWORD src1_sel:BYTE_1\n"
       "ds_read_u8 %[c2], %[x]\n"
       "s_waitcnt lgkmcnt(1)\n"
-      "v_lshlrev_b32 %[c0], 3, %[c0]\n"
+      "v_lshlrev_b32 %[c0], 2, %[c0]\n"
       "v_add_u32_sdwa %[x], %[e0], %[c0] dst_sel:DWORD dst_unused:UNUSED_PAD src0_sel:WORD_0 src1_sel:DWORD\n"
       "ds_read_b32 %[e1], %[x]\n"
       "v_add_u32_sdwa %[sum], %[sum], %[e0] dst_sel:DWORD dst_unused:UNUSED_PAD src0_sel:DWORD src1_sel:WORD_1\n"
       "v_lshlrev_b32_sdwa %[x], 0, %[w4] dst_sel:DWORD dst_unused:UNUSED_PAD src0_sel:DWORD src1_sel:BYTE_2\n"
       "ds_read_u8 %[c0], %[x]\n"
       "s_waitcnt lgkmcnt(1)\n"
-      "v_lshlrev_b32 %[c1], 3, %[c1]\n"
+      "v_lshlrev_b32 %[c1], 2, %[c1]\n"
       "v_add_u32_sdwa %[x], %[e1], %[c1] dst_sel:DWORD dst_unused:UNUSED_PAD src0_sel:WORD_0 src1_sel:DWORD\n"
       "ds_read_b32 %[e0], %[x]\n"
       "v_add_u32_sdwa %[sum], %[sum], %[e1] dst_sel:DWORD dst_unused:UNUSED_PAD src0_sel:DWORD src1_sel:WORD_1\n"
       "v_lshlrev_b32_sdwa %[x], 0, %[w4] dst_sel:DWORD dst_unused:UNUSED_PAD src0_sel:DWORD src1_sel:BYTE_3\n"
       "ds_read_u8 %[c1], %[x]\n"
       "s_waitcnt lgkmcnt(1)\n"
-      "v_lshlrev_b32 %[c2], 3, %[c2]\n"
+      "v_lshlrev_b32 %[c2], 2, %[c2]\n"
       "v_add_u32_sdwa %[x], %[e0], %[c2] dst_sel:DWORD dst_unused:UNUSED_PAD src0_sel:WORD_0 src1_sel:DWORD\n"
       "ds_read_b32 %[e1], %[x]\n"
       "v_add_u32_sdwa %[sum], %[sum], %[e0] dst_sel:DWORD dst_unused:UNUSED_PAD src0_sel:DWORD src1_sel:WORD_1\n"
       "v_lshlrev_b32_sdwa %[x], 0, %[w5] dst_sel:DWORD dst_unused:UNUSED_PAD src0_sel:DWORD src1_sel:BYTE_0\n"
       "ds_read_u8 %[c2], %[x]\n"
       "s_waitcnt lgkmcnt(1)\n"
-      "v_lshlrev_b32 %[c0], 3, %[c0]\n"
+      "v_lshlrev_b32 %[c0], 2, %[c0]\n"
       "v_add_u32_sdwa %[x], %[e1], %[c0] dst_sel:DWORD dst_unused:UNUSED_PAD src0_sel:WORD_0 src1_sel:DWORD\n"
       "ds_read_b32 %[e0], %[x]\n"
       "v_add_u32_sdwa %[sum], %[sum], %[e1] dst_sel:DWORD dst_unused:UNUSED_PAD src0_sel:DWORD src1_sel:WORD_1\n"
       "v_lshlrev_b32_sdwa %[x], 0, %[w5] dst_sel:DWORD dst_unused:UNUSED_PAD src0_sel:DWORD src1_sel:BYTE_1\n"
       "ds_read_u8 %[c0], %[x]\n"
       "s_waitcnt lgkmcnt(1)\n"
-      "v_lshlrev_b32 %[c1], 3, %[c1]\n"
+      "v_lshlrev_b32 %[c1], 2, %[c1]\n"
       "v_add_u32_sdwa %[x], %[e0], %[c1] dst_sel:DWORD dst_unused:UNUSED_PAD src0_sel:WORD_0 src1_sel:DWORD\n"
       "ds_read_b32 %[e1], %[x]\n"
       "v_add_u32_sdwa %[sum], %[sum], %[e0] dst_sel:DWORD dst_unused:UNUSED_PAD src0_sel:DWORD src1_sel:WORD_1\n"
       "v_lshlrev_b32_sdwa %[x], 0, %[w5] dst_sel:DWORD dst_unused:UNUSED_PAD src0_sel:DWORD src1_sel:BYTE_2\n"
       "ds_read_u8 %[c1], %[x]\n"
       "s_waitcnt lgkmcnt(1)\n"
-      "v_lshlrev_b32 %[c2], 3, %[c2]\n"
+      "v_lshlrev_b32 %[c2], 2, %[c2]\n"
       "v_add_u32_sdwa %[x], %[e1], %[c2] dst_sel:DWORD dst_unused:UNUSED_PAD src0_sel:WORD_0 src1_sel:DWORD\n"
       "ds_read_b32 %[e0], %[x]\n"
       "v_add_u32_sdwa %[sum], %[sum], %[e1] dst_sel:DWORD dst_unused:UNUSED_PAD src0_sel:DWORD src1_sel:WORD_1\n"
       "v_lshlrev_b32_sdwa %[x], 0, %[w5] dst_sel:DWORD dst_unused:UNUSED_PAD src0_sel:DWORD src1_sel:BYTE_3\n"
       "ds_read_u8 %[c2], %[x]\n"
       "s_waitcnt lgkmcnt(1)\n"
-      "v_lshlrev_b32 %[c0], 3, %[c0]\n"
+      "v_lshlrev_b32 %[c0], 2, %[c0]\n"
       "v_add_u32_sdwa %[x], %[e0], %[c0] dst_sel:DWORD dst_unused:UNUSED_PAD src0_sel:WORD_0 src1_sel:DWORD\n"
       "ds_read_b32 %[e1], %[x]\n"
       "v_add_u32_sdwa %[sum], %[sum], %[e0] dst_sel:DWORD dst_unused:UNUSED_PAD src0_sel:DWORD src1_sel:WORD_1\n"
       "v_lshlrev_b32_sdwa %[x], 0, %[w6] dst_sel:DWORD dst_unused:UNUSED_PAD src0_sel:DWORD src1_sel:BYTE_0\n"
       "ds_read_u8 %[c0], %[x]\n"
       "s_waitcnt lgkmcnt(1)\n"
-      "v_lshlrev_b32 %[c1], 3, %[c1]\n"
+      "v_lshlrev_b32 %[c1], 2, %[c1]\n"
       "v_add_u32_sdwa %[x], %[e1], %[c1] dst_sel:DWORD dst_unused:UNUSED_PAD src0_sel:WORD_0 src1_sel:DWORD\n"
       "ds_read_b32 %[e0], %[x]\n"
       "v_add_u32_sdwa %[sum], %[sum], %[e1] dst_sel:DWORD dst_unused:UNUSED_PAD src0_sel:DWORD src1_sel:WORD_1\n"
       "v_lshlrev_b32_sdwa %[x], 0, %[w6] dst_sel:DWORD dst_unused:UNUSED_PAD src0_sel:DWORD src1_sel:BYTE_1\n"
       "ds_read_u8 %[c1], %[x]\n"
       "s_waitcnt lgkmcnt(1)\n"
-      "v_lshlrev_b32 %[c2], 3, %[c2]\n"
+      "v_lshlrev_b32 %[c2], 2, %[c2]\n"
       "v_add_u32_sdwa %[x], %[e0], %[c2] dst_sel:DWORD dst_unused:UNUSED_PAD src0_sel:WORD_0 src1_sel:DWORD\n"
       "ds_read_b32 %[e1], %[x]\n"
       "v_add_u32_sdwa %[sum], %[sum], %[e0] dst_sel:DWORD dst_unused:UNUSED_PAD src0_sel:DWORD src1_sel:WORD_1\n"
       "v_lshlrev_b32_sdwa %[x], 0, %[w6] dst_sel:DWORD dst_unused:UNUSED_PAD src0_sel:DWORD src1_sel:BYTE_2\n"
       "ds_read_u8 %[c2], %[x]\n"
       "s_waitcnt lgkmcnt(1)\n"
-      "v_lshlrev_b32 %[c0], 3, %[c0]\n"
+      "v_lshlrev_b32 %[c0], 2, %[c0]\n"
       "v_add_u32_sdwa %[x], %[e1], %[c0] dst_sel:DWORD dst_unused:UNUSED_PAD src0_sel:WORD_0 src1_sel:DWORD\n"
       "ds_read_b32 %[e0], %[x]\n"
       "v_add_u32_sdwa %[sum], %[sum], %[e1] dst_sel:DWORD dst_unused:UNUSED_PAD src0_sel:DWORD src1_sel:WORD_1\n"
       "v_lshlrev_b32_sdwa %[x], 0, %[w6] dst_sel:DWORD dst_unused:UNUSED_PAD src0_sel:DWORD src1_sel:BYTE_3\n"
       "ds_read_u8 %[c0], %[x]\n"
       "s_waitcnt lgkmcnt(1)\n"
-      "v_lshlrev_b32 %[c1], 3, %[c1]\n"
+      "v_lshlrev_b32 %[c1], 2, %[c1]\n"
       "v_add_u32_sdwa %[x], %[e0], %[c1] dst_sel:DWORD dst_unused:UNUSED_PAD src0_sel:WORD_0 src1_sel:DWORD\n"
       "ds_read_b32 %[e1], %[x]\n"
       "v_add_u32_sdwa %[sum], %[sum], %[e0] dst_sel:DWORD dst_unused:UNUSED_PAD src0_sel:DWORD src1_sel:WORD_1\n"
       "v_lshlrev_b32_sdwa %[x], 0, %[w7] dst_sel:DWORD dst_unused:UNUSED_PAD src0_sel:DWORD src1_sel:BYTE_0\n"
       "ds_read_u8 %[c1], %[x]\n"
       "s_waitcnt lgkmcnt(1)\n"
-      "v_lshlrev_b32 %[c2], 3, %[c2]\n"
+      "v_lshlrev_b32 %[c2], 2, %[c2]\n"
       "v_add_u32_sdwa %[x], %[e1], %[c2] dst_sel:DWORD dst_unused:UNUSED_PAD src0_sel:WORD_0 src1_sel:DWORD\n"
       "ds_read_b32 %[e0], %[x]\n"
       "v_add_u32_sdwa %[sum], %[sum], %[e1] dst_sel:DWORD dst_unused:UNUSED_PAD src0_sel:DWORD src1_sel:WORD_1\n"
       "v_lshlrev_b32_sdwa %[x], 0, %[w7] dst_sel:DWORD dst_unused:UNUSED_PAD src0_sel:DWORD src1_sel:BYTE_1\n"
       "ds_read_u8 %[c2], %[x]\n"
       "s_waitcnt lgkmcnt(1)\n"
-      "v_lshlrev_b32 %[c0], 3, %[c0]\n"
+      "v_lshlrev_b32 %[c0], 2, %[c0]\n"
       "v_add_u32_sdwa %[x], %[e0], %[c0] dst_sel:DWORD dst_unused:UNUSED_PAD src0_sel:WORD_0 src1_sel:DWORD\n"
       "ds_read_b32 %[e1], %[x]\n"
       "v_add_u32_sdwa %[sum], %[sum], %[e0] dst_sel:DWORD dst_unused:UNUSED_PAD src0_sel:DWORD src1_sel:WORD_1\n"
       "v_lshlrev_b32_sdwa %[x], 0, %[w7] dst_sel:DWORD dst_unused:UNUSED_PAD src0_sel:DWORD src1_sel:BYTE_2\n"
       "ds_read_u8 %[c0], %[x]\n"
       "s_waitcnt lgkmcnt(1)\n"
-      "v_lshlrev_b32 %[c1], 3, %[c1]\n"
+      "v_lshlrev_b32 %[c1], 2, %[c1]\n"
       "v_add_u32_sdwa %[x], %[e1], %[c1] dst_sel:DWORD dst_unused:UNUSED_PAD src0_sel:WORD_0 src1_sel:DWORD\n"
       "ds_read_b32 %[e0], %[x]\n"
       "v_add_u32_sdwa %[sum], %[sum], %[e1] dst_sel:DWORD dst_unused:UNUSED_PAD src0_sel:DWORD src1_sel:WORD_1\n"
       "v_lshlrev_b32_sdwa %[x], 0, %[w7] dst_sel:DWORD dst_unused:UNUSED_PAD src0_sel:DWORD src1_sel:BYTE_3\n"
       "ds_read_u8 %[c1], %[x]\n"
       "s_waitcnt lgkmcnt(1)\n"
-      "v_lshlrev_b32 %[c2], 3, %[c2]\n"
+      "v_lshlrev_b32 %[c2], 2, %[c2]\n"
       "v_add_u32_sdwa %[x], %[e0], %[c2] dst_sel:DWORD dst_unused:UNUSED_PAD src0_sel:WORD_0 src1_sel:DWORD\n"
       "ds_read_b32 %[e1], %[x]\n"
       "v_add_u32_sdwa %[sum], %[sum], %[e0] dst_sel:DWORD dst_unused:UNUSED_PAD src0_sel:DWORD src1_sel:WORD_1\n"
       "v_lshlrev_b32_sdwa %[x], 0, %[w8] dst_sel:DWORD dst_unused:UNUSED_PAD src0_sel:DWORD src1_sel:BYTE_0\n"
       "ds_read_u8 %[c2], %[x]\n"
       "s_waitcnt lgkmcnt(1)\n"
-      "v_lshlrev_b32 %[c0], 3, %[c0]\n"
+      "v_lshlrev_b32 %[c0], 2, %[c0]\n"
       "v_add_u32_sdwa %[x], %[e1], %[c0] dst_sel:DWORD dst_unused:UNUSED_PAD src0_sel:WORD_0 src1_sel:DWORD\n"
       "ds_read_b32 %[e0], %[x]\n"
       "v_add_u32_sdwa %[sum], %[sum], %[e1] dst_sel:DWORD dst_unused:UNUSED_PAD src0_sel:DWORD src1_sel:WORD_1\n"
       "v_lshlrev_b32_sdwa %[x], 0, %[w8] dst_sel:DWORD dst_unused:UNUSED_PAD src0_sel:DWORD src1_sel:BYTE_1\n"
       "ds_read_u8 %[c0], %[x]\n"
       "s_waitcnt lgkmcnt(1)\n"
-      "v_lshlrev_b32 %[c1], 3, %[c1]\n"
+      "v_lshlrev_b32 %[c1], 2, %[c1]\n"
       "v_add_u32_sdwa %[x], %[e0], %[c1] dst_sel:DWORD dst_unused:UNUSED_PAD src0_sel:WORD_0 src1_sel:DWORD\n"
       "ds_read_b32 %[e1], %[x]\n"
       "v_add_u32_sdwa %[sum], %[sum], %[e0] dst_sel:DWORD dst_unused:UNUSED_PAD src0_sel:DWORD src1_sel:WORD_1\n"
       "v_lshlrev_b32_sdwa %[x], 0, %[w8] dst_sel:DWORD dst_unused:UNUSED_PAD src0_sel:DWORD src1_sel:BYTE_2\n"
       "ds_read_u8 %[c1], %[x]\n"
       "s_waitcnt lgkmcnt(1)\n"
-      "v_lshlrev_b32 %[c2], 3, %[c2]\n"
+      "v_lshlrev_b32 %[c2], 2, %[c2]\n"
       "v_add_u32_sdwa %[x], %[e1], %[c2] dst_sel:DWORD dst_unused:UNUSED_PAD src0_sel:WORD_0 src1_sel:DWORD\n"
       "ds_read_b32 %[e0], %[x]\n"
       "v_add_u32_sdwa %[sum], %[sum], %[e1] dst_sel:DWORD dst_unused:UNUSED_PAD src0_sel:DWORD src1_sel:WORD_1\n"
@@ -6940,213 +6940,213 @@
       "v_lshlrev_b32_sdwa %[x], 0, %[w8] dst_sel:DWORD dst_unused:UNUSED_PAD src0_sel:DWORD src1_sel:BYTE_3\n"
       "ds_read_u8 %[c2], %[x]\n"
       "s_waitcnt lgkmcnt(1)\n"
-      "v_lshlrev_b32 %[c0], 3, %[c0]\n"
+      "v_lshlrev_b32 %[c0], 2, %[c0]\n"
       "v_add_u32_sdwa %[x], %[e0], %[c0] dst_sel:DWORD dst_unused:UNUSED_PAD src0_sel:WORD_0 src1_sel:DWORD\n"
       "ds_read_b32 %[e1], %[x]\n"
       "v_add_u32_sdwa %[sum], %[sum], %[e0] dst_sel:DWORD dst_unused:UNUSED_PAD src0_sel:DWORD src1_sel:WORD_1\n"
       "v_lshlrev_b32_sdwa %[x], 0, %[w9] dst_sel:DWORD dst_unused:UNUSED_PAD src0_sel:DWORD src1_sel:BYTE_0\n"
       "ds_read_u8 %[c0], %[x]\n"
       "s_waitcnt lgkmcnt(1)\n"
-      "v_lshlrev_b32 %[c1], 3, %[c1]\n"
+      "v_lshlrev_b32 %[c1], 2, %[c1]\n"
       "v_add_u32_sdwa %[x], %[e1], %[c1] dst_sel:DWORD dst_unused:UNUSED_PAD src0_sel:WORD_0 src1_sel:DWORD\n"
       "ds_read_b32 %[e0], %[x]\n"
       "v_add_u32_sdwa %[sum], %[sum], %[e1] dst_sel:DWORD dst_unused:UNUSED_PAD src0_sel:DWORD src1_sel:WORD_1\n"
       "v_lshlrev_b32_sdwa %[x], 0, %[w9] dst_sel:DWORD dst_unused:UNUSED_PAD src0_sel:DWORD src1_sel:BYTE_1\n"
       "ds_read_u8 %[c1], %[x]\n"
       "s_waitcnt lgkmcnt(1)\n"
-      "v_lshlrev_b32 %[c2], 3, %[c2]\n"
+      "v_lshlrev_b32 %[c2], 2, %[c2]\n"
       "v_add_u32_sdwa %[x], %[e0], %[c2] dst_sel:DWORD dst_unused:UNUSED_PAD src0_sel:WORD_0 src1_sel:DWORD\n"
       "ds_read_b32 %[e1], %[x]\n"
       "v_add_u32_sdwa %[sum], %[sum], %[e0] dst_sel:DWORD dst_unused:UNUSED_PAD src0_sel:DWORD src1_sel:WORD_1\n"
       "v_lshlrev_b32_sdwa %[x], 0, %[w9] dst_sel:DWORD dst_unused:UNUSED_PAD src0_sel:DWORD src1_sel:BYTE_2\n"
       "ds_read_u8 %[c2], %[x]\n"
       "s_waitcnt lgkmcnt(1)\n"
-      "v_lshlrev_b32 %[c0], 3, %[c0]\n"
+      "v_lshlrev_b32 %[c0], 2, %[c0]\n"
       "v_add_u32_sdwa %[x], %[e1], %[c0] dst_sel:DWORD dst_unused:UNUSED_PAD src0_sel:WORD_0 src1_sel:DWORD\n"
       "ds_read_b32 %[e0], %[x]\n"
       "v_add_u32_sdwa %[sum], %[sum], %[e1] dst_sel:DWORD dst_unused:UNUSED_PAD src0_sel:DWORD src1_sel:WORD_1\n"
       "v_lshlrev_b32_sdwa %[x], 0, %[w9] dst_sel:DWORD dst_unused:UNUSED_PAD src0_sel:DWORD src1_sel:BYTE_3\n"
       "ds_read_u8 %[c0], %[x]\n"
       "s_waitcnt lgkmcnt(1)\n"
-      "v_lshlrev_b32 %[c1], 3, %[c1]\n"
+      "v_lshlrev_b32 %[c1], 2, %[c1]\n"
       "v_add_u32_sdwa %[x], %[e0], %[c1] dst_sel:DWORD dst_unused:UNUSED_PAD src0_sel:WORD_0 src1_sel:DWORD\n"
       "ds_read_b32 %[e1], %[x]\n"
       "v_add_u32_sdwa %[sum], %[sum], %[e0] dst_sel:DWORD dst_unused:UNUSED_PAD src0_sel:DWORD src1_sel:WORD_1\n"
       "v_lshlrev_b32_sdwa %[x], 0, %[w10] dst_sel:DWORD dst_unused:UNUSED_PAD src0_sel:DWORD src1_sel:BYTE_0\n"
       "ds_read_u8 %[c1], %[x]\n"
       "s_waitcnt lgkmcnt(1)\n"
-      "v_lshlrev_b32 %[c2], 3, %[c2]\n"
+      "v_lshlrev_b32 %[c2], 2, %[c2]\n"
       "v_add_u32_sdwa %[x], %[e1], %[c2] dst_sel:DWORD dst_unused:UNUSED_PAD src0_sel:WORD_0 src1_sel:DWORD\n"
       "ds_read_b32 %[e0], %[x]\n"
       "v_add_u32_sdwa %[sum], %[sum], %[e1] dst_sel:DWORD dst_unused:UNUSED_PAD src0_sel:DWORD src1_sel:WORD_1\n"
       "v_lshlrev_b32_sdwa %[x], 0, %[w10] dst_sel:DWORD dst_unused:UNUSED_PAD src0_sel:DWORD src1_sel:BYTE_1\n"
       "ds_read_u8 %[c2], %[x]\n"
       "s_waitcnt lgkmcnt(1)\n"
-      "v_lshlrev_b32 %[c0], 3, %[c0]\n"
+      "v_lshlrev_b32 %[c0], 2, %[c0]\n"
       "v_add_u32_sdwa %[x], %[e0], %[c0] dst_sel:DWORD dst_unused:UNUSED_PAD src0_sel:WORD_0 src1_sel:DWORD\n"
       "ds_read_b32 %[e1], %[x]\n"
       "v_add_u32_sdwa %[sum], %[sum], %[e0] dst_sel:DWORD dst_unused:UNUSED_PAD src0_sel:DWORD src1_sel:WORD_1\n"
       "v_lshlrev_b32_sdwa %[x], 0, %[w10] dst_sel:DWORD dst_unused:UNUSED_PAD src0_sel:DWORD src1_sel:BYTE_2\n"
       "ds_read_u8 %[c0], %[x]\n"
       "s_waitcnt lgkmcnt(1)\n"
-      "v_lshlrev_b32 %[c1], 3, %[c1]\n"
+      "v_lshlrev_b32 %[c1], 2, %[c1]\n"
       "v_add_u32_sdwa %[x], %[e1], %[c1] dst_sel:DWORD dst_unused:UNUSED_PAD src0_sel:WORD_0 src1_sel:DWORD\n"
       "ds_read_b32 %[e0], %[x]\n"
       "v_add_u32_sdwa %[sum], %[sum], %[e1] dst_sel:DWORD dst_unused:UNUSED_PAD src0_sel:DWORD src1_sel:WORD_1\n"
       "v_lshlrev_b32_sdwa %[x], 0, %[w10] dst_sel:DWORD dst_unused:UNUSED_PAD src0_sel:DWORD src1_sel:BYTE_3\n"
       "ds_read_u8 %[c1], %[x]\n"
       "s_waitcnt lgkmcnt(1)\n"
-      "v_lshlrev_b32 %[c2], 3, %[c2]\n"
+      "v_lshlrev_b32 %[c2], 2, %[c2]\n"
       "v_add_u32_sdwa %[x], %[e0], %[c2] dst_sel:DWORD dst_unused:UNUSED_PAD src0_sel:WORD_0 src1_sel:DWORD\n"
       "ds_read_b32 %[e1], %[x]\n"
       "v_add_u32_sdwa %[sum], %[sum], %[e0] dst_sel:DWORD dst_unused:UNUSED_PAD src0_sel:DWORD src1_sel:WORD_1\n"
       "v_lshlrev_b32_sdwa %[x], 0, %[w11] dst_sel:DWORD dst_unused:UNUSED_PAD src0_sel:DWORD src1_sel:BYTE_0\n"
       "ds_read_u8 %[c2], %[x]\n"
       "s_waitcnt lgkmcnt(1)\n"
-      "v_lshlrev_b32 %[c0], 3, %[c0]\n"
+      "v_lshlrev_b32 %[c0], 2, %[c0]\n"
       "v_add_u32_sdwa %[x], %[e1], %[c0] dst_sel:DWORD dst_unused:UNUSED_PAD src0_sel:WORD_0 src1_sel:DWORD\n"
       "ds_read_b32 %[e0], %[x]\n"
       "v_add_u32_sdwa %[sum], %[sum], %[e1] dst_sel:DWORD dst_unused:UNUSED_PAD src0_sel:DWORD src1_sel:WORD_1\n"
       "v_lshlrev_b32_sdwa %[x], 0, %[w11] dst_sel:DWORD dst_unused:UNUSED_PAD src0_sel:DWORD src1_sel:BYTE_1\n"
       "ds_read_u8 %[c0], %[x]\n"
       "s_waitcnt lgkmcnt(1)\n"
-      "v_lshlrev_b32 %[c1], 3, %[c1]\n"
+      "v_lshlrev_b32 %[c1], 2, %[c1]\n"
       "v_add_u32_sdwa %[x], %[e0], %[c1] dst_sel:DWORD dst_unused:UNUSED_PAD src0_sel:WORD_0 src1_sel:DWORD\n"
       "ds_read_b32 %[e1], %[x]\n"
       "v_add_u32_sdwa %[sum], %[sum], %[e0] dst_sel:DWORD dst_unused:UNUSED_PAD src0_sel:DWORD src1_sel:WORD_1\n"
       "v_lshlrev_b32_sdwa %[x], 0, %[w11] dst_sel:DWORD dst_unused:UNUSED_PAD src0_sel:DWORD src1_sel:BYTE_2\n"
       "ds_read_u8 %[c1], %[x]\n"
       "s_waitcnt lgkmcnt(1)\n"
-      "v_lshlrev_b32 %[c2], 3, %[c2]\n"
+      "v_lshlrev_b32 %[c2], 2, %[c2]\n"
       "v_add_u32_sdwa %[x], %[e1], %[c2] dst_sel:DWORD dst_unused:UNUSED_PAD src0_sel:WORD_0 src1_sel:DWORD\n"
       "ds_read_b32 %[e0], %[x]\n"
       "v_add_u32_sdwa %[sum], %[sum], %[e1] dst_sel:DWORD dst_unused:UNUSED_PAD src0_sel:DWORD src1_sel:WORD_1\n"
       "v_lshlrev_b32_sdwa %[x], 0, %[w11] dst_sel:DWORD dst_unused:UNUSED_PAD src0_sel:DWORD src1_sel:BYTE_3\n"
       "ds_read_u8 %[c2], %[x]\n"
       "s_waitcnt lgkmcnt(1)\n"
-      "v_lshlrev_b32 %[c0], 3, %[c0]\n"
+      "v_lshlrev_b32 %[c0], 2, %[c0]\n"
       "v_add_u32_sdwa %[x], %[e0], %[c0] dst_sel:DWORD dst_unused:UNUSED_PAD src0_sel:WORD_0 src1_sel:DWORD\n"
       "ds_read_b32 %[e1], %[x]\n"
       "v_add_u32_sdwa %[sum], %[sum], %[e0] dst_sel:DWORD dst_unused:UNUSED_PAD src0_sel:DWORD src1_sel:WORD_1\n"
       "v_lshlrev_b32_sdwa %[x], 0, %[w12] dst_sel:DWORD dst_unused:UNUSED_PAD src0_sel:DWORD src1_sel:BYTE_0\n"
       "ds_read_u8 %[c0], %[x]\n"
       "s_waitcnt lgkmcnt(1)\n"
-      "v_lshlrev_b32 %[c1], 3, %[c1]\n"
+      "v_lshlrev_b32 %[c1], 2, %[c1]\n"
       "v_add_u32_sdwa %[x], %[e1], %[c1] dst_sel:DWORD dst_unused:UNUSED_PAD src0_sel:WORD_0 src1_sel:DWORD\n"
       "ds_read_b32 %[e0], %[x]\n"
       "v_add_u32_sdwa %[sum], %[sum], %[e1] dst_sel:DWORD dst_unused:UNUSED_PAD src0_sel:DWORD src1_sel:WORD_1\n"
       "v_lshlrev_b32_sdwa %[x], 0, %[w12] dst_sel:DWORD dst_unused:UNUSED_PAD src0_sel:DWORD src1_sel:BYTE_1\n"
       "ds_read_u8 %[c1], %[x]\n"
       "s_waitcnt lgkmcnt(1)\n"
-      "v_lshlrev_b32 %[c2], 3, %[c2]\n"
+      "v_lshlrev_b32 %[c2], 2, %[c2]\n"
       "v_add_u32_sdwa %[x], %[e0], %[c2] dst_sel:DWORD dst_unused:UNUSED_PAD src0_sel:WORD_0 src1_sel:DWORD\n"
       "ds_read_b32 %[e1], %[x]\n"
       "v_add_u32_sdwa %[sum], %[sum], %[e0] dst_sel:DWORD dst_unused:UNUSED_PAD src0_sel:DWORD src1_sel:WORD_1\n"
       "v_lshlrev_b32_sdwa %[x], 0, %[w12] dst_sel:DWORD dst_unused:UNUSED_PAD src0_sel:DWORD src1_sel:BYTE_2\n"
       "ds_read_u8 %[c2], %[x]\n"
       "s_waitcnt lgkmcnt(1)\n"
-      "v_lshlrev_b32 %[c0], 3, %[c0]\n"
+      "v_lshlrev_b32 %[c0], 2, %[c0]\n"
       "v_add_u32_sdwa %[x], %[e1], %[c0] dst_sel:DWORD dst_unused:UNUSED_PAD src0_sel:WORD_0 src1_sel:DWORD\n"
       "ds_read_b32 %[e0], %[x]\n"
       "v_add_u32_sdwa %[sum], %[sum], %[e1] dst_sel:DWORD dst_unused:UNUSED_PAD src0_sel:DWORD src1_sel:WORD_1\n"
       "v_lshlrev_b32_sdwa %[x], 0, %[w12] dst_sel:DWORD dst_unused:UNUSED_PAD src0_sel:DWORD src1_sel:BYTE_3\n"
       "ds_read_u8 %[c0], %[x]\n"
       "s_waitcnt lgkmcnt(1)\n"
-      "v_lshlrev_b32 %[c1], 3, %[c1]\n"
+      "v_lshlrev_b32 %[c1], 2, %[c1]\n"
       "v_add_u32_sdwa %[x], %[e0], %[c1] dst_sel:DWORD dst_unused:UNUSED_PAD src0_sel:WORD_0 src1_sel:DWORD\n"
       "ds_read_b32 %[e1], %[x]\n"
       "v_add_u32_sdwa %[sum], %[sum], %[e0] dst_sel:DWORD dst_unused:UNUSED_PAD src0_sel:DWORD src1_sel:WORD_1\n"
       "v_lshlrev_b32_sdwa %[x], 0, %[w13] dst_sel:DWORD dst_unused:UNUSED_PAD src0_sel:DWORD src1_sel:BYTE_0\n"
       "ds_read_u8 %[c1], %[x]\n"
       "s_waitcnt lgkmcnt(1)\n"
-      "v_lshlrev_b32 %[c2], 3, %[c2]\n"
+      "v_lshlrev_b32 %[c2], 2, %[c2]\n"
       "v_add_u32_sdwa %[x], %[e1], %[c2] dst_sel:DWORD dst_unused:UNUSED_PAD src0_sel:WORD_0 src1_sel:DWORD\n"
       "ds_read_b32 %[e0], %[x]\n"
       "v_add_u32_sdwa %[sum], %[sum], %[e1] dst_sel:DWORD dst_unused:UNUSED_PAD src0_sel:DWORD src1_sel:WORD_1\n"
       "v_lshlrev_b32_sdwa %[x], 0, %[w13] dst_sel:DWORD dst_unused:UNUSED_PAD src0_sel:DWORD src1_sel:BYTE_1\n"
       "ds_read_u8 %[c2], %[x]\n"
       "s_waitcnt lgkmcnt(1)\n"
-      "v_lshlrev_b32 %[c0], 3, %[c0]\n"
+      "v_lshlrev_b32 %[c0], 2, %[c0]\n"
       "v_add_u32_sdwa %[x], %[e0], %[c0] dst_sel:DWORD dst_unused:UNUSED_PAD src0_sel:WORD_0 src1_sel:DWORD\n"
       "ds_read_b32 %[e1], %[x]\n"
       "v_add_u32_sdwa %[sum], %[sum], %[e0] dst_sel:DWORD dst_unused:UNUSED_PAD src0_sel:DWORD src1_sel:WORD_1\n"
       "v_lshlrev_b32_sdwa %[x], 0, %[w13] dst_sel:DWORD dst_unused:UNUSED_PAD src0_sel:DWORD src1_sel:BYTE_2\n"
       "ds_read_u8 %[c0], %[x]\n"
       "s_waitcnt lgkmcnt(1)\n"
-      "v_lshlrev_b32 %[c1], 3, %[c1]\n"
+      "v_lshlrev_b32 %[c1], 2, %[c1]\n"
       "v_add_u32_sdwa %[x], %[e1], %[c1] dst_sel:DWORD dst_unused:UNUSED_PAD src0_sel:WORD_0 src1_sel:DWORD\n"
       "ds_read_b32 %[e0], %[x]\n"
       "v_add_u32_sdwa %[sum], %[sum], %[e1] dst_sel:DWORD dst_unused:UNUSED_PAD src0_sel:DWORD src1_sel:WORD_1\n"
       "v_lshlrev_b32_sdwa %[x], 0, %[w13] dst_sel:DWORD dst_unused:UNUSED_PAD src0_sel:DWORD src1_sel:BYTE_3\n"
       "ds_read_u8 %[c1], %[x]\n"
       "s_waitcnt lgkmcnt(1)\n"
-      "v_lshlrev_b32 %[c2], 3, %[c2]\n"
+      "v_lshlrev_b32 %[c2], 2, %[c2]\n"
       "v_add_u32_sdwa %[x], %[e0], %[c2] dst_sel:DWORD dst_unused:UNUSED_PAD src0_sel:WORD_0 src1_sel:DWORD\n"
       "ds_read_b32 %[e1], %[x]\n"
       "v_add_u32_sdwa %[sum], %[sum], %[e0] dst_sel:DWORD dst_unused:UNUSED_PAD src0_sel:DWORD src1_sel:WORD_1\n"
       "v_lshlrev_b32_sdwa %[x], 0, %[w14] dst_sel:DWORD dst_unused:UNUSED_PAD src0_sel:DWORD src1_sel:BYTE_0\n"
       "ds_read_u8 %[c2], %[x]\n"
       "s_waitcnt lgkmcnt(1)\n"
-      "v_lshlrev_b32 %[c0], 3, %[c0]\n"
+      "v_lshlrev_b32 %[c0], 2, %[c0]\n"
       "v_add_u32_sdwa %[x], %[e1], %[c0] dst_sel:DWORD dst_unused:UNUSED_PAD src0_sel:WORD_0 src1_sel:DWORD\n"
       "ds_read_b32 %[e0], %[x]\n"
       "v_add_u32_sdwa %[sum], %[sum], %[e1] dst_sel:DWORD dst_unused:UNUSED_PAD src0_sel:DWORD src1_sel:WORD_1\n"
       "v_lshlrev_b32_sdwa %[x], 0, %[w14] dst_sel:DWORD dst_unused:UNUSED_PAD src0_sel:DWORD src1_sel:BYTE_1\n"
       "ds_read_u8 %[c0], %[x]\n"
       "s_waitcnt lgkmcnt(1)\n"
-      "v_lshlrev_b32 %[c1], 3, %[c1]\n"
+      "v_lshlrev_b32 %[c1], 2, %[c1]\n"
       "v_add_u32_sdwa %[x], %[e0], %[c1] dst_sel:DWORD dst_unused:UNUSED_PAD src0_sel:WORD_0 src1_sel:DWORD\n"
       "ds_read_b32 %[e1], %[x]\n"
       "v_add_u32_sdwa %[sum], %[sum], %[e0] dst_sel:DWORD dst_unused:UNUSED_PAD src0_sel:DWORD src1_sel:WORD_1\n"
       "v_lshlrev_b32_sdwa %[x], 0, %[w14] dst_sel:DWORD dst_unused:UNUSED_PAD src0_sel:DWORD src1_sel:BYTE_2\n"
       "ds_read_u8 %[c1], %[x]\n"
       "s_waitcnt lgkmcnt(1)\n"
-      "v_lshlrev_b32 %[c2], 3, %[c2]\n"
+      "v_lshlrev_b32 %[c2], 2, %[c2]\n"
       "v_add_u32_sdwa %[x], %[e1], %[c2] dst_sel:DWORD dst_unused:UNUSED_PAD src0_sel:WORD_0 src1_sel:DWORD\n"
       "ds_read_b32 %[e0], %[x]\n"
       "v_add_u32_sdwa %[sum], %[sum], %[e1] dst_sel:DWORD dst_unused:UNUSED_PAD src0_sel:DWORD src1_sel:WORD_1\n"
       "v_lshlrev_b32_sdwa %[x], 0, %[w14] dst_sel:DWORD dst_unused:UNUSED_PAD src0_sel:DWORD src1_sel:BYTE_3\n"
       "ds_read_u8 %[c2], %[x]\n"
       "s_waitcnt lgkmcnt(1)\n"
-      "v_lshlrev_b32 %[c0], 3, %[c0]\n"
+      "v_lshlrev_b32 %[c0], 2, %[c0]\n"
       "v_add_u32_sdwa %[x], %[e0], %[c0] dst_sel:DWORD dst_unused:UNUSED_PAD src0_sel:WORD_0 src1_sel:DWORD\n"
       "ds_read_b32 %[e1], %[x]\n"
       "v_add_u32_sdwa %[sum], %[sum], %[e0] dst_sel:DWORD dst_unused:UNUSED_PAD src0_sel:DWORD src1_sel:WORD_1\n"
       "v_lshlrev_b32_sdwa %[x], 0, %[w15] dst_sel:DWORD dst_unused:UNUSED_PAD src0_sel:DWORD src1_sel:BYTE_0\n"
       "ds_read_u8 %[c0], %[x]\n"
       "s_waitcnt lgkmcnt(1)\n"
-      "v_lshlrev_b32 %[c1], 3, %[c1]\n"
+      "v_lshlrev_b32 %[c1], 2, %[c1]\n"
       "v_add_u32_sdwa %[x], %[e1], %[c1] dst_sel:DWORD dst_unused:UNUSED_PAD src0_sel:WORD_0 src1_sel:DWORD\n"
       "ds_read_b32 %[e0], %[x]\n"
       "v_add_u32_sdwa %[sum], %[sum], %[e1] dst_sel:DWORD dst_unused:UNUSED_PAD src0_sel:DWORD src1_sel:WORD_1\n"
       "v_lshlrev_b32_sdwa %[x], 0, %[w15] dst_sel:DWORD dst_unused:UNUSED_PAD src0_sel:DWORD src1_sel:BYTE_1\n"
       "ds_read_u8 %[c1], %[x]\n"
       "s_waitcnt lgkmcnt(1)\n"
-      "v_lshlrev_b32 %[c2], 3, %[c2]\n"
+      "v_lshlrev_b32 %[c2], 2, %[c2]\n"
       "v_add_u32_sdwa %[x], %[e0], %[c2] dst_sel:DWORD dst_unused:UNUSED_PAD src0_sel:WORD_0 src1_sel:DWORD\n"
       "ds_read_b32 %[e1], %[x]\n"
       "v_add_u32_sdwa %[sum], %[sum], %[e0] dst_sel:DWORD dst_unused:UNUSED_PAD src0_sel:DWORD src1_sel:WORD_1\n"
       "v_lshlrev_b32_sdwa %[x], 0, %[w15] dst_sel:DWORD dst_unused:UNUSED_PAD src0_sel:DWORD src1_sel:BYTE_2\n"
       "ds_read_u8 %[c2], %[x]\n"
       "s_waitcnt lgkmcnt(1)\n"
-      "v_lshlrev_b32 %[c0], 3, %[c0]\n"
+      "v_lshlrev_b32 %[c0], 2, %[c0]\n"
       "v_add_u32_sdwa %[x], %[e1], %[c0] dst_sel:DWORD dst_unused:UNUSED_PAD src0_sel:WORD_0 src1_sel:DWORD\n"
       "ds_read_b32 %[e0], %[x]\n"
       "v_add_u32_sdwa %[sum], %[sum], %[e1] dst_sel:DWORD dst_unused:UNUSED_PAD src0_sel:DWORD src1_sel:WORD_1\n"
       "v_lshlrev_b32_sdwa %[x], 0, %[w15] dst_sel:DWORD dst_unused:UNUSED_PAD src0_sel:DWORD src1_sel:BYTE_3\n"
       "ds_read_u8 %[c0], %[x]\n"
       "s_waitcnt lgkmcnt(1)\n"
-      "v_lshlrev_b32 %[c1], 3, %[c1]\n"
+      "v_lshlrev_b32 %[c1], 2, %[c1]\n"
       "v_add_u32_sdwa %[x], %[e0], %[c1] dst_sel:DWORD dst_unused:UNUSED_PAD src0_sel:WORD_0 src1_sel:DWORD\n"
       "ds_read_b32 %[e1], %[x]\n"
       "v_add_u32_sdwa %[sum], %[sum], %[e0] dst_sel:DWORD dst_unused:UNUSED_PAD src0_sel:DWORD src1_sel:WORD_1\n"
       "s_waitcnt lgkmcnt(0)\n"
-      "v_lshlrev_b32 %[c2], 3, %[c2]\n"
+      "v_lshlrev_b32 %[c2], 2, %[c2]\n"
       "v_add_u32_sdwa %[x], %[e1], %[c2] dst_sel:DWORD dst_unused:UNUSED_PAD src0_sel:WORD_0 src1_sel:DWORD\n"
       "ds_read_b32 %[e0], %[x]\n"
       "v_add_u32_sdwa %[sum], %[sum], %[e1] dst_sel:DWORD dst_unused:UNUSED_PAD src0_sel:DWORD src1_sel:WORD_1\n"
       "s_waitcnt lgkmcnt(0)\n"
-      "v_lshlrev_b32 %[c0], 3, %[c0]\n"
+      "v_lshlrev_b32 %[c0], 2, %[c0]\n"
       "v_add_u32_sdwa %[x], %[e0], %[c0] dst_sel:DWORD dst_unused:UNUSED_PAD src0_sel:WORD_0 src1_sel:DWORD\n"
       "ds_read_b32 %[e1], %[x]\n"
       "v_add_u32_sdwa %[sum], %[sum], %[e0] dst_sel:DWORD dst_unused:UNUSED_PAD src0_sel:DWORD src1_sel:WORD_1\n"
diff --git a/kleenexlang_amd/host.py b/kleenexlang_amd/host.py
--- a/kleenexlang_amd/host.py
+++ b/kleenexlang_amd/host.py
@@ -826,6 +826,9 @@
         cfgp = ctypes.POINTER(KxConfig)
         lib.kx_df_describe_cfg.argtypes = [ctypes.c_char_p, sz, u32, cfgp, ctypes.POINTER(KxDfInfo), vp, sz]
         lib.kx_stage_describe_cfg.argtypes = [ctypes.c_char_p, sz, u32, cfgp, u32, ctypes.POINTER(KxStageInfo), vp, sz]
+        lib.kx_df_dense_image.argtypes = [ctypes.c_char_p, sz, u32, cfgp, vp, sz, ctypes.POINTER(sz)]
+        lib.kx_df_dense_handle.argtypes = [u32, u32, u32, ctypes.c_int]
+        lib.kx_df_dense_handle.restype = u32
         lib.kx_df_pending_cfg.argtypes = [ctypes.c_char_p, sz, u32, cfgp, u32, u32, ctypes.POINTER(u32), ctypes.POINTER(u32), ctypes.POINTER(u32)]
         lib.kx_df_deferred.argtypes = [ctypes.c_char_p, sz, u32, cfgp, u32, ctypes.c_void_p, sz, ctypes.POINTER(sz)]
         lib.kx_df_start_of_state.argtypes = [ctypes.c_char_p, sz, u32, cfgp, u32, ctypes.POINTER(u32)]
@@ -1053,6 +1056,22 @@
         probe = ctypes.create_string_buffer(info.image_bytes)
         lib.kx_stage_describe_cfg(blob, len(blob), stage, ctypes.byref(cfg), which, ctypes.byref(info), probe, info.image_bytes)
     return info, probe.raw[:info.image_bytes]
+
+
+def df_dense_image(blob, stage=0, cfg=None):
+    lib = load_engine()
+    blob = bytes(blob)
+    cfg = config_from_env() if cfg is None else cfg
+    n = ctypes.c_size_t()
+    buf = ctypes.create_string_buffer(1 << 17)
+    if lib.kx_df_dense_image(blob, len(blob), stage, ctypes.byref(cfg), buf, len(buf), ctypes.byref(n)):
+        raise EngineError(lib.kx_last_error().decode("utf-8", "replace"))
+    assert n.value <= len(buf)
+    return buf.raw[:n.value]
+
+
+def df_dense_handle(nclasses, off_pool, handle, to_dense=True):
+    return load_engine().kx_df_dense_handle(nclasses, off_pool, handle, 1 if to_dense else 0)
 
 
 def df_pending(blob, stage, state, slot, cfg=None):
diff --git a/profiles/df_bank_model.py b/profiles/df_bank_model.py
--- /dev/null
+++ b/profiles/df_bank_model.py
@@ -0,0 +1,52 @@
+import os
+import sys
+
+import numpy as np
+
+ROOT = os.path.dirname(os.path.dirname(os.path.abspath(__file__)))
+sys.path.insert(0, ROOT)
+from kleenexlang_amd import compile_file, host, workloads
+
+
+def walk(d, img, data):
+    C = d.C
+    cls = np.frombuffer(img[:256], np.uint8).astype(np.int64)
+    cls = cls if d.wide else cls >> 3
+    w = np.frombuffer(img[:d.words * 4], "<u4")
+    lo = (w[64:64 + (d.off_pool - 256) // 4:2] & 0xFFFF).astype(np.int64).tolist()
+    rows, cl = np.zeros(len(data), np.int64), cls[np.frombuffer(data, np.uint8)]
+    r = (d.starth - 256) // (8 * C)
+    for i, c in enumerate(cl.tolist()):
+        rows[i] = r
+        r = (lo[r * C + c] - 256) // (8 * C)
+    return rows, cl
+
+
+def cost(words, trials=4000, seed=1):
+    rng = np.random.default_rng(seed)
+    tot = 0
+    for _ in range(trials):
+        w = words[rng.integers(0, len(words), 64)]
+        for h in (w[:32], w[32:]):
+            tot += np.bincount(np.unique(h) % 32, minlength=32).max()
+    return tot / trials
+
+
+def main():
+    name = sys.argv[1]
+    n = int(sys.argv[2]) if len(sys.argv) > 2 else 1 << 19
+    info, img = host.stage_describe(compile_file(name), which=host.KX_STAGE_DELAYED, cfg=host.KxConfig())
+    d = info.d
+    data = workloads.generate(workloads.PROGRAM_INPUT[name], n, seed=3)
+    rows, cl = walk(d, img, data)
+    C, P = d.C, d.C | 1
+    even = P + 1
+    print("%s: C = %d, %d rows, %d entries in use, %d steps; lanes at independent positions" % (name, C, (d.off_pool - 256) // (8 * C), len(np.unique(rows * C + cl)), len(data)))
+    print("  cycles per entry read (conflict-free = 2):")
+    print("    image, lo words at 8-byte stride          %.2f" % cost(64 + (rows * C + cl) * 2))
+    print("    dense, 4-byte stride, odd pitch %-3d        %.2f" % (P, cost(64 + rows * P + cl)))
+    print("    dense, 4-byte stride, even pitch %-3d       %.2f" % (even, cost(64 + rows * even + cl)))
+
+
+if __name__ == "__main__":
+    main()
```

New measurement: 1112. Within noise of the previous version (-0.6%).
